# jmschrei/PyPore

Measured on NVIDIA B200. Metric: Msamples/s segmented (threshold+SpeedyStatSplit), higher is better.
Workload: dtype f64

## Files before the change

### include/pypore_b200.h

```cpp
#ifndef PYPORE_B200_H
#define PYPORE_B200_H

#include <stdint.h>

#ifdef __cplusplus
extern "C" {
#endif

typedef struct pp_ctx pp_ctx;

enum pp_status {
    PP_OK = 0,
    PP_ERR_CUDA = -1,
    PP_ERR_ARG = -2,
    PP_ERR_CAPACITY = -3,
    PP_ERR_STATE = -4,
    PP_ERR_FILTER_LEN = -5
};

enum pp_rule {
    PP_RULE_DURATION_GT = 1,
    PP_RULE_MIN_GT = 2,
    PP_RULE_MAX_LT = 4,
    PP_RULE_DURATION_LT = 8
};

enum pp_prefix_mode {
    PP_PREFIX_AUTO = 0,
    PP_PREFIX_SEQUENTIAL = 1,
    PP_PREFIX_PARALLEL = 2
};

int pp_version(void);
int pp_device_count(void);
int pp_create(int device, void *cuda_stream, pp_ctx **out);
void pp_destroy(pp_ctx *ctx);
const char *pp_last_error(pp_ctx *ctx);
int pp_sync(pp_ctx *ctx);
void *pp_stream(pp_ctx *ctx);
int pp_host_alloc(pp_ctx *ctx, int64_t bytes, void **out);
void pp_host_free(pp_ctx *ctx, void *p);
enum pp_option {
    PP_OPT_SCREEN = 0,
    PP_OPT_SPINE = 1,
    PP_OPT_SPLIT_CTAS = 2,
    PP_OPT_SPLIT_KERNEL = 3
};
int pp_set_option(pp_ctx *ctx, int option, int64_t value);
int pp_get_option(pp_ctx *ctx, int option, int64_t *value);
int64_t pp_launch_count(pp_ctx *ctx);
int pp_stage_ms(pp_ctx *ctx, int stage, float *ms);

int pp_trace_upload(pp_ctx *ctx, const float *host, int64_t n, int64_t extra_capacity);
int pp_trace_upload_f64(pp_ctx *ctx, const double *host, int64_t n);
int pp_trace_upload_adc16(pp_ctx *ctx, const int16_t *host, int64_t n, double scale, double offset);
int pp_adc16_check(double scale, double offset);
int pp_adc16_key_threshold(double scale, double offset, double threshold, int32_t *key, int32_t *kxor);
int pp_trace_prefetch(pp_ctx *ctx, const float *host, int64_t n, int64_t extra_capacity);
int pp_trace_swap(pp_ctx *ctx);
int pp_trace_prefetch_ms(pp_ctx *ctx, float *ms);
int pp_trace_adopt(pp_ctx *ctx, const float *dev, int64_t n, int64_t capacity);
int pp_trace_append(pp_ctx *ctx, const float *src, int64_t n, int src_is_device);
int pp_trace_truncate(pp_ctx *ctx, int64_t n);
int pp_trace_extend(pp_ctx *ctx, int64_t n);
int64_t pp_trace_len(pp_ctx *ctx);
const float *pp_trace_device_ptr(pp_ctx *ctx);

int pp_threshold_scan(pp_ctx *ctx, double threshold, int64_t scan_len, int64_t *n_runs);
int pp_runs_download(pp_ctx *ctx, int64_t cap, int64_t *start, int64_t *length, double *mn,
                     double *mx, uint8_t *below);
int pp_runs_download_range(pp_ctx *ctx, int64_t first, int64_t count, int64_t *start, int64_t *length,
                           double *mn, double *mx, uint8_t *below);
int pp_select_events(pp_ctx *ctx, int rule_mask, int64_t duration_gt, int64_t duration_lt,
                     double min_gt, double max_lt, int skip_first, int skip_last,
                     int64_t *n_events, int64_t *n_event_samples);
int pp_set_events(pp_ctx *ctx, const int64_t *start, const int64_t *length, int64_t n_events);
int pp_append_event(pp_ctx *ctx, int64_t start, int64_t length);
int pp_events_download(pp_ctx *ctx, int64_t cap, int64_t *start, int64_t *length);

int pp_events_upload_f64(pp_ctx *ctx, const double *host, const int64_t *length, int64_t n_events);

int pp_filter_events(pp_ctx *ctx, const double *b, const double *a, const double *zi, int ncoef);
int pp_event_samples_download(pp_ctx *ctx, int64_t cap, double *out);

int pp_statsplit(pp_ctx *ctx, int min_width, int max_width, int window_width, double min_gain,
                 int prefix_mode, int64_t *n_segments);
int pp_prefix(pp_ctx *ctx, int prefix_mode);
int pp_window_gains(pp_ctx *ctx, int64_t ev, int n_windows, const int32_t *ps, const int32_t *pe, int min_width,
                    double *out, int64_t cap);

int pp_segment_stats(pp_ctx *ctx);
int pp_segments_download(pp_ctx *ctx, int64_t cap, int32_t *event, int64_t *start, int64_t *end,
                         double *mean, double *std, double *mn, double *mx);
int pp_event_stats_download(pp_ctx *ctx, int64_t cap, double *mean, double *std, double *mn, double *mx);
const void *pp_table_device_ptr(pp_ctx *ctx, int which);
int pp_split_counters(pp_ctx *ctx, int64_t out[8]);

int pp_debug_screen(pp_ctx *ctx, int64_t ev, int ps, int pe, int min_width, double *h_screen,
                    double *h_exact, uint8_t *ok, double *eps);
int pp_debug_prefix(pp_ctx *ctx, int64_t cap, double *c, double *c2, uint8_t *redone);

int pp_debug_lg2_error(pp_ctx *ctx, double *max_err);

typedef struct pp_pipeline_params {
    double threshold;
    int rule_mask;
    int64_t duration_gt, duration_lt;
    double min_gt, max_lt;
    int filter_ncoef;
    const double *filter_b, *filter_a, *filter_zi;
    int min_width, max_width, window_width;
    double min_gain;
    int prefix_mode;
    int with_stats;
} pp_pipeline_params;
int pp_pipeline(pp_ctx *ctx, const pp_pipeline_params *p, int64_t out[4]);
int pp_pipeline_host(pp_ctx *ctx, const float *host, int64_t n, int64_t chunk_samples,
                     const pp_pipeline_params *p, int64_t out[4]);
typedef struct pp_host_tables {
    int64_t cap_events;
    int64_t *ev_start, *ev_len;
    int64_t cap_segments;
    int32_t *seg_event;
    int64_t *seg_start, *seg_end;
    double *mean, *std, *min, *max;
} pp_host_tables;
int pp_pipeline_host_tables(pp_ctx *ctx, const float *host, int64_t n, int64_t chunk_samples,
                            const pp_pipeline_params *p, const pp_host_tables *tables, int64_t out[4]);
int pp_pipeline_host_adc16(pp_ctx *ctx, const int16_t *host, int64_t n, double scale, double offset,
                           int64_t chunk_samples, const pp_pipeline_params *p,
                           const pp_host_tables *tables , int64_t out[4]);

typedef struct pp_hmm {
    int n_states;
    const double *mean, *inv_std, *log_norm, *log_start, *log_trans , *log_end ;
} pp_hmm;
int pp_hmm_decode(pp_ctx *ctx, const pp_hmm *model, int algorithm, int merge, int64_t *n_segments);
int pp_hmm_decode_sequences(pp_ctx *ctx, const pp_hmm *model, int algorithm, const double *x, const int64_t *len,
                            int64_t n);
int pp_hmm_download(pp_ctx *ctx, int64_t cap_seq, double *log_prob, int64_t cap_states, int32_t *state);

int pp_shard_scan(pp_ctx *ctx, double threshold, int64_t scan_len, double *dev_record);
int pp_shard_finish(pp_ctx *ctx, const pp_pipeline_params *p, int skip_first, int skip_last, int has_event,
                    int64_t ev_start, int64_t ev_len, int64_t *dev_record);
int pp_shard_plan(pp_ctx *ctx, const double *dev_infos, int rank, int world, const pp_pipeline_params *p,
                  int64_t halo_avail, int64_t *dev_plan);
int pp_shard_finish_planned(pp_ctx *ctx, const pp_pipeline_params *p, const int64_t *dev_plan, int64_t *dev_record);
int pp_shard_commit(pp_ctx *ctx, const int64_t rec[8]);
int pp_ctl_create(pp_ctx *ctx, int rank, int world, void *ipc_handle_out, void **local_ptr_out);
int pp_ctl_open(pp_ctx *ctx, const void *ipc_handles, void *const *local_ptrs);
int pp_ctl_exchange(pp_ctx *ctx, const void *dev_src, int n_words, void *dev_dst);
typedef struct pp_unpacked_tables {
    int64_t cap_events, cap_segments;
    int64_t *ev_start, *ev_len;
    int64_t *seg_event, *seg_start, *seg_end;
    double *mean, *std, *min, *max;
} pp_unpacked_tables;
int pp_unpack_tables(pp_ctx *ctx, const int64_t *dev_gathered, int world, int64_t words_per_rank,
                     const int64_t *dev_records, const pp_unpacked_tables *out, int out_is_host, void *cuda_stream);
int pp_unpack_tables_range(pp_ctx *ctx, const int64_t *dev_gathered, int world, int64_t words_per_rank,
                           const int64_t *dev_records, int rank_lo, int rank_hi, const pp_unpacked_tables *out,
                           int out_is_host, void *cuda_stream);
int pp_pack_tables(pp_ctx *ctx, const int64_t *dev_records, int rank, int64_t sample_offset, int64_t *dev_out,
                   int64_t cap_words);

#ifdef __cplusplus
}
#endif
#endif
```

### pypore_b200/csrc/api.cu

```cuda
#include "common.cuh"
#include "threshold.cuh"
#include "prefix.cuh"
#include "split.cuh"
#include "split_flow.cuh"
#include "stats.cuh"
#include "filter.cuh"
#include "hmm.cuh"

#include <new>
#include <stdarg.h>
#include <stdlib.h>

#include <nvtx3/nvToolsExt.h>

namespace {

struct DevBuf {
    void *p = nullptr;
    size_t cap = 0;
};

enum { ST_THRESHOLD = 0, ST_SELECT, ST_FILTER, ST_PREFIX, ST_SPLIT, ST_COMPACT, ST_STATS, ST_COUNT };

struct StageRange {
    explicit StageRange(const char *name) { nvtxRangePushA(name); }
    ~StageRange() { nvtxRangePop(); }
};

}

struct pp_ctx {
    int device = 0;
    int sm_count = 148;
    cudaStream_t stream = nullptr;
    bool own_stream = false;
    char err[512] = {0};
    int64_t launches = 0;

    DevBuf trace_buf;
    struct Pending {
        DevBuf buf;
        int64_t n = -1;
        cudaEvent_t done = nullptr, t0 = nullptr, t1 = nullptr;
    } pend[2];
    int n_pend = 0;
    DevBuf trace_spare;
    const float *trace = nullptr;
    const double *trace64 = nullptr;
    const int16_t *trace16 = nullptr;
    PPAdc adc = {1.0, 0.0};
    int64_t n = 0, trace_cap = 0;
    bool adopted = false;

    PPCounters *ctr = nullptr;
    PPCounters *h_ctr = nullptr;

    DevBuf k1_rec, k1_staged, k1_blk, run_start, run_minkey, run_maxkey, run_len, run_min, run_max, run_below;
    int64_t cap_runs = 0;
    int64_t n_runs = -1;
    int64_t scan_len = 0;
    int64_t k1_tiles_done = 0;
    int k1_flip = 0;

    DevBuf ev_start, ev_len, ev_off;
    int64_t cap_events = 0;
    int64_t n_events = -1, n_event_samples = -1;
    int src_kind = 0;
    DevBuf flat64;
    int64_t flat_cap = 0;

    DevBuf cc, bits, tasks, ready, block_count, block_off, inexact, Ttab, ev_tile_off, k2_bits, k2_tiles;
    DevBuf hk;
    DevBuf unpack_flag;
    DevBuf ctl_buf, ctl_peers_dev;
    void *ctl_peers[64] = {nullptr};
    bool ctl_ipc[64] = {false};
    int ctl_rank = -1, ctl_world = 0;
    unsigned long long ctl_seq = 0;
    int opt_spine = 1;
    int T_len = 0;
    int opt_screen = 1;
    int opt_split_ctas = 0;
    int opt_split_kernel = PP_SPLIT_KERNEL_DEFAULT;
    int64_t q_cap = 0;
    DevBuf seg_flat, seg_event, seg_start, seg_end, seg_mean, seg_std, seg_min, seg_max;
    int64_t cap_segs = 0;
    int64_t n_segments = -1;
    bool stats_valid = false;
    int64_t split_counters[8] = {0, 0, 0, 0, 0, 0, 0, 0};
    bool prefix_valid = false;
    int prefix_mode = PP_PREFIX_AUTO;

    DevBuf evs_mean, evs_std, evs_min, evs_max;

    DevBuf filt_tmp, filt_carry, filt_coef;

    DevBuf hmm_model, hmm_x, hmm_off, hmm_logp, hmm_state, hmm_bp, hmm_next, hmm_old_flat, hmm_old_state;
    int64_t hmm_n_seq = -1, hmm_n_rows = -1;
    bool hmm_states = false;

    cudaStream_t copy_stream = nullptr;
    cudaEvent_t copy_ev = nullptr, compute_ev = nullptr;
    cudaEvent_t pf_t0 = nullptr, pf_t1 = nullptr;
    int64_t n_words = 0, n_blocks = 0;

    cudaEvent_t ev[ST_COUNT + 1] = {0};
    bool stage_ran[ST_COUNT] = {false};
    bool rec[ST_COUNT + 1] = {false};
};

namespace {

int fail(pp_ctx *c, int code, const char *fmt, ...)
{
    if (c) {
        va_list ap;
        va_start(ap, fmt);
        vsnprintf(c->err, sizeof c->err, fmt, ap);
        va_end(ap);
    }
    return code;
}

#define CK(call)                                                                          \
    do {                                                                                  \
        cudaError_t e_ = (call);                                                          \
        if (e_ != cudaSuccess)                                                            \
            return fail(ctx, PP_ERR_CUDA, "%s failed: %s (%s:%d)", #call,                 \
                        cudaGetErrorString(e_), __FILE__, __LINE__);                      \
    } while (0)

#define CKR(call)                              \
    do {                                       \
        int r_ = (call);                       \
        if (r_ != PP_OK) return r_;            \
    } while (0)

#define LAUNCHED(ctx)                                                                     \
    do {                                                                                  \
        (ctx)->launches++;                                                                \
        cudaError_t e_ = cudaGetLastError();                                              \
        if (e_ != cudaSuccess)                                                            \
            return fail(ctx, PP_ERR_CUDA, "kernel launch failed: %s (%s:%d)",             \
                        cudaGetErrorString(e_), __FILE__, __LINE__);                      \
    } while (0)

int ensure(pp_ctx *ctx, DevBuf &b, size_t bytes)
{
    if (bytes <= b.cap && b.p) return PP_OK;
    bytes = (bytes + 255) & ~(size_t)255;
    CK(cudaStreamSynchronize(ctx->stream));
    if (b.p) CK(cudaFree(b.p));
    b.p = nullptr;
    b.cap = 0;
    CK(cudaMalloc(&b.p, bytes));
    b.cap = bytes;
    return PP_OK;
}

void release(DevBuf &b)
{
    if (b.p) cudaFree(b.p);
    b.p = nullptr;
    b.cap = 0;
}

int set_device(pp_ctx *ctx)
{
    CK(cudaSetDevice(ctx->device));
    return PP_OK;
}

int record_boundary(pp_ctx *ctx, int i)
{
    CK(cudaEventRecord(ctx->ev[i], ctx->stream));
    ctx->rec[i] = true;
    return PP_OK;
}

void reset_stages(pp_ctx *ctx)
{
    for (int i = 0; i < ST_COUNT; ++i) ctx->stage_ran[i] = false;
    for (int i = 0; i <= ST_COUNT; ++i) ctx->rec[i] = false;
}

PPSource make_source(pp_ctx *ctx)
{
    PPSource s;
    s.trace = ctx->trace;
    s.trace64 = ctx->trace64;
    s.trace16 = ctx->trace16;
    s.adc = ctx->adc;
    s.flat = (const double *)ctx->flat64.p;
    s.ev_start = (const int64_t *)ctx->ev_start.p;
    s.ev_off = (const int64_t *)ctx->ev_off.p;
    s.kind = ctx->src_kind;
    return s;
}

bool has_trace(const pp_ctx *ctx) { return ctx->trace || ctx->trace64 || ctx->trace16; }

int trace_kind(const pp_ctx *ctx)
{
    return ctx->trace64 ? PP_SRC_TRACE64 : ctx->trace16 ? PP_SRC_ADC16 : PP_SRC_TRACE32;
}

void point_trace(pp_ctx *ctx, void *p, size_t elem)
{
    ctx->trace = elem == sizeof(float) ? (const float *)p : nullptr;
    ctx->trace64 = elem == sizeof(double) ? (const double *)p : nullptr;
    ctx->trace16 = elem == sizeof(int16_t) ? (const int16_t *)p : nullptr;
}

const double *f64_samples(pp_ctx *ctx)
{
    return ctx->src_kind == PP_SRC_TRACE64 ? ctx->trace64 : (const double *)ctx->flat64.p;
}
const int64_t *f64_bases(pp_ctx *ctx)
{
    return (const int64_t *)(ctx->src_kind == PP_SRC_TRACE64 ? ctx->ev_start.p : ctx->ev_off.p);
}

int fetch_counters(pp_ctx *ctx)
{
    CK(cudaMemcpyAsync(ctx->h_ctr, ctx->ctr, sizeof(PPCounters), cudaMemcpyDeviceToHost, ctx->stream));
    CK(cudaStreamSynchronize(ctx->stream));
    return PP_OK;
}

int ensure_run_buffers(pp_ctx *ctx, int64_t cap_runs)
{
    if (cap_runs <= ctx->cap_runs) return PP_OK;
    CKR(ensure(ctx, ctx->run_start, sizeof(int64_t) * cap_runs));
    CKR(ensure(ctx, ctx->run_minkey, sizeof(unsigned long long) * cap_runs));
    CKR(ensure(ctx, ctx->run_maxkey, sizeof(unsigned long long) * cap_runs));
    CKR(ensure(ctx, ctx->run_len, sizeof(int64_t) * cap_runs));
    CKR(ensure(ctx, ctx->run_min, sizeof(double) * cap_runs));
// ... 42 lines not shown
int launch_threshold_tiles(pp_ctx *ctx, const T *x, typename K1Key<T>::V thr, int kxor, int64_t upto,
                           int64_t tile_begin, int64_t ntiles)
{
    const size_t smem = sizeof(K1Smem<T>);
    static int per_sm = 0;
    if (per_sm == 0) {
        CK(cudaFuncSetAttribute(k1_scan_tiles<T>, cudaFuncAttributeMaxDynamicSharedMemorySize, (int)smem));
        int nb = 0;
        CK(cudaOccupancyMaxActiveBlocksPerMultiprocessor(&nb, k1_scan_tiles<T>, K1_CTA_THREADS, smem));
        per_sm = nb > 0 ? nb : 1;
    }
    int64_t grid = (int64_t)ctx->sm_count * per_sm;
    if (grid > ntiles) grid = ntiles;
    k1_scan_tiles<T><<<(unsigned)grid, K1_CTA_THREADS, smem, ctx->stream>>>(
        x, upto, thr, kxor, tile_begin, ntiles, (K1Record *)ctx->k1_rec.p, (K1Staged *)ctx->k1_staged.p);
    LAUNCHED(ctx);
    const int64_t rec_begin = tile_begin * K1_WARPS, rec_end = (tile_begin + ntiles) * K1_WARPS;
    const int64_t nblk = (rec_end - rec_begin + K1B_THREADS - 1) / K1B_THREADS;
    CK(cudaMemsetAsync(ctx->k1_blk.p, 0, sizeof(unsigned long long) * nblk, ctx->stream));
    k1_stitch<T><<<(unsigned)nblk, K1B_THREADS, 0, ctx->stream>>>(
        x, upto, thr, kxor, rec_begin, rec_end, (const K1Record *)ctx->k1_rec.p, (const K1Staged *)ctx->k1_staged.p,
        (unsigned long long *)ctx->k1_blk.p, ctx->ctr, ctx->k1_flip, (int64_t *)ctx->run_start.p,
        (unsigned long long *)ctx->run_minkey.p, (unsigned long long *)ctx->run_maxkey.p, ctx->cap_runs);
    LAUNCHED(ctx);
    ctx->k1_flip ^= 1;
    return PP_OK;
}

int enqueue_threshold_tiles(pp_ctx *ctx, double threshold, int64_t upto, int64_t ntiles)
{
    StageRange nvtx_range("pypore:threshold");
    if (ntiles > 0) {
        if (ctx->trace64) {
            CKR(launch_threshold_tiles<double>(ctx, ctx->trace64, threshold, 0, upto, ctx->k1_tiles_done, ntiles));
        } else if (ctx->trace16) {
            int32_t key = 0, kxor = 0;
            pp_adc16_key_threshold(ctx->adc.scale, ctx->adc.offset, threshold, &key, &kxor);
            CKR(launch_threshold_tiles<int16_t>(ctx, ctx->trace16, key, kxor, upto, ctx->k1_tiles_done, ntiles));
        } else {
            float thr_f = (float)threshold;
            if ((double)thr_f < threshold) thr_f = nextafterf(thr_f, INFINITY);
            CKR(launch_threshold_tiles<float>(ctx, ctx->trace, thr_f, 0, upto, ctx->k1_tiles_done, ntiles));
        }
        ctx->k1_tiles_done += ntiles;
    }
    k1_finalize_runs<<<ctx->sm_count, 256, 0, ctx->stream>>>(
        upto, ctx->ctr, (const int64_t *)ctx->run_start.p, (const unsigned long long *)ctx->run_minkey.p,
        (const unsigned long long *)ctx->run_maxkey.p, ctx->cap_runs, (int64_t *)ctx->run_len.p,
        (double *)ctx->run_min.p, (double *)ctx->run_max.p, (unsigned char *)ctx->run_below.p,
        ctx->trace16 != nullptr, ctx->adc);
    LAUNCHED(ctx);
    return PP_OK;
}

int enqueue_threshold(pp_ctx *ctx, double threshold, int64_t scan_len)
{
    if (!has_trace(ctx) || ctx->n <= 0) return fail(ctx, PP_ERR_STATE, "no trace resident");
    if (scan_len < 0 || scan_len > ctx->n) scan_len = ctx->n;
    CKR(begin_threshold(ctx, scan_len));
    return enqueue_threshold_tiles(ctx, threshold, scan_len, (scan_len + K1_TILE - 1) / K1_TILE);
}

int enqueue_select(pp_ctx *ctx, int rule_mask, int64_t duration_gt, int64_t duration_lt,
                   double min_gt, double max_lt, int skip_first, int skip_last, int incremental = 0,
                   const long long *dev_plan = nullptr)
{
    StageRange nvtx_range("pypore:select");
    ctx->src_kind = trace_kind(ctx);
    ctx->flat_cap = ctx->n;
    k1_select_events<<<1, SEL_THREADS, 0, ctx->stream>>>(
        ctx->ctr, (const int64_t *)ctx->run_start.p, (const int64_t *)ctx->run_len.p,
        (const double *)ctx->run_min.p, (const double *)ctx->run_max.p, ctx->cap_runs, rule_mask,
        duration_gt, duration_lt, min_gt, max_lt, skip_first, skip_last, (int64_t *)ctx->ev_start.p,
        (int64_t *)ctx->ev_len.p, (int64_t *)ctx->ev_off.p, ctx->cap_events, incremental, dev_plan);
    LAUNCHED(ctx);
    ctx->n_events = ctx->n_event_samples = ctx->n_segments = -1;
    ctx->stats_valid = false;
    ctx->prefix_valid = false;
    return PP_OK;
}

template <int NZ>
void launch_filter_sequential(pp_ctx *ctx, const PPSource &src, int backward)
{
    k5_filter_sequential<NZ><<<ctx->sm_count * 8, 64, 0, ctx->stream>>>(
        src, (const int64_t *)ctx->ev_len.p, ctx->ctr, (const K5Coef *)ctx->filt_coef.p,
        (double *)ctx->filt_tmp.p, (double *)ctx->flat64.p, backward);
}

template <int NZ>
void launch_filter_pass(pp_ctx *ctx, const PPSource &src, int backward)
{
    cudaFuncSetAttribute(k5_filter_pass<NZ>, cudaFuncAttributeMaxDynamicSharedMemorySize,
                         (int)k5_smem_bytes<NZ>());
    k5_filter_pass<NZ><<<ctx->sm_count * 4, K5_THREADS, k5_smem_bytes<NZ>(), ctx->stream>>>(
        src, (const int64_t *)ctx->ev_len.p, ctx->ctr, (const K5Coef *)ctx->filt_coef.p,
        (double *)ctx->filt_tmp.p, (double *)ctx->flat64.p, backward);
}

int enqueue_filter(pp_ctx *ctx, const double *b, const double *a, const double *zi, int nc)
{
    StageRange nvtx_range("pypore:filter");
    if (nc < 2 || nc > FILT_MAX_COEF) return fail(ctx, PP_ERR_ARG, "filter order must be 1..%d", FILT_NZ);
    if (a[0] != 1.0) return fail(ctx, PP_ERR_ARG, "filter coefficients must be normalised (a[0] == 1)");
    const int64_t ncap = ctx->flat_cap;
    if (ncap <= 0) return fail(ctx, PP_ERR_STATE, "no events selected");
    const int P = 3 * nc;
    int64_t max_events = ncap / (P + 1) + 1;
    if (ctx->n_events >= 0 && ctx->n_events < max_events) max_events = ctx->n_events;
    if (ctx->cap_events < max_events) max_events = ctx->cap_events;
    CKR(ensure(ctx, ctx->filt_tmp, sizeof(double) * (size_t)(ncap + 2 * P * max_events + 64)));
    CKR(ensure(ctx, ctx->flat64, sizeof(double) * (size_t)ncap));
    CKR(ensure(ctx, ctx->filt_coef, sizeof(K5Coef)));
    K5Coef C;
    k5_prepare(b, a, zi, nc, &C);
    CK(cudaMemcpyAsync(ctx->filt_coef.p, &C, sizeof C, cudaMemcpyHostToDevice, ctx->stream));
    for (int backward = 0; backward < 2; ++backward) {
        PPSource src = make_source(ctx);
        switch (nc - 1) {
        case 1: launch_filter_pass<1>(ctx, src, backward); break;
        case 2: launch_filter_pass<2>(ctx, src, backward); break;
        case 3: launch_filter_sequential<3>(ctx, src, backward); break;
        case 4: launch_filter_sequential<4>(ctx, src, backward); break;
        case 5: launch_filter_sequential<5>(ctx, src, backward); break;
        case 6: launch_filter_sequential<6>(ctx, src, backward); break;
        case 7: launch_filter_sequential<7>(ctx, src, backward); break;
        default: launch_filter_sequential<8>(ctx, src, backward); break;
        }
        LAUNCHED(ctx);
    }
    ctx->src_kind = PP_SRC_FLAT64;
    CKR(record_boundary(ctx, ST_FILTER + 1));
    ctx->stage_ran[ST_FILTER] = true;
    ctx->n_segments = -1;
    ctx->stats_valid = false;
    ctx->prefix_valid = false;
    return PP_OK;
}

int prepare_split(pp_ctx *ctx, int mw, int MW, int W)
{
    if (mw < 0 || MW < mw || W < 2 * mw || W / 2 < 1)
        return fail(ctx, PP_ERR_ARG, "invalid split parameters (min_width=%d max_width=%d window_width=%d)",
                    mw, MW, W);
    const int64_t ncap = ctx->flat_cap;
    if (ncap <= 0) return fail(ctx, PP_ERR_STATE, "no events selected");
    const int64_t div = mw > 0 ? mw : 1;
    const int64_t cap_segs = 2 * (ncap / div) + ctx->cap_events + 16;
    const int64_t q_cap = ctx->cap_events + 2 * (ncap / div) + 1024;
    const int64_t n_words = (ncap + 31) / 32 + 1;
    const int64_t n_blocks = (n_words + CP_BLOCK_WORDS - 1) / CP_BLOCK_WORDS;
    CKR(ensure(ctx, ctx->cc, sizeof(double2) * ncap));
    CKR(ensure(ctx, ctx->bits, sizeof(unsigned) * n_words));
    CKR(ensure(ctx, ctx->tasks, sizeof(PPTask) * q_cap));
    CKR(ensure(ctx, ctx->ready, sizeof(int) * q_cap));
    CKR(ensure(ctx, ctx->block_count, sizeof(unsigned) * n_blocks));
    CKR(ensure(ctx, ctx->block_off, sizeof(unsigned long long) * n_blocks));
    if (cap_segs > ctx->cap_segs) {
        CKR(ensure(ctx, ctx->seg_flat, sizeof(int64_t) * cap_segs));
        CKR(ensure(ctx, ctx->seg_event, sizeof(int) * cap_segs));
        CKR(ensure(ctx, ctx->seg_start, sizeof(int64_t) * cap_segs));
        CKR(ensure(ctx, ctx->seg_end, sizeof(int64_t) * cap_segs));
        CKR(ensure(ctx, ctx->seg_mean, sizeof(double) * cap_segs));
        CKR(ensure(ctx, ctx->seg_std, sizeof(double) * cap_segs));
        CKR(ensure(ctx, ctx->seg_min, sizeof(double) * cap_segs));
        CKR(ensure(ctx, ctx->seg_max, sizeof(double) * cap_segs));
        ctx->cap_segs = cap_segs;
    }
    ctx->q_cap = q_cap;
    ctx->n_words = n_words;
    ctx->n_blocks = n_blocks;
    if (W + 1 > ctx->T_len) {
        CKR(ensure(ctx, ctx->Ttab, sizeof(double) * (size_t)(W + 1)));
        k3_fill_RN<<<ctx->sm_count, 256, 0, ctx->stream>>>((double *)ctx->Ttab.p, W + 1);
        LAUNCHED(ctx);
        ctx->T_len = W + 1;
    }
    CK(cudaMemsetAsync(ctx->bits.p, 0, sizeof(unsigned) * n_words, ctx->stream));
    CK(cudaMemsetAsync(&ctx->ctr->seg_done, 0, 3 * sizeof(unsigned long long), ctx->stream));
    return PP_OK;
}

template <typename T>
int enqueue_prefix_tiled(pp_ctx *ctx, const PPSource &src, const T *samples, int prefix_mode)
{
    k2_event_scan<T><<<ctx->sm_count * K2F_CFG_CTAS * 2, K2F_WARPS * 32, 0, ctx->stream>>>(
        src, samples, (const int64_t *)ctx->ev_len.p, ctx->ctr, (unsigned *)ctx->inexact.p, (double2 *)ctx->cc.p,
        prefix_mode != PP_PREFIX_PARALLEL);
    LAUNCHED(ctx);
    const int grid = ctx->sm_count * 8;
    k2_tile_reduce<T><<<grid, K2_THREADS, 0, ctx->stream>>>(
        src, samples, (const int64_t *)ctx->ev_len.p, (const int64_t *)ctx->ev_tile_off.p, ctx->ctr,
        (K2TileState *)ctx->k2_tiles.p, (K2EventBits *)ctx->k2_bits.p);
    LAUNCHED(ctx);
    k2_event_carries<<<ctx->sm_count * 2, 256, 0, ctx->stream>>>(
        ctx->ctr, (const int64_t *)ctx->ev_len.p, (const int64_t *)ctx->ev_tile_off.p,
        (K2TileState *)ctx->k2_tiles.p, (const K2EventBits *)ctx->k2_bits.p, (unsigned *)ctx->inexact.p,
        prefix_mode != PP_PREFIX_PARALLEL);
    LAUNCHED(ctx);
    k2_tile_scan<T><<<grid, K2_THREADS, 0, ctx->stream>>>(
        src, samples, (const int64_t *)ctx->ev_len.p, (const int64_t *)ctx->ev_tile_off.p, ctx->ctr,
        (const K2TileState *)ctx->k2_tiles.p, (double2 *)ctx->cc.p);
    LAUNCHED(ctx);
    return PP_OK;
}

int enqueue_prefix(pp_ctx *ctx, int prefix_mode)
{
    StageRange nvtx_range("pypore:prefix");
    const int64_t ncap = ctx->flat_cap;
    PPSource src = make_source(ctx);
    ctx->prefix_mode = prefix_mode;
    if (prefix_mode == PP_PREFIX_SEQUENTIAL) {
        k2_prefix_sequential<<<ctx->sm_count * 3, K2S_WARPS * 32, 0, ctx->stream>>>(
            src, (const int64_t *)ctx->ev_len.p, ctx->ctr, nullptr, (double2 *)ctx->cc.p);
        LAUNCHED(ctx);
    } else {
        const int64_t max_tiles = ncap / K2_TILE + ctx->cap_events + 2;
        CKR(ensure(ctx, ctx->ev_tile_off, sizeof(int64_t) * (ctx->cap_events + 2)));
        CKR(ensure(ctx, ctx->k2_bits, sizeof(K2EventBits) * (ctx->cap_events + 1)));
        CKR(ensure(ctx, ctx->inexact, sizeof(unsigned) * (ctx->cap_events + 1)));
        CKR(ensure(ctx, ctx->k2_tiles, sizeof(K2TileState) * (size_t)max_tiles));
        k2_tile_offsets<<<1, 1024, 0, ctx->stream>>>(ctx->ctr, (const int64_t *)ctx->ev_len.p,
                                                     (int64_t *)ctx->ev_tile_off.p, (K2EventBits *)ctx->k2_bits.p,
                                                     (unsigned *)ctx->inexact.p);
        LAUNCHED(ctx);
        if (ctx->src_kind == PP_SRC_TRACE32) CKR(enqueue_prefix_tiled<float>(ctx, src, ctx->trace, prefix_mode));
        else if (ctx->src_kind == PP_SRC_ADC16) CKR(enqueue_prefix_tiled<int16_t>(ctx, src, ctx->trace16, prefix_mode));
        else CKR(enqueue_prefix_tiled<double>(ctx, src, f64_samples(ctx), prefix_mode));
        if (prefix_mode != PP_PREFIX_PARALLEL) {
            k2_prefix_sequential<<<ctx->sm_count * 3, K2S_WARPS * 32, 0, ctx->stream>>>(
                src, (const int64_t *)ctx->ev_len.p, ctx->ctr, (const unsigned *)ctx->inexact.p,
                (double2 *)ctx->cc.p);
            LAUNCHED(ctx);
        }
    }
    return PP_OK;
}

int enqueue_search(pp_ctx *ctx, int mw, int MW, int W, double min_gain)
{
    StageRange nvtx_range("pypore:split");
    const int64_t q_cap = ctx->q_cap;
    CK(cudaMemsetAsync(ctx->ready.p, 0, sizeof(int) * q_cap, ctx->stream));
    K3Global G;
    G.cc = (const double2 *)ctx->cc.p;
    G.ev_off = (const int64_t *)ctx->ev_off.p;
    G.ev_len = (const int64_t *)ctx->ev_len.p;
    G.bits = (unsigned *)ctx->bits.p;
    G.tasks = (PPTask *)ctx->tasks.p;
    G.ready = (int *)ctx->ready.p;
    G.q_cap = q_cap;
    G.ctr = ctx->ctr;
    if (W + 1 > ctx->T_len) {
        CKR(ensure(ctx, ctx->Ttab, sizeof(double) * (size_t)(W + 1)));
        k3_fill_RN<<<ctx->sm_count, 256, 0, ctx->stream>>>((double *)ctx->Ttab.p, W + 1);
        LAUNCHED(ctx);
        ctx->T_len = W + 1;
    }
    G.RN = (const double *)ctx->Ttab.p;
    G.screen = ctx->opt_screen;
#if K3_CFG_HALFKEY
    CKR(ensure(ctx, ctx->hk, 2 * sizeof(unsigned long long) * (size_t)ctx->flat_cap));
    G.hkL = (unsigned long long *)ctx->hk.p;
    G.hkR = G.hkL + ctx->flat_cap;
#endif
    K3Params P;
    P.mw = mw; P.MW = MW; P.W = W; P.min_gain = min_gain;
    k3_init_queue<<<ctx->sm_count, 256, 0, ctx->stream>>>(G, ctx->opt_spine);
    LAUNCHED(ctx);
    if (ctx->opt_spine) {
        k3_spine<<<(ctx->sm_count / K3S_CLUSTER) * K3S_CLUSTER, K3S_THREADS, 0, ctx->stream>>>(G, P);
        LAUNCHED(ctx);
    }
    const int wave = ctx->sm_count * (ctx->opt_split_kernel ? K3F_CTAS_PER_SM : K3_CTAS_PER_SM);
    const int k3_grid = ctx->opt_split_ctas > 0 && ctx->opt_split_ctas < wave ? ctx->opt_split_ctas : wave;
    if (ctx->opt_split_kernel)
        k3_flow<<<k3_grid, K3F_THREADS, K3F_SMEM_BYTES, ctx->stream>>>(G, P);
    else
        k3_split<<<k3_grid, K3_THREADS, K3_SMEM_BYTES, ctx->stream>>>(G, P);
    LAUNCHED(ctx);
    return PP_OK;
}

int enqueue_compact(pp_ctx *ctx)
{
    StageRange nvtx_range("pypore:compact");
    const int64_t n_blocks = ctx->n_blocks;
    k3c_count<<<(unsigned)n_blocks, CP_THREADS, 0, ctx->stream>>>((const unsigned *)ctx->bits.p, ctx->ctr,
                                                                 (unsigned *)ctx->block_count.p);
    LAUNCHED(ctx);
    k3c_scan<<<1, 1024, 0, ctx->stream>>>((const unsigned *)ctx->block_count.p,
                                          (unsigned long long *)ctx->block_off.p, ctx->ctr, ctx->cap_segs);
    LAUNCHED(ctx);
    k3c_write<<<(unsigned)n_blocks, CP_THREADS, 0, ctx->stream>>>(
        (const unsigned *)ctx->bits.p, (const unsigned long long *)ctx->block_off.p,
        (const int64_t *)ctx->ev_off.p, ctx->ctr, (int64_t *)ctx->seg_flat.p, (int *)ctx->seg_event.p,
        (int64_t *)ctx->seg_start.p, ctx->cap_segs);
    LAUNCHED(ctx);
    k3c_ends<<<ctx->sm_count, 256, 0, ctx->stream>>>(ctx->ctr, (const int64_t *)ctx->seg_flat.p,
                                                     (const int *)ctx->seg_event.p,
                                                     (const int64_t *)ctx->ev_off.p,
                                                     (int64_t *)ctx->seg_end.p, ctx->cap_segs);
    LAUNCHED(ctx);
    return PP_OK;
}

int enqueue_export(pp_ctx *ctx, const PPHostTables &H, int with_stats)
{
    StageRange nvtx_range("pypore:export");
    k_export_tables<<<ctx->sm_count * 2, 256, 0, ctx->stream>>>(
        ctx->ctr, H, (const int64_t *)ctx->ev_start.p, (const int64_t *)ctx->ev_len.p, (const int *)ctx->seg_event.p,
        (const int64_t *)ctx->seg_start.p, (const int64_t *)ctx->seg_end.p, (const double *)ctx->seg_mean.p,
        (const double *)ctx->seg_std.p, (const double *)ctx->seg_min.p, (const double *)ctx->seg_max.p, with_stats);
    LAUNCHED(ctx);
    k_tables_advance<<<1, 32, 0, ctx->stream>>>(ctx->ctr);
    LAUNCHED(ctx);
    return PP_OK;
}

int enqueue_split(pp_ctx *ctx, int mw, int MW, int W, double min_gain, int prefix_mode)
{
    CKR(prepare_split(ctx, mw, MW, W));
    CKR(enqueue_prefix(ctx, prefix_mode));
    ctx->prefix_valid = true;
    CKR(record_boundary(ctx, ST_PREFIX + 1));
    ctx->stage_ran[ST_PREFIX] = true;
    CKR(enqueue_search(ctx, mw, MW, W, min_gain));
    CKR(record_boundary(ctx, ST_SPLIT + 1));
    ctx->stage_ran[ST_SPLIT] = true;
    CKR(enqueue_compact(ctx));
    CKR(record_boundary(ctx, ST_COMPACT + 1));
    ctx->stage_ran[ST_COMPACT] = true;
    ctx->n_segments = -1;
    ctx->stats_valid = false;
    return PP_OK;
}

int launch_stats(pp_ctx *ctx, int rows_are_events, const int64_t *flat_start, const int *row_event, int64_t cap_rows,
                 double *mean, double *sd, double *mn, double *mx)
{
    const unsigned grid = ctx->sm_count * 8;
    const int64_t *ev_off = (const int64_t *)ctx->ev_off.p;
    if (ctx->src_kind == PP_SRC_TRACE32)
        k4_segment_stats<float><<<grid, 256, 0, ctx->stream>>>(
            ctx->trace, (const int64_t *)ctx->ev_start.p, ev_off, ctx->ctr, rows_are_events, flat_start, row_event,
            cap_rows, mean, sd, mn, mx, ctx->adc);
    else if (ctx->src_kind == PP_SRC_ADC16)
        k4_segment_stats<int16_t><<<grid, 256, 0, ctx->stream>>>(
            ctx->trace16, (const int64_t *)ctx->ev_start.p, ev_off, ctx->ctr, rows_are_events, flat_start, row_event,
            cap_rows, mean, sd, mn, mx, ctx->adc);
    else
        k4_segment_stats<double><<<grid, 256, 0, ctx->stream>>>(
            f64_samples(ctx), f64_bases(ctx), ev_off, ctx->ctr, rows_are_events, flat_start, row_event, cap_rows,
            mean, sd, mn, mx, ctx->adc);
    LAUNCHED(ctx);
    return PP_OK;
}

int enqueue_stats(pp_ctx *ctx)
{
    StageRange nvtx_range("pypore:stats");
    CKR(launch_stats(ctx, 0, (const int64_t *)ctx->seg_flat.p, (const int *)ctx->seg_event.p, ctx->cap_segs,
                     (double *)ctx->seg_mean.p, (double *)ctx->seg_std.p, (double *)ctx->seg_min.p,
                     (double *)ctx->seg_max.p));
    CKR(record_boundary(ctx, ST_STATS + 1));
    ctx->stage_ran[ST_STATS] = true;
    ctx->stats_valid = true;
    return PP_OK;
}

int check_overflow(pp_ctx *ctx)
{
    const unsigned o = ctx->h_ctr->overflow;
    if (o & PP_OVF_QUEUE) return fail(ctx, PP_ERR_CAPACITY, "split work queue overflow");
    if (o & PP_OVF_SEGS) return fail(ctx, PP_ERR_CAPACITY, "segment table overflow");
    if (o & PP_OVF_FILTER_SHORT)
        return fail(ctx, PP_ERR_FILTER_LEN,
                    "The length of the input vector x must be greater than padlen");
    return PP_OK;
}

void absorb_counters(pp_ctx *ctx)
{
    const PPCounters *h = ctx->h_ctr;
    ctx->n_events = (int64_t)h->n_events;
    ctx->n_event_samples = (int64_t)h->n_event_samples;
    ctx->split_counters[0] = (int64_t)h->n_cand;
    ctx->split_counters[1] = (int64_t)h->n_scan;
    ctx->split_counters[2] = (int64_t)h->n_seq_redo;
    ctx->split_counters[3] = (int64_t)h->n_tasks;
    ctx->split_counters[4] = (int64_t)h->n_exact;
    ctx->split_counters[5] = (int64_t)h->n_sure;
    ctx->split_counters[6] = (int64_t)h->n_multi;
    ctx->split_counters[7] = (int64_t)h->n_full;
}

}

extern "C" {

int pp_version(void) { return 100; }

int pp_device_count(void)
{
    int n = 0;
    if (cudaGetDeviceCount(&n) != cudaSuccess) return 0;
    return n;
}

int pp_create(int device, void *cuda_stream, pp_ctx **out)
{
    if (!out) return PP_ERR_ARG;
    *out = nullptr;
    pp_ctx *ctx = new (std::nothrow) pp_ctx();
    if (!ctx) return PP_ERR_ARG;
    ctx->device = device;
    cudaError_t e = cudaSetDevice(device);
    if (e != cudaSuccess) { delete ctx; return PP_ERR_CUDA; }
    cudaDeviceProp prop;
    if (cudaGetDeviceProperties(&prop, device) != cudaSuccess) { delete ctx; return PP_ERR_CUDA; }
    ctx->sm_count = prop.multiProcessorCount;
    if (prop.major < 10) {
        delete ctx;
        return PP_ERR_CUDA;
    }
    if (cuda_stream) {
        ctx->stream = (cudaStream_t)cuda_stream;
    } else {
        if (cudaStreamCreateWithFlags(&ctx->stream, cudaStreamNonBlocking) != cudaSuccess) {
            delete ctx;
            return PP_ERR_CUDA;
        }
        ctx->own_stream = true;
    }
    bool ok = cudaMalloc((void **)&ctx->ctr, sizeof(PPCounters)) == cudaSuccess &&
              cudaMallocHost((void **)&ctx->h_ctr, sizeof(PPCounters)) == cudaSuccess &&
              cudaMemset(ctx->ctr, 0, sizeof(PPCounters)) == cudaSuccess;
    for (int i = 0; ok && i <= ST_COUNT; ++i) ok = cudaEventCreate(&ctx->ev[i]) == cudaSuccess;
    ok = ok && cudaFuncSetAttribute(k3_split, cudaFuncAttributeMaxDynamicSharedMemorySize,
                                    (int)K3_SMEM_BYTES) == cudaSuccess;
    ok = ok && cudaFuncSetAttribute(k3_flow, cudaFuncAttributeMaxDynamicSharedMemorySize,
                                    (int)K3F_SMEM_BYTES) == cudaSuccess;
    if (!ok) { pp_destroy(ctx); return PP_ERR_CUDA; }
    memset(ctx->h_ctr, 0, sizeof(PPCounters));
    *out = ctx;
    return PP_OK;
}

void pp_destroy(pp_ctx *ctx)
{
    if (!ctx) return;
    cudaSetDevice(ctx->device);
    if (ctx->stream) cudaStreamSynchronize(ctx->stream);
    for (int q = 0; q < 64; ++q)
        if (ctx->ctl_ipc[q] && ctx->ctl_peers[q]) cudaIpcCloseMemHandle(ctx->ctl_peers[q]);
    DevBuf *bufs[] = {&ctx->trace_buf, &ctx->pend[0].buf, &ctx->pend[1].buf, &ctx->trace_spare, &ctx->k1_rec, &ctx->k1_staged, &ctx->k1_blk, &ctx->run_start, &ctx->run_minkey,
                      &ctx->run_maxkey, &ctx->run_len, &ctx->run_min, &ctx->run_max, &ctx->run_below,
                      &ctx->ev_start, &ctx->ev_len, &ctx->ev_off, &ctx->flat64, &ctx->cc, &ctx->bits,
                      &ctx->tasks, &ctx->ready, &ctx->block_count, &ctx->block_off, &ctx->inexact, &ctx->Ttab, &ctx->ev_tile_off, &ctx->k2_bits, &ctx->k2_tiles,
                      &ctx->seg_flat, &ctx->seg_event, &ctx->seg_start, &ctx->seg_end, &ctx->seg_mean,
                      &ctx->seg_std, &ctx->seg_min, &ctx->seg_max, &ctx->evs_mean, &ctx->evs_std,
                      &ctx->evs_min, &ctx->evs_max, &ctx->filt_tmp, &ctx->filt_carry, &ctx->filt_coef, &ctx->hk, &ctx->unpack_flag, &ctx->ctl_buf, &ctx->ctl_peers_dev,
                      &ctx->hmm_model, &ctx->hmm_x, &ctx->hmm_off, &ctx->hmm_logp, &ctx->hmm_state, &ctx->hmm_bp,
                      &ctx->hmm_next, &ctx->hmm_old_flat, &ctx->hmm_old_state};
    for (DevBuf *b : bufs) release(*b);
    if (ctx->ctr) cudaFree(ctx->ctr);
    if (ctx->h_ctr) cudaFreeHost(ctx->h_ctr);
    for (int i = 0; i <= ST_COUNT; ++i)
        if (ctx->ev[i]) cudaEventDestroy(ctx->ev[i]);
    if (ctx->copy_ev) cudaEventDestroy(ctx->copy_ev);
    if (ctx->compute_ev) cudaEventDestroy(ctx->compute_ev);
    if (ctx->pf_t0) cudaEventDestroy(ctx->pf_t0);
    if (ctx->pf_t1) cudaEventDestroy(ctx->pf_t1);
    for (auto &q : ctx->pend) {
        if (q.done) cudaEventDestroy(q.done);
        if (q.t0) cudaEventDestroy(q.t0);
        if (q.t1) cudaEventDestroy(q.t1);
    }
    if (ctx->copy_stream) cudaStreamDestroy(ctx->copy_stream);
    if (ctx->own_stream && ctx->stream) cudaStreamDestroy(ctx->stream);
    delete ctx;
}

const char *pp_last_error(pp_ctx *ctx) { return ctx ? ctx->err : "null context"; }

void *pp_stream(pp_ctx *ctx) { return ctx ? (void *)ctx->stream : nullptr; }

int pp_host_alloc(pp_ctx *ctx, int64_t bytes, void **out)
{
    if (!ctx || !out || bytes <= 0) return fail(ctx, PP_ERR_ARG, "bad host allocation");
    CKR(set_device(ctx));
    CK(cudaMallocHost(out, (size_t)bytes));
    return PP_OK;
}

void pp_host_free(pp_ctx *ctx, void *p)
{
    if (ctx) cudaSetDevice(ctx->device);
    if (p) cudaFreeHost(p);
}

int pp_sync(pp_ctx *ctx)
{
    if (!ctx) return PP_ERR_ARG;
    CKR(set_device(ctx));
    CK(cudaStreamSynchronize(ctx->stream));
    return PP_OK;
}

int pp_set_option(pp_ctx *ctx, int option, int64_t value)
{
    if (!ctx) return PP_ERR_ARG;
    switch (option) {
    case PP_OPT_SCREEN: ctx->opt_screen = value ? 1 : 0; return PP_OK;
    case PP_OPT_SPINE: ctx->opt_spine = value ? 1 : 0; return PP_OK;
    case PP_OPT_SPLIT_KERNEL: ctx->opt_split_kernel = value ? 1 : 0; return PP_OK;
    case PP_OPT_SPLIT_CTAS:
        if (value < 0 || value > (1 << 20)) return fail(ctx, PP_ERR_ARG, "bad CTA count %lld", (long long)value);
        ctx->opt_split_ctas = (int)value;
        return PP_OK;
    default: return fail(ctx, PP_ERR_ARG, "unknown option %d", option);
    }
}

int pp_get_option(pp_ctx *ctx, int option, int64_t *value)
{
    if (!ctx || !value) return PP_ERR_ARG;
    switch (option) {
    case PP_OPT_SCREEN: *value = ctx->opt_screen; return PP_OK;
    case PP_OPT_SPINE: *value = ctx->opt_spine; return PP_OK;
    case PP_OPT_SPLIT_KERNEL: *value = ctx->opt_split_kernel; return PP_OK;
    case PP_OPT_SPLIT_CTAS: *value = ctx->opt_split_ctas; return PP_OK;
    default: return fail(ctx, PP_ERR_ARG, "unknown option %d", option);
    }
}

int64_t pp_launch_count(pp_ctx *ctx) { return ctx ? ctx->launches : 0; }

int pp_stage_ms(pp_ctx *ctx, int stage, float *ms)
{
    if (!ctx || !ms || stage < 0 || stage >= ST_COUNT) return PP_ERR_ARG;
    *ms = 0.f;
    if (!ctx->stage_ran[stage] || !ctx->rec[stage + 1]) return PP_OK;
    int prev = stage;
    while (prev > 0 && !ctx->rec[prev]) --prev;
    if (!ctx->rec[prev]) return PP_OK;
    CK(cudaEventElapsedTime(ms, ctx->ev[prev], ctx->ev[stage + 1]));
    return PP_OK;
}

static int trace_upload_impl(pp_ctx *ctx, const void *host, int64_t n, int64_t extra_capacity, size_t elem)
{
    if (!ctx || !host || n <= 0 || extra_capacity < 0) return fail(ctx, PP_ERR_ARG, "bad trace");
    CKR(set_device(ctx));
    CKR(ensure(ctx, ctx->trace_buf, elem * (size_t)(n + extra_capacity)));
    CK(cudaMemcpyAsync(ctx->trace_buf.p, host, elem * (size_t)n, cudaMemcpyHostToDevice, ctx->stream));
    point_trace(ctx, ctx->trace_buf.p, elem);
    ctx->n = n;
    ctx->trace_cap = (int64_t)(ctx->trace_buf.cap / elem);
    ctx->adopted = false;
    ctx->n_runs = ctx->n_events = ctx->n_event_samples = ctx->n_segments = -1;
    ctx->prefix_valid = false;
    return PP_OK;
}

int pp_trace_upload(pp_ctx *ctx, const float *host, int64_t n, int64_t extra_capacity)
{
    return trace_upload_impl(ctx, host, n, extra_capacity, sizeof(float));
}

int pp_trace_upload_f64(pp_ctx *ctx, const double *host, int64_t n)
{
    return trace_upload_impl(ctx, host, n, 0, sizeof(double));
}

static double adc_decode_host(int c, double scale, double offset)
{
    volatile double prod = (double)c * scale;
    return prod + offset;
}

int pp_adc16_check(double scale, double offset)
{
    if (!isfinite(scale) || scale == 0.0 || !isfinite(offset)) return PP_ERR_ARG;
    if (!isfinite(adc_decode_host(-32768, scale, offset)) || !isfinite(adc_decode_host(32767, scale, offset)))
        return PP_ERR_ARG;
    return PP_OK;
}

int pp_adc16_key_threshold(double scale, double offset, double threshold, int32_t *key, int32_t *kxor)
{
    if (!key || !kxor || pp_adc16_check(scale, offset) != PP_OK) return PP_ERR_ARG;
    const int kx = scale < 0.0 ? -1 : 0;
    int lo = -32768, hi = 32768;
    while (lo < hi) {
        const int mid = lo + ((hi - lo) >> 1);
        if (!(adc_decode_host(mid ^ kx, scale, offset) < threshold)) hi = mid;
        else lo = mid + 1;
    }
    *key = lo;
    *kxor = kx;
    return PP_OK;
}

int pp_trace_upload_adc16(pp_ctx *ctx, const int16_t *host, int64_t n, double scale, double offset)
{
    if (pp_adc16_check(scale, offset) != PP_OK)
        return fail(ctx, PP_ERR_ARG, "ADC scale must be finite and non-zero, offset finite, every count decoding finite");
    CKR(trace_upload_impl(ctx, host, n, 0, sizeof(int16_t)));
    ctx->adc = PPAdc{scale, offset};
    return PP_OK;
}

static int ensure_copy_stream(pp_ctx *ctx)
{
    if (!ctx->copy_stream) {
        CK(cudaStreamCreateWithFlags(&ctx->copy_stream, cudaStreamNonBlocking));
        CK(cudaEventCreateWithFlags(&ctx->copy_ev, cudaEventDisableTiming));
        CK(cudaEventCreateWithFlags(&ctx->compute_ev, cudaEventDisableTiming));
    }
    return PP_OK;
}

int pp_trace_prefetch(pp_ctx *ctx, const float *host, int64_t n, int64_t extra_capacity)
{
    if (!ctx || !host || n <= 0 || extra_capacity < 0) return fail(ctx, PP_ERR_ARG, "bad trace");
    if (ctx->trace16) return fail(ctx, PP_ERR_STATE, "prefetch takes float32 traces; an ADC trace is resident");
    if (ctx->n_pend >= 2) return fail(ctx, PP_ERR_STATE, "two prefetched traces are already waiting for pp_trace_swap");
    CKR(set_device(ctx));
    CKR(ensure_copy_stream(ctx));
    pp_ctx::Pending &q = ctx->pend[ctx->n_pend];
    if (!q.done) {
        CK(cudaEventCreateWithFlags(&q.done, cudaEventDisableTiming));
        CK(cudaEventCreate(&q.t0));
        CK(cudaEventCreate(&q.t1));
    }
    if (!q.buf.p && ctx->trace_spare.p) {
        q.buf = ctx->trace_spare;
        ctx->trace_spare = DevBuf();
    }
    CKR(ensure(ctx, q.buf, sizeof(float) * (size_t)(n + extra_capacity)));
    CK(cudaEventRecord(ctx->compute_ev, ctx->stream));
    CK(cudaStreamWaitEvent(ctx->copy_stream, ctx->compute_ev, 0));
    CK(cudaEventRecord(q.t0, ctx->copy_stream));
    CK(cudaMemcpyAsync(q.buf.p, host, sizeof(float) * (size_t)n, cudaMemcpyHostToDevice, ctx->copy_stream));
    CK(cudaEventRecord(q.t1, ctx->copy_stream));
    CK(cudaEventRecord(q.done, ctx->copy_stream));
    q.n = n;
    ++ctx->n_pend;
    return PP_OK;
}

int pp_trace_prefetch_ms(pp_ctx *ctx, float *ms)
{
    if (!ctx || !ms) return PP_ERR_ARG;
    if (!ctx->pf_t1) return fail(ctx, PP_ERR_STATE, "no prefetched trace has been swapped in so far");
    CKR(set_device(ctx));
    CK(cudaEventSynchronize(ctx->pf_t1));
    CK(cudaEventElapsedTime(ms, ctx->pf_t0, ctx->pf_t1));
    return PP_OK;
}

int pp_trace_swap(pp_ctx *ctx)
{
    if (!ctx) return PP_ERR_ARG;
    if (ctx->n_pend <= 0) return fail(ctx, PP_ERR_STATE, "no prefetched trace");
    CKR(set_device(ctx));
    pp_ctx::Pending &q = ctx->pend[0];
    CK(cudaStreamWaitEvent(ctx->stream, q.done, 0));
    if (ctx->trace_spare.p) release(ctx->trace_spare);
    ctx->trace_spare = ctx->trace_buf;
    ctx->trace_buf = q.buf;
    q.buf = DevBuf();
    cudaEvent_t a = ctx->pf_t0, b = ctx->pf_t1;
    ctx->pf_t0 = q.t0; ctx->pf_t1 = q.t1;
    q.t0 = a; q.t1 = b;
    if (!q.t0) { CK(cudaEventCreate(&q.t0)); CK(cudaEventCreate(&q.t1)); }
    point_trace(ctx, ctx->trace_buf.p, sizeof(float));
    ctx->n = q.n;
    q.n = -1;
    if (ctx->n_pend == 2) {
        pp_ctx::Pending t = ctx->pend[0];
        ctx->pend[0] = ctx->pend[1];
        ctx->pend[1] = t;
    }
// ... 331 lines not shown
}

int pp_segment_stats(pp_ctx *ctx)
{
    if (!ctx) return PP_ERR_ARG;
    if (ctx->n_segments < 0) return fail(ctx, PP_ERR_STATE, "pp_statsplit has not run");
    CKR(set_device(ctx));
    reset_stages(ctx);
    CKR(record_boundary(ctx, ST_STATS));
    CKR(enqueue_stats(ctx));
    return PP_OK;
}

int pp_segments_download(pp_ctx *ctx, int64_t cap, int32_t *event, int64_t *start, int64_t *end,
                         double *mean, double *std, double *mn, double *mx)
{
    if (!ctx) return PP_ERR_ARG;
    if (ctx->n_segments < 0) return fail(ctx, PP_ERR_STATE, "pp_statsplit has not run");
    if (cap < ctx->n_segments) return fail(ctx, PP_ERR_CAPACITY, "segment buffers too small");
    if ((mean || std || mn || mx) && !ctx->stats_valid)
        return fail(ctx, PP_ERR_STATE, "pp_segment_stats has not run");
    CKR(set_device(ctx));
    const size_t s = (size_t)ctx->n_segments;
    if (s) {
        if (event) CK(cudaMemcpyAsync(event, ctx->seg_event.p, 4 * s, cudaMemcpyDeviceToHost, ctx->stream));
        if (start) CK(cudaMemcpyAsync(start, ctx->seg_start.p, 8 * s, cudaMemcpyDeviceToHost, ctx->stream));
        if (end) CK(cudaMemcpyAsync(end, ctx->seg_end.p, 8 * s, cudaMemcpyDeviceToHost, ctx->stream));
        if (mean) CK(cudaMemcpyAsync(mean, ctx->seg_mean.p, 8 * s, cudaMemcpyDeviceToHost, ctx->stream));
        if (std) CK(cudaMemcpyAsync(std, ctx->seg_std.p, 8 * s, cudaMemcpyDeviceToHost, ctx->stream));
        if (mn) CK(cudaMemcpyAsync(mn, ctx->seg_min.p, 8 * s, cudaMemcpyDeviceToHost, ctx->stream));
        if (mx) CK(cudaMemcpyAsync(mx, ctx->seg_max.p, 8 * s, cudaMemcpyDeviceToHost, ctx->stream));
    }
    CK(cudaStreamSynchronize(ctx->stream));
    return PP_OK;
}

int pp_event_stats_download(pp_ctx *ctx, int64_t cap, double *mean, double *std, double *mn, double *mx)
{
    if (!ctx) return PP_ERR_ARG;
    if (ctx->n_events < 0) return fail(ctx, PP_ERR_STATE, "no event table");
    if (cap < ctx->n_events) return fail(ctx, PP_ERR_CAPACITY, "event buffers too small");
    CKR(set_device(ctx));
    const size_t e = (size_t)ctx->n_events;
    if (!e) return PP_OK;
    CKR(ensure(ctx, ctx->evs_mean, 8 * e));
    CKR(ensure(ctx, ctx->evs_std, 8 * e));
    CKR(ensure(ctx, ctx->evs_min, 8 * e));
    CKR(ensure(ctx, ctx->evs_max, 8 * e));
    CKR(launch_stats(ctx, 1, (const int64_t *)ctx->ev_off.p, nullptr, (int64_t)e, (double *)ctx->evs_mean.p,
                     (double *)ctx->evs_std.p, (double *)ctx->evs_min.p, (double *)ctx->evs_max.p));
    if (mean) CK(cudaMemcpyAsync(mean, ctx->evs_mean.p, 8 * e, cudaMemcpyDeviceToHost, ctx->stream));
    if (std) CK(cudaMemcpyAsync(std, ctx->evs_std.p, 8 * e, cudaMemcpyDeviceToHost, ctx->stream));
    if (mn) CK(cudaMemcpyAsync(mn, ctx->evs_min.p, 8 * e, cudaMemcpyDeviceToHost, ctx->stream));
    if (mx) CK(cudaMemcpyAsync(mx, ctx->evs_max.p, 8 * e, cudaMemcpyDeviceToHost, ctx->stream));
    CK(cudaStreamSynchronize(ctx->stream));
    return PP_OK;
}

const void *pp_table_device_ptr(pp_ctx *ctx, int which)
{
    if (!ctx) return nullptr;
    switch (which) {
    case 0: return ctx->seg_event.p;
    case 1: return ctx->seg_start.p;
    case 2: return ctx->seg_end.p;
    case 3: return ctx->seg_mean.p;
    case 4: return ctx->seg_std.p;
    case 5: return ctx->seg_min.p;
    case 6: return ctx->seg_max.p;
    case 7: return ctx->ev_start.p;
    case 8: return ctx->ev_len.p;
    default: return nullptr;
    }
}

int pp_split_counters(pp_ctx *ctx, int64_t out[8])
{
    if (!ctx || !out) return PP_ERR_ARG;
    for (int i = 0; i < 8; ++i) out[i] = ctx->split_counters[i];
    return PP_OK;
}

int pp_debug_screen(pp_ctx *ctx, int64_t ev, int ps, int pe, int min_width, double *h_screen,
                    double *h_exact, uint8_t *ok, double *eps)
{
    if (!ctx || !h_screen || !h_exact || !ok) return PP_ERR_ARG;
    if (ctx->n_segments < 0) return fail(ctx, PP_ERR_STATE, "pp_statsplit has not run");
    const int n = pe - ps - 2 * min_width + 1;
    if (ev < 0 || ev >= ctx->n_events || ps < 0 || n <= 0 || pe - ps + 1 > ctx->T_len)
        return fail(ctx, PP_ERR_ARG, "bad debug window");
    CKR(set_device(ctx));
    DevBuf a, b, c;
    CKR(ensure(ctx, a, 8 * (size_t)n));
    CKR(ensure(ctx, b, 8 * (size_t)n));
    CKR(ensure(ctx, c, (size_t)n));
    K3Global G;
    memset(&G, 0, sizeof G);
    G.cc = (const double2 *)ctx->cc.p;
    G.ev_off = (const int64_t *)ctx->ev_off.p;
    G.RN = (const double *)ctx->Ttab.p;
    k3_debug_screen<<<64, 256, 0, ctx->stream>>>(G, (int)ev, ps, pe, min_width, (double *)a.p, (double *)b.p,
                                                 (unsigned char *)c.p);
    LAUNCHED(ctx);
    CK(cudaMemcpyAsync(h_screen, a.p, 8 * (size_t)n, cudaMemcpyDeviceToHost, ctx->stream));
    CK(cudaMemcpyAsync(h_exact, b.p, 8 * (size_t)n, cudaMemcpyDeviceToHost, ctx->stream));
    CK(cudaMemcpyAsync(ok, c.p, (size_t)n, cudaMemcpyDeviceToHost, ctx->stream));
    CK(cudaStreamSynchronize(ctx->stream));
    release(a); release(b); release(c);
    if (eps) *eps = (double)(pe - ps) * K3_EPS_PER_SAMPLE + K3_EPS_CONST;
    return PP_OK;
}

int pp_debug_prefix(pp_ctx *ctx, int64_t cap, double *c, double *c2, uint8_t *redone)
{
    if (!ctx || !c || !c2 || !redone) return PP_ERR_ARG;
    if (!ctx->prefix_valid) return fail(ctx, PP_ERR_STATE, "prefix sums are not resident (pp_prefix / pp_statsplit)");
    if (cap < ctx->n_event_samples || cap < ctx->n_events) return fail(ctx, PP_ERR_CAPACITY, "buffers too small");
    CKR(set_device(ctx));
    const size_t n = (size_t)ctx->n_event_samples, e = (size_t)ctx->n_events;
    double2 *cc = (double2 *)malloc(sizeof(double2) * (n ? n : 1));
    unsigned *fl = (unsigned *)malloc(sizeof(unsigned) * (e ? e : 1));
    if (!cc || !fl) { free(cc); free(fl); return fail(ctx, PP_ERR_ARG, "out of host memory"); }
    auto run = [&]() -> int {
        if (n) CK(cudaMemcpyAsync(cc, ctx->cc.p, sizeof(double2) * n, cudaMemcpyDeviceToHost, ctx->stream));
        if (e && ctx->prefix_mode == PP_PREFIX_AUTO)
            CK(cudaMemcpyAsync(fl, ctx->inexact.p, sizeof(unsigned) * e, cudaMemcpyDeviceToHost, ctx->stream));
        CK(cudaStreamSynchronize(ctx->stream));
        return PP_OK;
    };
    const int rc = run();
    if (rc == PP_OK) {
        for (size_t i = 0; i < n; ++i) { c[i] = cc[i].x; c2[i] = cc[i].y; }
        for (size_t i = 0; i < e; ++i)
            redone[i] = ctx->prefix_mode == PP_PREFIX_AUTO ? (fl[i] != 0u) : ctx->prefix_mode == PP_PREFIX_SEQUENTIAL;
    }
    free(cc); free(fl);
    return rc;
}

int pp_debug_lg2_error(pp_ctx *ctx, double *max_err)
{
    if (!ctx || !max_err) return PP_ERR_ARG;
    CKR(set_device(ctx));
    DevBuf a;
    CKR(ensure(ctx, a, 256));
    CK(cudaMemsetAsync(a.p, 0, 8, ctx->stream));
    k3_debug_lg2_error<<<ctx->sm_count * 4, 256, 0, ctx->stream>>>((unsigned long long *)a.p);
    LAUNCHED(ctx);
    CK(cudaMemcpyAsync(max_err, a.p, 8, cudaMemcpyDeviceToHost, ctx->stream));
    CK(cudaStreamSynchronize(ctx->stream));
    release(a);
    return PP_OK;
}

int pp_pipeline(pp_ctx *ctx, const pp_pipeline_params *p, int64_t out[4])
{
    if (!ctx || !p) return PP_ERR_ARG;
    CKR(set_device(ctx));
    for (int attempt = 0; attempt < 2; ++attempt) {
        reset_stages(ctx);
        CKR(record_boundary(ctx, 0));
        CKR(enqueue_threshold(ctx, p->threshold, -1));
        CKR(record_boundary(ctx, ST_THRESHOLD + 1));
        ctx->stage_ran[ST_THRESHOLD] = true;
        CKR(enqueue_select(ctx, p->rule_mask, p->duration_gt, p->duration_lt, p->min_gt, p->max_lt, 0, 0));
        CKR(record_boundary(ctx, ST_SELECT + 1));
        ctx->stage_ran[ST_SELECT] = true;
        if (p->filter_ncoef > 0)
            CKR(enqueue_filter(ctx, p->filter_b, p->filter_a, p->filter_zi, p->filter_ncoef));
        CKR(enqueue_split(ctx, p->min_width, p->max_width, p->window_width, p->min_gain, p->prefix_mode));
        if (p->with_stats) CKR(enqueue_stats(ctx));
        CKR(fetch_counters(ctx));
        const int64_t runs = (int64_t)ctx->h_ctr->n_runs;
        if (runs > ctx->cap_runs) {
            CKR(ensure_run_buffers(ctx, runs + 16));
            continue;
        }
        absorb_counters(ctx);
        ctx->n_runs = runs;
        CKR(check_overflow(ctx));
        ctx->n_segments = (int64_t)ctx->h_ctr->n_segments;
        if (out) {
            out[0] = runs;
            out[1] = ctx->n_events;
            out[2] = ctx->n_event_samples;
            out[3] = ctx->n_segments;
        }
        return PP_OK;
    }
    return fail(ctx, PP_ERR_CAPACITY, "run table overflow");
}

int pp_shard_scan(pp_ctx *ctx, double threshold, int64_t scan_len, double *dev_record)
{
    if (!ctx || !dev_record) return PP_ERR_ARG;
    if (ctx->trace16) return fail(ctx, PP_ERR_STATE, "the sharded path takes float32 traces");
    CKR(set_device(ctx));
    reset_stages(ctx);
    CKR(record_boundary(ctx, 0));
    CKR(enqueue_threshold(ctx, threshold, scan_len));
    CKR(record_boundary(ctx, ST_THRESHOLD + 1));
    ctx->stage_ran[ST_THRESHOLD] = true;
    k1_boundary_record<<<1, 32, 0, ctx->stream>>>(
        ctx->scan_len, ctx->ctr, (const int64_t *)ctx->run_start.p, (const int64_t *)ctx->run_len.p,
        (const double *)ctx->run_min.p, (const double *)ctx->run_max.p, (const unsigned char *)ctx->run_below.p,
        ctx->cap_runs, dev_record);
    LAUNCHED(ctx);
    return PP_OK;
}

int pp_shard_finish(pp_ctx *ctx, const pp_pipeline_params *p, int skip_first, int skip_last, int has_event,
                    int64_t ev_start, int64_t ev_len, int64_t *dev_record)
{
    if (!ctx || !p || !dev_record) return PP_ERR_ARG;
    if (ctx->trace16) return fail(ctx, PP_ERR_STATE, "the sharded path takes float32 traces");
    if (p->filter_ncoef > 0) return fail(ctx, PP_ERR_ARG, "the sharded path does not filter");
    CKR(set_device(ctx));
    CKR(enqueue_select(ctx, p->rule_mask, p->duration_gt, p->duration_lt, p->min_gt, p->max_lt, skip_first,
                       skip_last));
    if (has_event) {
        if (ev_start < 0 || ev_len <= 0 || ev_start + ev_len > ctx->n)
            return fail(ctx, PP_ERR_ARG, "bad appended event");
        k_append_event<<<1, 1, 0, ctx->stream>>>(ctx->ctr, (int64_t *)ctx->ev_start.p, (int64_t *)ctx->ev_len.p,
                                                 (int64_t *)ctx->ev_off.p, ev_start, ev_len);
        LAUNCHED(ctx);
    }
    CKR(record_boundary(ctx, ST_SELECT + 1));
    ctx->stage_ran[ST_SELECT] = true;
    CKR(enqueue_split(ctx, p->min_width, p->max_width, p->window_width, p->min_gain, p->prefix_mode));
    if (p->with_stats) CKR(enqueue_stats(ctx));
    k_result_record<<<1, 32, 0, ctx->stream>>>(ctx->ctr, (long long *)dev_record);
    LAUNCHED(ctx);
    return PP_OK;
}

int pp_shard_plan(pp_ctx *ctx, const double *dev_infos, int rank, int world, const pp_pipeline_params *p,
                  int64_t halo_avail, int64_t *dev_plan)
{
    if (!ctx || !p || !dev_infos || !dev_plan || world < 1 || rank < 0 || rank >= world || halo_avail < 0)
        return fail(ctx, PP_ERR_ARG, "bad shard plan arguments");
    if (ctx->trace16) return fail(ctx, PP_ERR_STATE, "the sharded path takes float32 traces");
    CKR(set_device(ctx));
    k_shard_plan<<<1, 32, 0, ctx->stream>>>(dev_infos, rank, world, p->rule_mask, p->duration_gt, p->duration_lt,
                                            p->min_gt, p->max_lt, halo_avail, (long long *)dev_plan);
    LAUNCHED(ctx);
    return PP_OK;
}

int pp_shard_finish_planned(pp_ctx *ctx, const pp_pipeline_params *p, const int64_t *dev_plan, int64_t *dev_record)
{
    if (!ctx || !p || !dev_plan || !dev_record) return PP_ERR_ARG;
    if (ctx->trace16) return fail(ctx, PP_ERR_STATE, "the sharded path takes float32 traces");
    if (p->filter_ncoef > 0) return fail(ctx, PP_ERR_ARG, "the sharded path does not filter");
    CKR(set_device(ctx));
    CKR(enqueue_select(ctx, p->rule_mask, p->duration_gt, p->duration_lt, p->min_gt, p->max_lt, 0, 0, 0,
                       (const long long *)dev_plan));
    k_append_planned_event<<<1, 32, 0, ctx->stream>>>(ctx->ctr, (int64_t *)ctx->ev_start.p, (int64_t *)ctx->ev_len.p,
                                                      (int64_t *)ctx->ev_off.p, ctx->cap_events,
                                                      (const long long *)dev_plan);
    LAUNCHED(ctx);
    CKR(record_boundary(ctx, ST_SELECT + 1));
    ctx->stage_ran[ST_SELECT] = true;
    CKR(enqueue_split(ctx, p->min_width, p->max_width, p->window_width, p->min_gain, p->prefix_mode));
    if (p->with_stats) CKR(enqueue_stats(ctx));
    k_result_record<<<1, 32, 0, ctx->stream>>>(ctx->ctr, (long long *)dev_record, (const long long *)dev_plan);
    LAUNCHED(ctx);
    return PP_OK;
}

int pp_shard_commit(pp_ctx *ctx, const int64_t rec[8])
{
    if (!ctx || !rec) return PP_ERR_ARG;
    if (ctx->trace16) return fail(ctx, PP_ERR_STATE, "the sharded path takes float32 traces");
    ctx->n_runs = rec[0];
    ctx->n_events = rec[1];
    ctx->n_event_samples = rec[2];
    ctx->n_segments = rec[3];
    ctx->split_counters[0] = rec[5];
    ctx->split_counters[1] = rec[6];
    ctx->split_counters[4] = rec[7];
    const unsigned o = (unsigned)rec[4];
    if (o & PP_OVF_CTL) return fail(ctx, PP_ERR_STATE, "a peer's control record did not arrive (pp_ctl_exchange timed out)");
    if (rec[0] > ctx->cap_runs) return fail(ctx, PP_ERR_CAPACITY, "run table overflow");
    if (o & PP_OVF_QUEUE) return fail(ctx, PP_ERR_CAPACITY, "split work queue overflow");
    if (o & PP_OVF_SEGS) return fail(ctx, PP_ERR_CAPACITY, "segment table overflow");
    return PP_OK;
}

int pp_pack_tables(pp_ctx *ctx, const int64_t *dev_records, int rank, int64_t sample_offset, int64_t *dev_out,
                   int64_t cap_words)
{
    if (!ctx || !dev_out || !dev_records || rank < 0) return PP_ERR_ARG;
    CKR(set_device(ctx));
    k_pack_tables<<<ctx->sm_count * 4, 256, 0, ctx->stream>>>(
        (const long long *)dev_records, rank, cap_words, sample_offset, (const int64_t *)ctx->ev_start.p,
        (const int64_t *)ctx->ev_len.p, (const int *)ctx->seg_event.p, (const int64_t *)ctx->seg_start.p,
        (const int64_t *)ctx->seg_end.p, (const double *)ctx->seg_mean.p, (const double *)ctx->seg_std.p,
        (const double *)ctx->seg_min.p, (const double *)ctx->seg_max.p, (long long *)dev_out);
    LAUNCHED(ctx);
    return PP_OK;
}

int pp_ctl_create(pp_ctx *ctx, int rank, int world, void *ipc_handle_out, void **local_ptr_out)
{
    if (!ctx || rank < 0 || world < 1 || world > PP_MAX_WORLD || rank >= world)
        return fail(ctx, PP_ERR_ARG, "bad control-exchange arguments");
    CKR(set_device(ctx));
    const size_t bytes = sizeof(unsigned long long) * 2 * (size_t)world * PP_CTL_SLOT;
    CKR(ensure(ctx, ctx->ctl_buf, bytes));
    CK(cudaMemsetAsync(ctx->ctl_buf.p, 0, ctx->ctl_buf.cap, ctx->stream));
    CK(cudaStreamSynchronize(ctx->stream));
    ctx->ctl_rank = rank;
    ctx->ctl_world = world;
    ctx->ctl_seq = 0;
    if (ipc_handle_out) {
        cudaIpcMemHandle_t h;
        CK(cudaIpcGetMemHandle(&h, ctx->ctl_buf.p));
        memcpy(ipc_handle_out, &h, sizeof h);
    }
    if (local_ptr_out) *local_ptr_out = ctx->ctl_buf.p;
    return PP_OK;
}

int pp_ctl_open(pp_ctx *ctx, const void *ipc_handles, void *const *local_ptrs)
{
    if (!ctx || ctx->ctl_world < 1 || (!ipc_handles && !local_ptrs))
        return fail(ctx, PP_ERR_ARG, "pp_ctl_create first; handles or pointers of every rank");
    CKR(set_device(ctx));
    for (int q = 0; q < ctx->ctl_world; ++q) {
        if (q == ctx->ctl_rank) { ctx->ctl_peers[q] = ctx->ctl_buf.p; continue; }
        if (local_ptrs) { ctx->ctl_peers[q] = local_ptrs[q]; continue; }
        cudaIpcMemHandle_t h;
        memcpy(&h, (const char *)ipc_handles + (size_t)q * sizeof h, sizeof h);
        CK(cudaIpcOpenMemHandle(&ctx->ctl_peers[q], h, cudaIpcMemLazyEnablePeerAccess));
        ctx->ctl_ipc[q] = true;
    }
    CKR(ensure(ctx, ctx->ctl_peers_dev, sizeof(void *) * PP_MAX_WORLD));
    CK(cudaMemcpyAsync(ctx->ctl_peers_dev.p, ctx->ctl_peers, sizeof(void *) * (size_t)ctx->ctl_world,
                       cudaMemcpyHostToDevice, ctx->stream));
    CK(cudaStreamSynchronize(ctx->stream));
    return PP_OK;
}

int pp_ctl_exchange(pp_ctx *ctx, const void *dev_src, int n_words, void *dev_dst)
{
    if (!ctx || !dev_src || !dev_dst || n_words < 1 || n_words > PP_CTL_PAYLOAD)
        return fail(ctx, PP_ERR_ARG, "bad control record");
    if (!ctx->ctl_peers_dev.p) return fail(ctx, PP_ERR_STATE, "pp_ctl_open has not run");
    CKR(set_device(ctx));
    const unsigned long long seq = ++ctx->ctl_seq;
    k_ctl_exchange<<<1, 64, 0, ctx->stream>>>((unsigned long long *const *)ctx->ctl_peers_dev.p, ctx->ctl_rank,
                                              ctx->ctl_world, seq, (const unsigned long long *)dev_src, n_words,
                                              (unsigned long long *)dev_dst, ctx->ctr);
    LAUNCHED(ctx);
    return PP_OK;
}

int pp_unpack_tables(pp_ctx *ctx, const int64_t *dev_gathered, int world, int64_t words_per_rank,
                     const int64_t *dev_records, const pp_unpacked_tables *out, int out_is_host, void *cuda_stream)
{
    return pp_unpack_tables_range(ctx, dev_gathered, world, words_per_rank, dev_records, 0, world, out, out_is_host,
                                  cuda_stream);
}

int pp_unpack_tables_range(pp_ctx *ctx, const int64_t *dev_gathered, int world, int64_t words_per_rank,
                           const int64_t *dev_records, int rank_lo, int rank_hi, const pp_unpacked_tables *out,
                           int out_is_host, void *cuda_stream)
{
    if (!ctx || !dev_gathered || !dev_records || !out || world < 1 || world > PP_MAX_WORLD || words_per_rank < 0 ||
        rank_lo < 0 || rank_hi > world || rank_lo >= rank_hi ||
        (words_per_rank & 1) || !out->ev_start || !out->ev_len || !out->seg_event || !out->seg_start ||
        !out->seg_end || !out->mean || !out->std || !out->min || !out->max)
        return fail(ctx, PP_ERR_ARG, "bad unpack arguments");
    CKR(set_device(ctx));
    PPUnpacked O;
    O.cap_events = out->cap_events;
    O.cap_segments = out->cap_segments;
    void *src[9] = {out->ev_start, out->ev_len, out->seg_event, out->seg_start, out->seg_end,
                    out->mean, out->std, out->min, out->max};
    void *dst[9];
    for (int i = 0; i < 9; ++i) {
        dst[i] = src[i];
        if (out_is_host) CK(cudaHostGetDevicePointer(&dst[i], src[i], 0));
    }
    O.ev_start = (long long *)dst[0]; O.ev_len = (long long *)dst[1];
    O.seg_event = (long long *)dst[2]; O.seg_start = (long long *)dst[3]; O.seg_end = (long long *)dst[4];
    O.mean = (double *)dst[5]; O.sd = (double *)dst[6]; O.mn = (double *)dst[7]; O.mx = (double *)dst[8];
    CKR(ensure(ctx, ctx->unpack_flag, 256));
    cudaStream_t st = cuda_stream ? (cudaStream_t)cuda_stream : ctx->stream;
    CK(cudaMemsetAsync(ctx->unpack_flag.p, 0, sizeof(unsigned), st));
    k_unpack_tables<<<ctx->sm_count * 4, 256, 0, st>>>(
        (const long long *)dev_gathered, world, words_per_rank, (const long long *)dev_records, rank_lo, rank_hi, O,
        (unsigned *)ctx->unpack_flag.p);
    LAUNCHED(ctx);
    if (cuda_stream) return PP_OK;
    unsigned flag = 0;
    CK(cudaMemcpyAsync(&flag, ctx->unpack_flag.p, sizeof flag, cudaMemcpyDeviceToHost, st));
    CK(cudaStreamSynchronize(st));
    if (flag & 1u) return fail(ctx, PP_ERR_CAPACITY, "unpack tables too small");
    return PP_OK;
}

static int pipeline_host_impl(pp_ctx *ctx, const void *host, int kind, PPAdc adc, int64_t n, int64_t chunk_samples,
                              const pp_pipeline_params *p, const pp_host_tables *tables, int64_t out[4])
{
    if (!ctx || !p || !host || n <= 0) return fail(ctx, PP_ERR_ARG, "bad trace");
    const size_t elem = kind == PP_SRC_ADC16 ? sizeof(int16_t) : sizeof(float);
    CKR(set_device(ctx));
    PPHostTables H;
    memset(&H, 0, sizeof H);
    if (tables) {
        if (tables->cap_events < 0 || tables->cap_segments < 0 || !tables->ev_start || !tables->ev_len ||
            !tables->seg_event || !tables->seg_start || !tables->seg_end ||
            (p->with_stats && (!tables->mean || !tables->std || !tables->min || !tables->max)))
            return fail(ctx, PP_ERR_ARG, "incomplete host tables");
        H.cap_events = tables->cap_events;
        H.cap_segments = tables->cap_segments;
        CK(cudaHostGetDevicePointer((void **)&H.ev_start, tables->ev_start, 0));
        CK(cudaHostGetDevicePointer((void **)&H.ev_len, tables->ev_len, 0));
        CK(cudaHostGetDevicePointer((void **)&H.seg_event, tables->seg_event, 0));
        CK(cudaHostGetDevicePointer((void **)&H.seg_start, tables->seg_start, 0));
        CK(cudaHostGetDevicePointer((void **)&H.seg_end, tables->seg_end, 0));
        if (p->with_stats) {
            CK(cudaHostGetDevicePointer((void **)&H.mean, tables->mean, 0));
            CK(cudaHostGetDevicePointer((void **)&H.sd, tables->std, 0));
            CK(cudaHostGetDevicePointer((void **)&H.mn, tables->min, 0));
            CK(cudaHostGetDevicePointer((void **)&H.mx, tables->max, 0));
        }
    }
    if (chunk_samples <= 0) chunk_samples = (int64_t)16 << 20;
    chunk_samples = (chunk_samples + K1_TILE - 1) / K1_TILE * K1_TILE;
    if (p->filter_ncoef > 0 || n <= chunk_samples) {
        if (kind == PP_SRC_ADC16) CKR(pp_trace_upload_adc16(ctx, (const int16_t *)host, n, adc.scale, adc.offset));
        else CKR(pp_trace_upload(ctx, (const float *)host, n, 0));
        CKR(pp_pipeline(ctx, p, out));
        if (tables) {
// ... 290 lines not shown
```

### pypore_b200/csrc/split.cuh

```cuda
#pragma once
#include "common.cuh"
#include <cooperative_groups.h>

#ifndef K3_CFG_THREADS
#define K3_CFG_THREADS 128
#endif
#ifndef K3_CFG_CTAS
#define K3_CFG_CTAS 7
#endif
constexpr int K3_THREADS = K3_CFG_THREADS;
constexpr int K3_CTAS_PER_SM = K3_CFG_CTAS;
constexpr int K3_WARPS = K3_THREADS / 32;
constexpr int K3_CAP = 10240;
#ifndef K3_CFG_LIST
#define K3_CFG_LIST 128
#endif
#ifndef K3_CFG_SURE
#define K3_CFG_SURE 1
#endif
#ifndef K3_CFG_SHARE
#define K3_CFG_SHARE 0
#endif
constexpr int K3_LIST = K3_CFG_LIST;
constexpr int K3_REQ = K3_CFG_LIST;
constexpr int K3_SHARE = K3_CFG_SHARE;
#ifndef K3_CFG_IDLE_SHARE
#define K3_CFG_IDLE_SHARE 512
#endif
constexpr int K3_IDLE_SHARE = K3_CFG_IDLE_SHARE;
constexpr int K3_PIECES = K3_LIST + K3_WARPS;
#ifndef K3_CFG_LDCS
#define K3_CFG_LDCS 0
#endif
#ifndef K3_CFG_PREFETCH
#define K3_CFG_PREFETCH 1
#endif
#ifndef K3_CFG_HALFKEY
#define K3_CFG_HALFKEY 0
#endif
constexpr int K3_NO_EBASE = 0x7fffffff;
constexpr unsigned long long K3_NO_TICKET = ~0ull;
constexpr int K3_FULL_FLAG = 0x40000000;
constexpr int K3_MULTI_FLAG = 0x20000000;
constexpr unsigned K3_ALLOC_SLOT = 1u << 20;
constexpr int K3_BAD_FLAG = 0x40000000;
constexpr int K3_RESCAN_FLAG = (int)0x80000000;
constexpr int K3_MAX_SCREEN_W = 1 << 24;

constexpr int K3_RATIO_BITS = 24;
constexpr double K3_EPS_PER_SAMPLE = 3.6e-7;
constexpr double K3_EPS_CONST = 1e-6;
constexpr double K3_KEY_PER_NAT = 12102203.161561485;
constexpr double K3_HUGE = 1e280;
constexpr unsigned long long K3_NOKEY = ~0ull;

struct PPTask { int ev, s, e, flags; };
struct K3Item { int s, e, ps, pad; };
struct K3Params { int mw, MW, W; double min_gain; };
struct K3Best { double g; int x; };
struct K3Scr { unsigned long long k1, k2; int i1, bad; };
struct K3Branches { unsigned sure, multi, full; };

struct K3Global {
    const double2 *cc;
    const int64_t *ev_off;
    const int64_t *ev_len;
    unsigned *bits;
    PPTask *tasks;
    int *ready;
    int64_t q_cap;
    PPCounters *ctr;
    const double *RN;
    int screen;
#if K3_CFG_HALFKEY
    unsigned long long *hkL, *hkR;
#endif
};

struct K3Level {
    K3Item item[K3_LIST];
    int c0[K3_LIST];
    int cn[K3_LIST];
    int flag[K3_LIST];
};

struct K3Count {
    unsigned alloc;
    int nfull;
    int nreq, nrescan, nmulti;
};

struct K3Shared {
    K3Level lv[2];
    K3Count cnt[3];
    unsigned long long win_thr[K3_LIST];
    unsigned long long best_key[K3_LIST];
    int best_idx[K3_LIST];
    unsigned long long pc_k1[K3_PIECES];
    unsigned long long pc_k2[K3_PIECES];
    int pc_i1[K3_PIECES];
    unsigned long long pc_kt[K3_PIECES];
    int req_k[K3_REQ];
    int req_i[K3_REQ];
    double req_g[K3_REQ];
    double red_g[K3_WARPS];
    unsigned long long red_k[K3_WARPS];
    int red_x[K3_WARPS];
    int share;
    int few;
    int have;
    int ev;
    long long off;
    int ebase;
    PPTask task;
    unsigned long long cand, scans, exact;
    unsigned n_sure, n_multi, n_full;
    unsigned n_cont;
    K3Global G;
    K3Params P;
};

constexpr size_t K3_SMEM_BYTES = sizeof(K3Shared);

struct K3GlobalCC {
    const double2 *g;
    __device__ __forceinline__ double2 at(int p) const
    {
        if (p < 0) return make_double2(0.0, 0.0);
        return __ldg(g + p);
    }
};

__device__ __forceinline__ double k3_var(const double2 hi, const double2 lo, int cnt)
{
    if (cnt == 0) return 0.0;
    const double n = (double)cnt;
    const double m = __ddiv_rn(__dsub_rn(hi.x, lo.x), n);
    return __dsub_rn(__ddiv_rn(__dsub_rn(hi.y, lo.y), n), __dmul_rn(m, m));
}

__device__ __forceinline__ K3Best k3_better(const K3Best a, const K3Best b)
{
    if (b.x >= 0 && (a.x < 0 || b.g > a.g || (b.g == a.g && b.x < a.x))) return b;
    return a;
}

__device__ __forceinline__ double k3_exact_gain(const double2 lo, const double2 mid, const double2 hi,
                                                int ps, int pe, int i, double tot)
{
    const double low = __dmul_rn((double)(i - ps), log(k3_var(mid, lo, i - ps)));
    const double high = __dmul_rn((double)(pe - i), log(k3_var(hi, mid, pe - i)));
    return __dsub_rn(tot, __dadd_rn(low, high));
}

__device__ __forceinline__ double k3_exact_tot(const double2 lo, const double2 hi, int ps, int pe)
{
    return __dmul_rn((double)(pe - ps), log(k3_var(hi, lo, pe - ps)));
}

template <class CC>
__device__ __forceinline__ K3Best k3_scan_range(const CC &cc, int ps, int pe, int mw,
                                                double min_gain, int first, int stride)
{
    const double2 lo = cc.at(ps - 1), hi = cc.at(pe - 1);
    const double tot = k3_exact_tot(lo, hi, ps, pe);
    K3Best b;
    b.g = min_gain;
    b.x = -1;
    const int last = pe - mw;
    for (int i = ps + mw + first; i <= last; i += stride) {
        const double g = k3_exact_gain(lo, cc.at(i - 1), hi, ps, pe, i, tot);
        if (g > b.g) { b.g = g; b.x = i; }
    }
    return b;
}

__device__ __forceinline__ K3Best k3_warp_reduce(K3Best b)
{
#pragma unroll
    for (int d = 16; d > 0; d >>= 1) {
        K3Best o;
        o.g = __shfl_xor_sync(PP_FULL, b.g, d);
        o.x = __shfl_xor_sync(PP_FULL, b.x, d);
        b = k3_better(b, o);
    }
    return b;
}

__device__ __forceinline__ K3Best k3_cta_reduce(K3Best b, K3Shared &S)
{
    const int tid = threadIdx.x;
    b = k3_warp_reduce(b);
    __syncthreads();
    if ((tid & 31) == 0) { S.red_g[tid >> 5] = b.g; S.red_x[tid >> 5] = b.x; }
    __syncthreads();
    K3Best r;
    r.g = S.red_g[0];
    r.x = S.red_x[0];
#pragma unroll
    for (int w = 1; w < K3_WARPS; ++w) {
        K3Best o;
        o.g = S.red_g[w];
        o.x = S.red_x[w];
        r = k3_better(r, o);
    }
    return r;
}

__device__ __forceinline__ bool k3_window_ebase(double vtot, int &ebase)
{
    const int e = __double2hiint(vtot) >> 20;
    ebase = e - 127;
    return e >= 128 && e <= 1919;
}

__device__ __forceinline__ bool k3_side(double S, double Q, double r, unsigned n, int ebase,
                                        unsigned long long &key)
{
    const double m = __dmul_rn(S, r);
    const double m2 = __dmul_rn(m, m);
    const double V = fma(Q, r, -m2);
    const int vh = __double2hiint(V);
    const unsigned mant = (__funnelshift_l((unsigned)__double2loint(V), (unsigned)vh, 3) & 0x007fffffu) | 0x3f800000u;
    float lg;
    asm("lg2.approx.ftz.f32 %0, %1;" : "=f"(lg) : "f"(__uint_as_float(mant)));
    const unsigned tb = __float_as_uint(__fadd_rn(lg, 1.0f));
    const unsigned x = (unsigned)((vh >> 20) - ebase);
    const unsigned LV = x * 0x00800000u + tb;
    key += (unsigned long long)n * LV;
    return (x <= 254u) & ((__double2hiint(m2) - vh) < (K3_RATIO_BITS << 20));
}

__device__ __forceinline__ bool k3_screen_key(const double2 mid, const double r1, const double r2, const double2 lo,
                                              const double2 hi, unsigned n1, unsigned n2, int ebase,
                                              unsigned long long &key)
{
    key = 0ull;
    const bool ok1 = k3_side(__dsub_rn(mid.x, lo.x), __dsub_rn(mid.y, lo.y), r1, n1, ebase, key);
    const bool ok2 = k3_side(__dsub_rn(hi.x, mid.x), __dsub_rn(hi.y, mid.y), r2, n2, ebase, key);
    return ok1 & ok2;
}

__device__ __forceinline__ bool k3_screen_key_at(const double2 *__restrict__ ccg, const double2 lo, const double2 hi,
                                                 int ps, int pe, int i, const double *__restrict__ RN, int ebase,
                                                 unsigned long long &key)
{
    return k3_screen_key(__ldg(ccg + (i - 1)), __ldg(RN + (i - ps)), __ldg(RN + (pe - i)), lo, hi,
                         (unsigned)(i - ps), (unsigned)(pe - i), ebase, key);
}

__device__ __forceinline__ void k3_scr_init(K3Scr &a)
{
    a.k1 = a.k2 = K3_NOKEY;
    a.i1 = -1;
    a.bad = 0;
}

__device__ __forceinline__ void k3_scr_update(K3Scr &a, bool ok, unsigned long long key, int i)
{
    if (!ok) a.bad = 1;
    else if (key < a.k2) {
        if (key < a.k1) { a.k2 = a.k1; a.k1 = key; a.i1 = i; }
        else a.k2 = key;
    }
}

#ifndef K3_CFG_UNROLL
#define K3_CFG_UNROLL 2
#endif
#ifndef K3_CFG_L1PF
#define K3_CFG_L1PF 1
#endif
__device__ __forceinline__ void k3_prefetch_l1(const void *p) { asm volatile("prefetch.global.L1 [%0];" ::"l"(p)); }
#if K3_CFG_LDCS
#define K3_LD_MID(p) __ldcs(p)
// ... 130 lines not shown

template <int MODE>
__device__ __forceinline__ void k3_hk_eval(unsigned long long *hkL, unsigned long long *hkR, const double2 lo,
                                           const double2 hi, int ps, int pe, int ebase, int j, const double2 m,
                                           double r1, double r2, unsigned long long h, bool store, K3Scr &a)
{
    unsigned long long kl = 0ull, kr = 0ull;
    bool ok = true;
    if (MODE != 1) {
        ok = k3_side(__dsub_rn(m.x, lo.x), __dsub_rn(m.y, lo.y), r1, (unsigned)(j - ps), ebase, kl);
        if (store) __stcg(hkL + j, kl);
    } else {
        kl = h;
    }
    if (MODE != 2) {
        ok = ok & k3_side(__dsub_rn(hi.x, m.x), __dsub_rn(hi.y, m.y), r2, (unsigned)(pe - j), ebase, kr);
        if (store) __stcg(hkR + j, kr);
    } else {
        kr = h;
    }
    k3_scr_update(a, ok, kl + kr, j);
}

template <int MODE>
__device__ __forceinline__ void k3_screen_lane_hk(const double2 *__restrict__ ccg, unsigned long long *hkL,
                                                  unsigned long long *hkR, const double2 lo, const double2 hi, int ps,
                                                  int pe, int ebase, const double *__restrict__ RN, int i, int i_last,
                                                  int stride, bool store, K3Scr &a)
{
    if (i > i_last) return;
    double2 mA = make_double2(0.0, 0.0), mB = mA, mA_n = mA, mB_n = mA;
    double a1 = 0.0, a2 = 0.0, b1 = 0.0, b2 = 0.0, a1_n = 0.0, a2_n = 0.0, b1_n = 0.0, b2_n = 0.0;
    unsigned long long hA = 0ull, hB = 0ull, hA_n = 0ull, hB_n = 0ull;
    k3_hk_load<MODE>(ccg, hkL, hkR, RN, ps, pe, i, mA, a1, a2, hA);
    bool haveB = i + stride <= i_last;
    if (haveB) k3_hk_load<MODE>(ccg, hkL, hkR, RN, ps, pe, i + stride, mB, b1, b2, hB);
    for (;;) {
        const int in = i + 2 * stride;
        const bool nextA = haveB && in <= i_last, nextB = nextA && in + stride <= i_last;
        if (nextA) k3_hk_load<MODE>(ccg, hkL, hkR, RN, ps, pe, in, mA_n, a1_n, a2_n, hA_n);
        if (nextB) k3_hk_load<MODE>(ccg, hkL, hkR, RN, ps, pe, in + stride, mB_n, b1_n, b2_n, hB_n);
        k3_hk_eval<MODE>(hkL, hkR, lo, hi, ps, pe, ebase, i, mA, a1, a2, hA, store, a);
        if (haveB) k3_hk_eval<MODE>(hkL, hkR, lo, hi, ps, pe, ebase, i + stride, mB, b1, b2, hB, store, a);
        if (!nextA) break;
        i = in;
        mA = mA_n; a1 = a1_n; a2 = a2_n; hA = hA_n;
        mB = mB_n; b1 = b1_n; b2 = b2_n; hB = hB_n;
        haveB = nextB;
    }
}
#endif

__device__ __forceinline__ unsigned long long k3_eps2_key(int n)
{
    return (unsigned long long)(2.0 * ((double)n * K3_EPS_PER_SAMPLE + K3_EPS_CONST) * K3_KEY_PER_NAT) + 2ull;
}

__device__ __forceinline__ unsigned long long k3_okey(double g)
{
    const long long b = __double_as_longlong(__dadd_rn(g, 0.0));
    return (unsigned long long)(b ^ ((b >> 63) | (long long)0x8000000000000000LL));
}

__device__ __forceinline__ unsigned long long k3_warp_min_u64(unsigned long long k)
{
    const unsigned hi = (unsigned)(k >> 32);
    const unsigned mh = __reduce_min_sync(PP_FULL, hi);
    const unsigned lo = hi == mh ? (unsigned)k : 0xffffffffu;
    const unsigned ml = __reduce_min_sync(PP_FULL, lo);
    return ((unsigned long long)mh << 32) | ml;
}

__device__ __forceinline__ void k3_warp_summary(const K3Scr &a, unsigned long long &K1, unsigned long long &K2,
                                                int &I1, bool &bad)
{
    const int lane = threadIdx.x & 31;
    K1 = k3_warp_min_u64(a.k1);
    const int winner = __ffs(__ballot_sync(PP_FULL, a.k1 == K1)) - 1;
    K2 = k3_warp_min_u64(lane == winner ? a.k2 : a.k1);
    I1 = __shfl_sync(PP_FULL, a.i1, winner);
    bad = __any_sync(PP_FULL, a.bad != 0);
}

template <class CC>
__device__ __forceinline__ K3Best k3_cta_scan(const CC &cc, int ps, int pe, const K3Params &P,
                                              const K3Global &G, K3Shared &S)
{
    const int tid = threadIdx.x;
    K3Best b;
    b.g = P.min_gain;
    b.x = -1;
    const double2 lo = cc.at(ps - 1), hi = cc.at(pe - 1);
    const double tot = k3_exact_tot(lo, hi, ps, pe);
    int ebase = 0;
    bool screen = G.screen && P.mw >= 1 && pe - ps <= K3_MAX_SCREEN_W && fabs(tot) <= K3_HUGE;
    screen = screen && k3_window_ebase(k3_var(hi, lo, pe - ps), ebase);
    K3Scr a;
    k3_scr_init(a);
    if (screen) {
        k3_screen_lane(cc.g, lo, hi, ps, pe, ebase, G.RN, ps + P.mw + tid, pe - P.mw, K3_THREADS, a);
        if (__syncthreads_or(a.bad)) screen = false;
    }
    if (!screen) {
        if (tid == 0 && G.screen && P.mw >= 1 && P.W <= K3_MAX_SCREEN_W) S.n_full += 1;
        b = k3_scan_range(cc, ps, pe, P.mw, P.min_gain, tid, K3_THREADS);
        return k3_cta_reduce(b, S);
    }
    unsigned long long m = k3_warp_min_u64(a.k1);
    if ((tid & 31) == 0) S.red_k[tid >> 5] = m;
    __syncthreads();
    m = S.red_k[0];
#pragma unroll
    for (int w = 1; w < K3_WARPS; ++w) m = S.red_k[w] < m ? S.red_k[w] : m;
    const unsigned long long thr = m + k3_eps2_key(pe - ps);
    const unsigned ncont = (a.k1 <= thr ? 1u : 0u) + (a.k2 <= thr ? 1u : 0u);
    if (ncont) atomicAdd(&S.n_cont, ncont);
    unsigned nexact = 0;
    if (a.k2 <= thr) {
        const int last = pe - P.mw;
        for (int i = ps + P.mw + tid; i <= last; i += K3_THREADS) {
            unsigned long long key;
            k3_screen_key_at(cc.g, lo, hi, ps, pe, i, G.RN, ebase, key);
            if (key <= thr) {
                const double g = k3_exact_gain(lo, cc.at(i - 1), hi, ps, pe, i, tot);
                ++nexact;
                if (g > b.g) { b.g = g; b.x = i; }
            }
        }
    } else if (a.k1 <= thr) {
        const double g = k3_exact_gain(lo, cc.at(a.i1 - 1), hi, ps, pe, a.i1, tot);
        ++nexact;
        if (g > b.g) { b.g = g; b.x = a.i1; }
    }
    if (nexact) atomicAdd(&S.exact, (unsigned long long)nexact);
    b = k3_cta_reduce(b, S);
    if (tid == 0) {
        if (S.n_cont > 1) S.n_multi += 1;
        S.n_cont = 0;
    }
    return b;
}

__device__ __forceinline__ void k3_emit(const K3Global &G, int64_t off, int x)
{
    const int64_t f = off + x;
    atomicOr(&G.bits[f >> 5], 1u << (unsigned)(f & 31));
}

__device__ __forceinline__ bool k3_worth(const K3Params &P, int s, int e)
{
    return ((long long)e - s > 2LL * P.mw) || (e - s > P.MW);
}

__device__ void k3_push_global(const K3Global &G, int ev, int s, int e, int ps)
{
    atomicAdd((unsigned long long *)&G.ctr->q_pending, 1ull);
    const unsigned long long slot = atomicAdd(&G.ctr->q_tail, 1ull);
    if ((int64_t)slot >= G.q_cap) {
        atomicOr(&G.ctr->overflow, (unsigned)PP_OVF_QUEUE);
        atomicAdd((unsigned long long *)&G.ctr->q_pending, (unsigned long long)(-1LL));
        return;
    }
    PPTask t;
    t.ev = ev; t.s = s; t.e = e; t.flags = ps - s;
    *reinterpret_cast<int4 *>(&G.tasks[slot]) = *reinterpret_cast<int4 *>(&t);
    __threadfence();
    atomicExch(&G.ready[slot], 1);
}

__device__ __forceinline__ int k3_forced(const K3Params &P, int s, int e)
{
    const long long a = (long long)s + P.MW, b = (long long)e - P.mw;
    return (int)(a < b ? a : b);
}

__device__ __forceinline__ int k3_next_ps(const K3Params &P, int ps, int e)
{
    const long long n = (long long)ps + P.W / 2;
    return (int)(n < e ? n : e);
}

__device__ __forceinline__ int k3_window_end(const K3Params &P, const K3Item &it)
{
    const long long pe_l = (long long)it.ps + P.W;
    return (int)(pe_l < it.e ? pe_l : it.e);
}

__device__ __forceinline__ void k3_mark_full(K3Level &L, K3Count &C, int k)
{
    if (!(atomicOr(&L.flag[k], K3_FULL_FLAG) & K3_FULL_FLAG)) atomicAdd(&C.nfull, 1);
}

__device__ __noinline__ void k3_place(K3Shared *Sp, K3Level *nxp, K3Count *ncp, int screen, K3Item it)
{
    K3Shared &S = *Sp;
    const K3Global &G = S.G;
    const K3Params &P = S.P;
    K3Level &nx = *nxp;
    K3Count &nc = *ncp;
    const int mw = P.mw, MW = P.MW;
    const int64_t off = (int64_t)S.off;
    K3Item st[4];
    int sp = 0;
    for (;;) {
        for (;;) {
            const long long lim = (long long)it.e - 2LL * mw;
            if (it.ps >= lim) {
                if (it.e - it.s > MW) {
                    const int x = k3_forced(P, it.s, it.e);
                    k3_emit(G, off, x);
                    K3Item l, r;
                    l.s = it.s; l.e = x; l.ps = it.s; l.pad = 0;
                    r.s = x; r.e = it.e; r.ps = x; r.pad = 0;
                    const bool wl = k3_worth(P, l.s, l.e), wr = k3_worth(P, r.s, r.e);
                    if (wl && wr) {
                        if (sp < 4) st[sp++] = r; else k3_push_global(G, S.ev, r.s, r.e, r.ps);
                        it = l;
                        continue;
                    }
                    if (wl) { it = l; continue; }
                    if (wr) { it = r; continue; }
                }
                break;
            }
            if (it.ps > (long long)it.s + MW) {
                const int x = k3_forced(P, it.s, it.e);
                k3_emit(G, off, x);
                if (!k3_worth(P, x, it.e)) break;
                it.s = x; it.ps = x;
#if K3_CFG_HALFKEY
                it.pad = 0;
#endif
                continue;
            }
            const int pe = k3_window_end(P, it);
            if (pe - it.ps <= 2 * mw) { it.ps = k3_next_ps(P, it.ps, it.e); continue; }
            const bool ok = screen && S.ebase != K3_NO_EBASE;
            const unsigned nch = ok ? (unsigned)((pe - it.ps - 2 * mw + 1 + 31) >> 5) : 0u;
            const unsigned old = atomicAdd(&nc.alloc, K3_ALLOC_SLOT | nch);
            const unsigned slot = old >> 20;
            if (slot >= (unsigned)K3_LIST) {
                k3_push_global(G, S.ev, it.s, it.e, it.ps);
                break;
            }
            nx.item[slot] = it;
            nx.c0[slot] = (int)(old & (K3_ALLOC_SLOT - 1u));
            nx.cn[slot] = (int)nch;
            nx.flag[slot] = ok ? 0 : K3_FULL_FLAG;
            if (!ok) atomicAdd(&nc.nfull, 1);
            break;
        }
        if (sp == 0) break;
        it = st[--sp];
    }
}

#ifndef K3_CFG_NOINLINE_RESOLVE
#define K3_CFG_NOINLINE_RESOLVE 0
#endif
#if K3_CFG_NOINLINE_RESOLVE
__device__ __noinline__
#else
__device__ __forceinline__
#endif
void k3_resolve(const K3Global &G, K3Shared &S, K3Level &nx, K3Count &nc,
                                           const K3Params &P, int screen, const K3Item it, int x, int reuse = 0)
{
    const int pe = k3_window_end(P, it);
    atomicAdd(&S.cand, (unsigned long long)(pe - it.ps - 2 * P.mw + 1));
    atomicAdd(&S.scans, 1ull);
    K3Item c;
    c.pad = 0;
    if (x >= 0) {
        k3_emit(G, (int64_t)S.off, x);
#if K3_CFG_HALFKEY
        c.pad = (reuse && it.ps == it.s) ? 1 : 0;
#endif
        if (k3_worth(P, it.s, x)) { c.s = it.s; c.e = x; c.ps = it.s; k3_place(&S, &nx, &nc, screen, c); }
#if K3_CFG_HALFKEY
        c.pad = (reuse && pe == it.e) ? 2 : 0;
#endif
        if (k3_worth(P, x, it.e)) {
            bool away = K3_SHARE > 0 && x - it.s >= K3_SHARE && it.e - x >= K3_SHARE;
            if (!away && K3_IDLE_SHARE > 0 && S.share > 0 && x - it.s >= K3_IDLE_SHARE && it.e - x >= K3_IDLE_SHARE)
                away = atomicSub(&S.share, 1) > 0;
            if (away) k3_push_global(G, S.ev, x, it.e, x);
            else { c.s = x; c.e = it.e; c.ps = x; k3_place(&S, &nx, &nc, screen, c); }
        }
    } else {
#if K3_CFG_HALFKEY
        c.pad = 0;
#endif
        c.s = it.s; c.e = it.e; c.ps = k3_next_ps(P, it.ps, it.e);
        k3_place(&S, &nx, &nc, screen, c);
    }
}

__device__ __forceinline__ void k3_request(K3Shared &S, K3Level &L, K3Count &C, int k, int i)
{
    const int r = atomicAdd(&C.nreq, 1);
    if (r < K3_REQ) { S.req_k[r] = k; S.req_i[r] = i; }
    else k3_mark_full(L, C, k);
}

template <class F>
__device__ __forceinline__ void k3_for_pieces(const K3Level &L, int warp, int nwin, int nchunk, F f)
{
    const int per = (nchunk + K3_WARPS - 1) / K3_WARPS;
    const int c_lo = warp * per;
    const int c_hi = c_lo + per < nchunk ? c_lo + per : nchunk;
    if (c_lo >= c_hi) return;
    int lo_s = 0, hi_s = nwin;
    while (hi_s - lo_s > 1) {
        const int mid = (lo_s + hi_s) >> 1;
        if (L.c0[mid] <= c_lo) lo_s = mid; else hi_s = mid;
    }
    int slot = lo_s;
    int c = c_lo;
    while (c < c_hi) {
        while (L.c0[slot] + L.cn[slot] <= c) ++slot;
        const int w_c0 = L.c0[slot], w_c1 = w_c0 + L.cn[slot];
        const int cb = w_c1 < c_hi ? w_c1 : c_hi;
        f(slot, c - w_c0, cb - w_c0);
        c = cb;
    }
}

#ifndef K3_CFG_NOINLINE_SCREEN
#define K3_CFG_NOINLINE_SCREEN 0
#endif
#if K3_CFG_NOINLINE_SCREEN
__device__ __noinline__
#else
__device__ __forceinline__
#endif
void k3_screen_level(const K3Global &G, const K3Params &P, K3Shared &S, int cur, int nwin, int nchunk)
{
    const K3Level &L = S.lv[cur];
    const int lane = threadIdx.x & 31, warp = threadIdx.x >> 5;
    const int mw = P.mw;
    const double2 *ccg = G.cc + S.off;
    K3GlobalCC acc;
    acc.g = ccg;
    const int ebase = S.ebase;
    k3_for_pieces(L, warp, nwin, nchunk, [&](int slot, int ca, int cb) {
        const K3Item it = L.item[slot];
        const int w_pe = k3_window_end(P, it);
        const int w_last = w_pe - mw;
        const int i_end = it.ps + mw + cb * 32 - 1;
        const double2 w_lo = acc.at(it.ps - 1), w_hi = acc.at(w_pe - 1);
        K3Scr a;
        k3_scr_init(a);
#if K3_CFG_HALFKEY
        {
            unsigned long long *hl = G.hkL + S.off, *hr = G.hkR + S.off;
            const int hmode = (it.ps == it.s && w_pe == it.e) ? (it.pad & 3) : 0;
            const int i0 = it.ps + mw + ca * 32 + lane, i1 = i_end < w_last ? i_end : w_last;
            const bool st = (long long)w_pe - it.ps > 3LL * mw;
            if (hmode == 1) k3_screen_lane_hk<1>(ccg, hl, hr, w_lo, w_hi, it.ps, w_pe, ebase, G.RN, i0, i1, 32, st, a);
            else if (hmode == 2) k3_screen_lane_hk<2>(ccg, hl, hr, w_lo, w_hi, it.ps, w_pe, ebase, G.RN, i0, i1, 32, st, a);
            else k3_screen_lane_hk<0>(ccg, hl, hr, w_lo, w_hi, it.ps, w_pe, ebase, G.RN, i0, i1, 32, st, a);
        }
#else
        k3_screen_lane(ccg, w_lo, w_hi, it.ps, w_pe, ebase, G.RN, it.ps + mw + ca * 32 + lane,
                       i_end < w_last ? i_end : w_last, 32, a);
#endif
        unsigned long long K1, K2;
        int I1;
        bool bad;
        k3_warp_summary(a, K1, K2, I1, bad);
        unsigned long long kt = 0ull;
        const unsigned nw = (unsigned)(w_pe - it.ps);
        const bool tok = k3_side(__dsub_rn(w_hi.x, w_lo.x), __dsub_rn(w_hi.y, w_lo.y), __ldg(G.RN + nw), nw, ebase, kt);
        if (lane == 0) {
            S.pc_k1[slot + warp] = K1;
            S.pc_k2[slot + warp] = K2;
            S.pc_i1[slot + warp] = ((I1 - it.ps) & 0x1fffffff) | (bad ? K3_BAD_FLAG : 0);
            S.pc_kt[slot + warp] = tok ? kt : K3_NOKEY;
        }
    });
}

__global__ void __launch_bounds__(K3_THREADS, K3_CTAS_PER_SM) k3_split(K3Global G, K3Params P)
{
    extern __shared__ __align__(16) unsigned char k3_smem[];
    K3Shared &S = *reinterpret_cast<K3Shared *>(k3_smem);
    const int tid = threadIdx.x, lane = tid & 31, warp = tid >> 5;
    const int mw = P.mw, MW = P.MW, W = P.W;
    const int screen = (G.screen && mw >= 1 && W <= K3_MAX_SCREEN_W) ? 1 : 0;

    if (tid == 0) {
        S.G = G;
        S.P = P;
        S.few = ((long long)G.ctr->n_events - (long long)G.ctr->ev_begin) < 2LL * gridDim.x ? 1 : 0;
        S.n_sure = 0; S.n_multi = 0; S.n_full = 0; S.n_cont = 0;
    }
    if (tid == 0 && blockIdx.x == 0) G.ctr->n_long = 0ull;
    for (;;) {
        __syncthreads();
        if (tid == 0) {
            const unsigned long long h = atomicAdd(&G.ctr->q_head, 1ull);
            bool ok = false;
            for (;;) {
                if ((int64_t)h < G.q_cap && *((volatile int *)&G.ready[h]) != 0) { ok = true; break; }
                if (*((volatile long long *)&G.ctr->q_pending) <= 0) break;
                __nanosleep(256);
            }
            S.have = ok ? 1 : 0;
            if (ok) {
                __threadfence();
                const int4 t = __ldcg(reinterpret_cast<const int4 *>(&G.tasks[h]));
                PPTask tk;
                tk.ev = t.x; tk.s = t.y; tk.e = t.z; tk.flags = t.w;
                S.task = tk;
                S.ev = t.x;
                S.off = (long long)G.ev_off[t.x];
                K3GlobalCC a;
                a.g = G.cc + S.off;
                int ebase = 0;
                const bool eok = screen && k3_window_ebase(k3_var(a.at(tk.e - 1), a.at(tk.s - 1), tk.e - tk.s), ebase);
                S.ebase = eok ? ebase : K3_NO_EBASE;
            }
            S.share = 0;
            S.cand = 0;
            S.scans = 0;
            S.exact = 0;
            for (int q = 0; q < 3; ++q) {
                S.cnt[q].alloc = 0; S.cnt[q].nfull = 0; S.cnt[q].nreq = 0; S.cnt[q].nrescan = 0; S.cnt[q].nmulti = 0;
            }
        }
        __syncthreads();
        if (!S.have) break;

        {
            const int ev = S.ev;
            const int64_t off = (int64_t)S.off;
            int s = S.task.s;
            const int e = S.task.e;
            K3GlobalCC acc;
            acc.g = G.cc + off;
            int ps = s + S.task.flags;
            bool done = false;
            while ((long long)e - s > K3_CAP) {
                const long long lim = (long long)e - 2LL * mw;
                if (ps >= lim) {
                    if (e - s <= MW) { done = true; break; }
                    const int x = k3_forced(P, s, e);
                    if (tid == 0) {
                        k3_emit(G, off, x);
                        if (k3_worth(P, s, x)) k3_push_global(G, ev, s, x, s);
                    }
                    s = x; ps = s;
                    continue;
                }
                if (ps > (long long)s + MW) {
                    const int x = k3_forced(P, s, e);
                    if (tid == 0) k3_emit(G, off, x);
                    s = x; ps = s;
                    continue;
                }
                const long long pe_l = (long long)ps + W;
                const int pe = (int)(pe_l < e ? pe_l : e);
                if (pe - ps <= 2 * mw) { ps = k3_next_ps(P, ps, e); continue; }
                const K3Best b = k3_cta_scan(acc, ps, pe, P, G, S);
                if (tid == 0) {
                    atomicAdd(&S.cand, (unsigned long long)(pe - ps - 2 * mw + 1));
                    atomicAdd(&S.scans, 1ull);
                }
                if (b.x >= 0) {
                    if (tid == 0) {
                        k3_emit(G, off, b.x);
                        if (k3_worth(P, s, b.x)) k3_push_global(G, ev, s, b.x, s);
                    }
                    s = b.x; ps = s;
                } else {
                    ps = k3_next_ps(P, ps, e);
                }
            }
            if (!done && tid == 0) {
                K3Item it;
                it.s = s; it.e = e; it.ps = ps; it.pad = 0;
                k3_place(&S, &S.lv[0], &S.cnt[0], screen, it);
            }
        }

        int cur = 0, ci = 0;
        __syncthreads();
        for (;;) {
            K3Level &L = S.lv[cur], &NX = S.lv[cur ^ 1];
            K3Count &C = S.cnt[ci], &NC = S.cnt[ci == 2 ? 0 : ci + 1];
            const unsigned al = C.alloc;
            int nwin = (int)(al >> 20);
            int nchunk = (int)(al & (K3_ALLOC_SLOT - 1u));
            if (nwin == 0) break;
            if (nwin > K3_LIST) {
                nwin = K3_LIST;
                nchunk = L.c0[K3_LIST - 1] + L.cn[K3_LIST - 1];
            }
            const int per = (nchunk + K3_WARPS - 1) / K3_WARPS;
            const double2 *ccg = G.cc + S.off;
            K3GlobalCC acc;
            acc.g = ccg;
            const int ebase = S.ebase;
            unsigned long long qh = 0ull, qt = 0ull;
            if (K3_IDLE_SHARE > 0 && tid == 0 && S.few) {
                qh = *((volatile unsigned long long *)&G.ctr->q_head);
                qt = *((volatile unsigned long long *)&G.ctr->q_tail);
            }
            k3_screen_level(G, P, S, cur, nwin, nchunk);
            if (K3_IDLE_SHARE > 0 && tid == 0 && S.few) {
                const long long waiting = (long long)(qh - qt);
                S.share = waiting > 0 ? (int)(waiting > 64 ? 64 : waiting) : 0;
            }
            __syncthreads();
            if (tid == 0) {
                K3Count &Z = S.cnt[ci == 0 ? 2 : ci - 1];
                Z.alloc = 0; Z.nfull = 0; Z.nreq = 0; Z.nrescan = 0; Z.nmulti = 0;
            }
            for (int k = tid; k < nwin; k += K3_THREADS) {
                const int c0 = L.c0[k], cn = L.cn[k];
                if (cn == 0) continue;
                const int w_first = c0 / per, w_last = (c0 + cn - 1) / per;
                unsigned long long gmin = K3_NOKEY;
                bool bad = false;
                for (int w = w_first; w <= w_last; ++w) {
                    const unsigned long long k1 = S.pc_k1[k + w];
                    gmin = k1 < gmin ? k1 : gmin;
                    bad = bad || (S.pc_i1[k + w] & K3_BAD_FLAG);
                }
                if (bad || gmin == K3_NOKEY) { k3_mark_full(L, C, k); continue; }
                const K3Item it = L.item[k];
                const int nw = k3_window_end(P, it) - it.ps;
                const unsigned long long eps2 = k3_eps2_key(nw);
                const unsigned long long thr = gmin + eps2;
                S.win_thr[k] = thr;
                int nr = 0, i_one = 0;
                bool rescan = false;
                for (int w = w_first; w <= w_last; ++w) {
                    if (S.pc_k2[k + w] <= thr) rescan = true;
                    else if (S.pc_k1[k + w] <= thr) { ++nr; i_one = it.ps + (S.pc_i1[k + w] & 0x1fffffff); }
                }
#if K3_CFG_SURE
                if (!rescan && nr == 1) {
                    const unsigned long long kt = S.pc_kt[k + w_first];
                    if (kt != K3_NOKEY) {
                        const double d = (double)(long long)(kt - gmin);
                        const double want = P.min_gain * K3_KEY_PER_NAT;
                        const double margin = (double)eps2 + 64.0;
                        if (d > want + margin || d < want - margin) {
                            atomicAdd(&S.n_sure, 1u);
                            k3_resolve(G, S, NX, NC, P, screen, it, d > want ? i_one : -1, 1);
                            continue;
                        }
                    }
                }
#endif
                if (rescan || nr > 1) {
                    atomicOr(&L.flag[k], K3_MULTI_FLAG);
                    atomicAdd(&C.nmulti, 1);
                    S.best_key[k] = 0ull;
                    S.best_idx[k] = 0x7fffffff;
                }
                if (rescan) atomicAdd(&C.nrescan, 1);
                for (int w = w_first; w <= w_last; ++w) {
                    if (S.pc_k2[k + w] <= thr) S.pc_i1[k + w] |= K3_RESCAN_FLAG;
                    else if (S.pc_k1[k + w] <= thr) k3_request(S, L, C, k, it.ps + (S.pc_i1[k + w] & 0x1fffffff));
                }
            }
            __syncthreads();
            bool more_work = false;
            if (C.nrescan) {
                more_work = true;
                k3_for_pieces(L, warp, nwin, nchunk, [&](int slot, int ca, int cb) {
                    if (!(S.pc_i1[slot + warp] & K3_RESCAN_FLAG)) return;
                    if (L.flag[slot] & K3_FULL_FLAG) return;
                    const K3Item it = L.item[slot];
                    const int w_pe = k3_window_end(P, it);
                    const int w_last = w_pe - mw;
                    int i_end = it.ps + mw + cb * 32 - 1;
                    i_end = i_end < w_last ? i_end : w_last;
                    const double2 w_lo = acc.at(it.ps - 1), w_hi = acc.at(w_pe - 1);
                    const unsigned long long thr = S.win_thr[slot];
                    for (int i = it.ps + mw + ca * 32 + lane; i <= i_end; i += 32) {
                        unsigned long long key;
                        k3_screen_key_at(ccg, w_lo, w_hi, it.ps, w_pe, i, G.RN, ebase, key);
                        if (key <= thr) k3_request(S, L, C, slot, i);
                    }
                });
                __syncthreads();
            }
            const int nreq = C.nreq < K3_REQ ? C.nreq : K3_REQ;
            if (nreq) {
                more_work = true;
                for (int r0 = 0; r0 < nreq; r0 += 10 * K3_WARPS) {
                    const int part = lane % 3;
                    const int r = r0 + warp * 10 + lane / 3;
                    const bool act = lane < 30 && r < nreq;
                    double v = 0.0;
                    int k = 0, i = 0, fl = 0;
                    K3Item it;
                    it.s = it.e = it.ps = it.pad = 0;
                    if (act) {
                        k = S.req_k[r];
                        i = S.req_i[r];
                        it = L.item[k];
                        fl = L.flag[k];
                        const int w_ps = it.ps, w_pe = k3_window_end(P, it);
                        const double2 lo = acc.at(w_ps - 1), hi = acc.at(w_pe - 1), mid = acc.at(i - 1);
                        if (part == 0) v = k3_exact_tot(lo, hi, w_ps, w_pe);
                        else if (part == 1) v = __dmul_rn((double)(i - w_ps), log(k3_var(mid, lo, i - w_ps)));
                        else v = __dmul_rn((double)(w_pe - i), log(k3_var(hi, mid, w_pe - i)));
                    }
                    const double low = __shfl_down_sync(PP_FULL, v, 1), high = __shfl_down_sync(PP_FULL, v, 2);
                    if (act && part == 0) {
                        const double g = __dsub_rn(v, __dadd_rn(low, high));
                        if (fl & K3_MULTI_FLAG) {
                            S.req_g[r] = g;
                            if (g > P.min_gain) atomicMax(&S.best_key[k], k3_okey(g));
                        } else if (!(fl & K3_FULL_FLAG)) {
                            k3_resolve(G, S, NX, NC, P, screen, it, g > P.min_gain ? i : -1, 1);
                        }
                    }
                }
                if (tid == 0) atomicAdd(&S.exact, (unsigned long long)nreq);
                if (C.nmulti) {
                    __syncthreads();
                    for (int r = tid; r < nreq; r += K3_THREADS) {
                        const int k = S.req_k[r];
                        if (!(L.flag[k] & K3_MULTI_FLAG)) continue;
                        const double g = S.req_g[r];
                        if (g > P.min_gain && k3_okey(g) == S.best_key[k]) atomicMin(&S.best_idx[k], S.req_i[r]);
                    }
                    __syncthreads();
                    for (int k = tid; k < nwin; k += K3_THREADS) {
                        const int fl = L.flag[k];
                        if ((fl & K3_MULTI_FLAG) && !(fl & K3_FULL_FLAG)) {
                            atomicAdd(&S.n_multi, 1u);
                            k3_resolve(G, S, NX, NC, P, screen, L.item[k], S.best_key[k] ? S.best_idx[k] : -1, 1);
                        }
                    }
                }
            }
            if (C.nfull) {
                more_work = true;
                __syncthreads();
                for (int k = 0; k < nwin; ++k) {
                    if (!(L.flag[k] & K3_FULL_FLAG)) continue;
                    const K3Item it = L.item[k];
                    const int pe = k3_window_end(P, it);
                    K3Best b = k3_scan_range(acc, it.ps, pe, mw, P.min_gain, tid, K3_THREADS);
                    b = k3_cta_reduce(b, S);
                    if (tid == 0) {
                        if (screen) {
                            atomicAdd(&S.exact, (unsigned long long)(pe - it.ps - 2 * mw + 1));
                            S.n_full += 1;
                        }
                        k3_resolve(G, S, NX, NC, P, screen, it, b.x);
                    }
                }
            }
            if (more_work) __syncthreads();
            cur ^= 1;
            ci = ci == 2 ? 0 : ci + 1;
        }
        __syncthreads();
        if (tid == 0) {
            atomicAdd(&G.ctr->n_cand, S.cand);
            atomicAdd(&G.ctr->n_scan, S.scans);
            atomicAdd(&G.ctr->n_exact, S.exact);
            atomicAdd(&G.ctr->n_tasks, 1ull);
            __threadfence();
            atomicAdd((unsigned long long *)&G.ctr->q_pending, (unsigned long long)(-1LL));
        }
    }
    if (tid == 0) {
        if (S.n_sure) atomicAdd(&G.ctr->n_sure, (unsigned long long)S.n_sure);
        if (S.n_multi) atomicAdd(&G.ctr->n_multi, (unsigned long long)S.n_multi);
        if (S.n_full) atomicAdd(&G.ctr->n_full, (unsigned long long)S.n_full);
    }
}

#ifndef K3S_CFG_CLUSTER
#define K3S_CFG_CLUSTER 4
#endif
#ifndef K3S_CFG_THREADS
#define K3S_CFG_THREADS 512
#endif
constexpr int K3S_CLUSTER = K3S_CFG_CLUSTER;
constexpr int K3S_THREADS = K3S_CFG_THREADS;
constexpr int K3S_WARPS = K3S_THREADS / 32;
constexpr int K3S_TOTAL = K3S_CLUSTER * K3S_THREADS;

struct K3SpineShared {
    unsigned long long wk1[K3S_WARPS], wk2[K3S_WARPS];
    int wi1[K3S_WARPS];
    int wbad[K3S_WARPS];
    unsigned long long ck1[2][K3S_CLUSTER], ck2[2][K3S_CLUSTER];
    int ci1[2][K3S_CLUSTER];
    int cbad[2][K3S_CLUSTER];
    double wred_g[K3S_WARPS];
    int wred_x[K3S_WARPS];
    double cred_g[2][K3S_CLUSTER];
    int cred_x[2][K3S_CLUSTER];
    int list[K3S_THREADS];
    unsigned char flag[K3S_THREADS];
    int n_list;
};

__device__ __forceinline__ K3Best k3_spine_reduce(K3Best b, K3SpineShared &S, int par)
{
    namespace cg = cooperative_groups;
    cg::cluster_group cluster = cg::this_cluster();
    const int tid = threadIdx.x, lane = tid & 31, warp = tid >> 5;
    b = k3_warp_reduce(b);
    if (lane == 0) { S.wred_g[warp] = b.g; S.wred_x[warp] = b.x; }
    __syncthreads();
    if (warp == 0) {
        K3Best c;
        c.g = lane < K3S_WARPS ? S.wred_g[lane] : 0.0;
        c.x = lane < K3S_WARPS ? S.wred_x[lane] : -1;
        c = k3_warp_reduce(c);
        if (lane == 0) {
            const int rank = (int)cluster.block_rank();
            for (int r = 0; r < K3S_CLUSTER; ++r) {
                K3SpineShared *R = cluster.map_shared_rank(&S, r);
                R->cred_g[par][rank] = c.g;
                R->cred_x[par][rank] = c.x;
            }
        }
    }
    cluster.sync();
    K3Best r;
    r.g = S.cred_g[par][0];
    r.x = S.cred_x[par][0];
#pragma unroll
    for (int w = 1; w < K3S_CLUSTER; ++w) {
        K3Best o;
        o.g = S.cred_g[par][w];
        o.x = S.cred_x[par][w];
        r = k3_better(r, o);
    }
    return r;
}

__device__ __forceinline__ int k3_spine_scan(const K3GlobalCC &acc, int ps, int pe, const K3Params &P, const K3Global &G,
                                             K3SpineShared &S, int ebase, bool screen, int par, unsigned &nexact,
                                             K3Branches &br)
{
    namespace cg = cooperative_groups;
    cg::cluster_group cluster = cg::this_cluster();
    const int tid = threadIdx.x, lane = tid & 31, warp = tid >> 5;
    const int rank = (int)cluster.block_rank();
    const int gtid = rank * K3S_THREADS + tid;
    const double2 lo = acc.at(ps - 1), hi = acc.at(pe - 1);
    asm volatile("prefetch.global.L2 [%0];" ::"l"(acc.g + pe + (long long)gtid * 8));
    if (screen) {
        K3Scr a;
        k3_scr_init(a);
        k3_screen_lane(acc.g, lo, hi, ps, pe, ebase, G.RN, ps + P.mw + gtid, pe - P.mw, K3S_TOTAL, a);
        unsigned long long K1, K2;
        int I1;
        bool bad;
        k3_warp_summary(a, K1, K2, I1, bad);
        unsigned long long kt = 0ull;
        const unsigned nw = (unsigned)(pe - ps);
        const bool tok = k3_side(__dsub_rn(hi.x, lo.x), __dsub_rn(hi.y, lo.y), __ldg(G.RN + nw), nw, ebase, kt);
        if (lane == 0) { S.wk1[warp] = K1; S.wk2[warp] = K2; S.wi1[warp] = I1; S.wbad[warp] = bad ? 1 : 0; }
        __syncthreads();
        if (warp == 0) {
            K3Scr c;
            k3_scr_init(c);
            if (lane < K3S_WARPS) { c.k1 = S.wk1[lane]; c.k2 = S.wk2[lane]; c.i1 = S.wi1[lane]; c.bad = S.wbad[lane]; }
            unsigned long long C1, C2;
            int CI;
            bool cbad;
            k3_warp_summary(c, C1, C2, CI, cbad);
            if (lane == 0) {
                for (int r = 0; r < K3S_CLUSTER; ++r) {
                    K3SpineShared *R = cluster.map_shared_rank(&S, r);
                    R->ck1[par][rank] = C1;
                    R->ck2[par][rank] = C2;
                    R->ci1[par][rank] = CI;
                    R->cbad[par][rank] = cbad ? 1 : 0;
                }
            }
        }
        cluster.sync();
        unsigned long long gmin = K3_NOKEY;
        bool anybad = false;
#pragma unroll
        for (int w = 0; w < K3S_CLUSTER; ++w) {
            const unsigned long long k1 = S.ck1[par][w];
            gmin = k1 < gmin ? k1 : gmin;
            anybad = anybad || S.cbad[par][w];
        }
        if (!anybad && gmin != K3_NOKEY) {
            const unsigned long long eps2 = k3_eps2_key(pe - ps);
            const unsigned long long thr = gmin + eps2;
            int nr = 0, i_one = -1;
            bool rescan = false;
#pragma unroll
            for (int w = 0; w < K3S_CLUSTER; ++w) {
                if (S.ck2[par][w] <= thr) rescan = true;
                else if (S.ck1[par][w] <= thr) { ++nr; i_one = S.ci1[par][w]; }
            }
            if (!rescan && nr == 1 && tok) {
                const double d = (double)(long long)(kt - gmin);
                const double want = P.min_gain * K3_KEY_PER_NAT;
                const double margin = (double)eps2 + 64.0;
                if (d > want + margin) { ++br.sure; return i_one; }
                if (d < want - margin) { ++br.sure; return -1; }
            }
            if (rescan || nr > 1) ++br.multi;
            K3Best b;
            b.g = P.min_gain;
            b.x = -1;
            const double tot = k3_exact_tot(lo, hi, ps, pe);
            if (a.k2 <= thr) {
                const int last = pe - P.mw;
                for (int i = ps + P.mw + gtid; i <= last; i += K3S_TOTAL) {
                    unsigned long long key;
                    k3_screen_key_at(acc.g, lo, hi, ps, pe, i, G.RN, ebase, key);
                    if (key <= thr) {
                        const double g = k3_exact_gain(lo, acc.at(i - 1), hi, ps, pe, i, tot);
                        ++nexact;
                        if (g > b.g) { b.g = g; b.x = i; }
                    }
                }
            } else if (a.k1 <= thr) {
                const double g = k3_exact_gain(lo, acc.at(a.i1 - 1), hi, ps, pe, a.i1, tot);
                ++nexact;
                if (g > b.g) { b.g = g; b.x = a.i1; }
            }
            return k3_spine_reduce(b, S, par).x;
        }
    }
    if (screen) ++br.full;
    K3Best b = k3_scan_range(acc, ps, pe, P.mw, P.min_gain, gtid, K3S_TOTAL);
    if (ps + P.mw + gtid <= pe - P.mw) nexact += (unsigned)((pe - P.mw - (ps + P.mw + gtid)) / K3S_TOTAL + 1);
    return k3_spine_reduce(b, S, par).x;
}

struct K3SpineQueue {
    long long next, end;
    __device__ __forceinline__ void push(const K3Global &G, int ev, int s, int e, int ps)
    {
        if (next == end) {
            next = (long long)atomicAdd(&G.ctr->q_tail, 32ull);
            atomicAdd((unsigned long long *)&G.ctr->q_pending, 32ull);
            end = next + 32;
        }
        if (next < G.q_cap) {
            PPTask t;
            t.ev = ev; t.s = s; t.e = e; t.flags = ps - s;
            *reinterpret_cast<int4 *>(&G.tasks[next]) = *reinterpret_cast<int4 *>(&t);
            G.ready[next] = 1;
        } else {
            atomicOr(&G.ctr->overflow, (unsigned)PP_OVF_QUEUE);
            atomicAdd((unsigned long long *)&G.ctr->q_pending, (unsigned long long)(-1LL));
        }
        ++next;
    }
    __device__ __forceinline__ void flush(const K3Global &G, int ev)
    {
        while (next < end) push(G, ev, 0, 0, 0);
    }
};

__global__ void __cluster_dims__(K3S_CLUSTER, 1, 1) __launch_bounds__(K3S_THREADS, 1) k3_spine(K3Global G, K3Params P)
{
    namespace cg = cooperative_groups;
    cg::cluster_group cluster = cg::this_cluster();
    __shared__ K3SpineShared S;
    const int tid = threadIdx.x;
    const int rank = (int)cluster.block_rank();
    const int cid = blockIdx.x / K3S_CLUSTER, ncl = gridDim.x / K3S_CLUSTER;
    const bool leader = rank == 0 && tid == 0;
    const int mw = P.mw, MW = P.MW, W = P.W;
    const bool screen_ok = G.screen && mw >= 1 && W <= K3_MAX_SCREEN_W;
    if (G.ctr->n_long == 0ull) return;
    const int64_t n_events = (int64_t)G.ctr->n_events, ev_begin = (int64_t)G.ctr->ev_begin;
    int par = 0;
    K3SpineQueue Q;
    Q.next = Q.end = 0;
    for (int64_t base = ev_begin + cid; base < n_events; base += (int64_t)K3S_THREADS * ncl) {
        __syncthreads();
        {
            const int64_t cand_ev = base + (int64_t)tid * ncl;
            bool is_long = false;
            if (cand_ev < n_events) {
                const int64_t l = G.ev_len[cand_ev];
                is_long = l > K3_CAP && l < 0x7fffffffLL;
            }
            S.flag[tid] = is_long ? 1 : 0;
        }
        __syncthreads();
        if (tid == 0) {
            int n = 0;
            for (int t = 0; t < K3S_THREADS; ++t)
                if (S.flag[t]) S.list[n++] = (int)(base + (int64_t)t * ncl);
            S.n_list = n;
        }
        __syncthreads();
        const int n_mine = S.n_list;
        for (int q = 0; q < n_mine; ++q) {
            const int ev = S.list[q];
            const int64_t off = G.ev_off[ev];
            const int e = (int)G.ev_len[ev];
            K3GlobalCC acc;
            acc.g = G.cc + off;
            int ebase = 0;
            const bool screen = screen_ok && k3_window_ebase(k3_var(acc.at(e - 1), acc.at(-1), e), ebase);
            int s = 0, ps = 0;
            unsigned long long cand = 0, scans = 0;
            unsigned nexact = 0;
            K3Branches br;
            br.sure = br.multi = br.full = 0u;
            while ((long long)e - s > K3_CAP) {
                const long long lim = (long long)e - 2LL * mw;
                if (ps >= lim) {
                    if (e - s <= MW) { s = e; break; }
                    const int x = k3_forced(P, s, e);
                    if (leader) {
                        k3_emit(G, off, x);
                        if (k3_worth(P, s, x)) Q.push(G, ev, s, x, s);
                    }
                    s = x; ps = s;
                    continue;
                }
                if (ps > (long long)s + MW) {
                    const int x = k3_forced(P, s, e);
                    if (leader) k3_emit(G, off, x);
                    s = x; ps = s;
                    continue;
                }
                const long long pe_l = (long long)ps + W;
                const int pe = (int)(pe_l < e ? pe_l : e);
                if (pe - ps <= 2 * mw) { ps = k3_next_ps(P, ps, e); continue; }
                const int x = k3_spine_scan(acc, ps, pe, P, G, S, ebase, screen, par, nexact, br);
                if (screen_ok && !screen) ++br.full;
                par ^= 1;
                cand += (unsigned long long)(pe - ps - 2 * mw + 1);
                scans += 1;
                if (x >= 0) {
                    if (leader) {
                        k3_emit(G, off, x);
                        if (k3_worth(P, s, x)) Q.push(G, ev, s, x, s);
                    }
                    s = x; ps = s;
                } else {
                    ps = k3_next_ps(P, ps, e);
                }
            }
            if (leader && s < e && k3_worth(P, s, e)) Q.push(G, ev, s, e, ps);
            if (leader) Q.flush(G, ev);
#pragma unroll
            for (int d = 16; d > 0; d >>= 1) nexact += __shfl_xor_sync(PP_FULL, nexact, d);
            if ((tid & 31) == 0 && nexact) atomicAdd(&G.ctr->n_exact, (unsigned long long)nexact);
            if (leader) {
                atomicAdd(&G.ctr->n_cand, cand);
                atomicAdd(&G.ctr->n_scan, scans);
                if (br.sure) atomicAdd(&G.ctr->n_sure, (unsigned long long)br.sure);
                if (br.multi) atomicAdd(&G.ctr->n_multi, (unsigned long long)br.multi);
                if (br.full) atomicAdd(&G.ctr->n_full, (unsigned long long)br.full);
            }
        }
    }
    cluster.sync();
}

__global__ void __launch_bounds__(256)
k3_debug_screen(K3Global G, int ev, int ps, int pe, int mw, double *h_screen, double *h_exact,
                unsigned char *ok_out)
{
    K3GlobalCC cc;
    cc.g = G.cc + G.ev_off[ev];
    const double2 lo = cc.at(ps - 1), hi = cc.at(pe - 1);
    int ebase = 0;
    const bool wok = k3_window_ebase(k3_var(hi, lo, pe - ps), ebase);
    const int n = pe - mw - (ps + mw) + 1;
    for (int j = blockIdx.x * blockDim.x + threadIdx.x; j < n; j += gridDim.x * blockDim.x) {
        const int i = ps + mw + j;
        unsigned long long key = 0;
        const bool ok = wok && k3_screen_key_at(cc.g, lo, hi, ps, pe, i, G.RN, ebase, key);
        const double2 mid = cc.at(i - 1);
        const double low = __dmul_rn((double)(i - ps), log(k3_var(mid, lo, i - ps)));
        const double high = __dmul_rn((double)(pe - i), log(k3_var(hi, mid, pe - i)));
        h_screen[j] = 0.6931471805599453094 * ((double)key / 8388608.0 + (double)(pe - ps) * (double)(ebase - 1150));
        h_exact[j] = __dadd_rn(low, high);
        ok_out[j] = ok ? 1 : 0;
    }
}

__global__ void __launch_bounds__(256)
k3_window_gains(K3Global G, int ev, int n_windows, const int *__restrict__ ps_a, const int *__restrict__ pe_a, int mw,
                const int64_t *__restrict__ out_off, double *__restrict__ out)
{
    K3GlobalCC cc;
    cc.g = G.cc + G.ev_off[ev];
    for (int w = blockIdx.y; w < n_windows; w += gridDim.y) {
        const int ps = ps_a[w], pe = pe_a[w];
        const int n = pe - ps - 2 * mw + 1;
        if (n <= 0) continue;
        const double2 lo = cc.at(ps - 1), hi = cc.at(pe - 1);
        const double tot = k3_exact_tot(lo, hi, ps, pe);
        double *o = out + out_off[w];
        for (int j = blockIdx.x * blockDim.x + threadIdx.x; j < n; j += gridDim.x * blockDim.x) {
            const int i = ps + mw + j;
            o[j] = k3_exact_gain(lo, cc.at(i - 1), hi, ps, pe, i, tot);
        }
    }
}

__global__ void __launch_bounds__(256) k3_debug_lg2_error(unsigned long long *max_bits)
{
    double worst = 0.0;
    for (unsigned k = blockIdx.x * blockDim.x + threadIdx.x; k < (1u << 23); k += gridDim.x * blockDim.x) {
        const float m = __uint_as_float(0x3f800000u | k);
        float lg;
        asm("lg2.approx.ftz.f32 %0, %1;" : "=f"(lg) : "f"(m));
        const unsigned tb = __float_as_uint(__fadd_rn(lg, 1.0f));
        const double fixed = (double)(tb - 0x3f800000u) / 8388608.0;
        const double err = fabs(fixed - log2((double)m));
        worst = err > worst ? err : worst;
    }
    atomicMax(max_bits, (unsigned long long)__double_as_longlong(worst));
}

__global__ void __launch_bounds__(256) k3_fill_RN(double *RN, int len)
{
    for (int n = blockIdx.x * blockDim.x + threadIdx.x; n < len; n += gridDim.x * blockDim.x)
        RN[n] = n > 0 ? __ddiv_rn(1.0, (double)n) : 0.0;
}

__global__ void __launch_bounds__(256)
k3_init_queue(K3Global G, int use_spine)
{
    const int64_t n_events = (int64_t)G.ctr->n_events;
    const int64_t ev_begin = (int64_t)G.ctr->ev_begin;
    for (int64_t e = ev_begin + blockIdx.x * (int64_t)blockDim.x + threadIdx.x; e < n_events;
         e += (int64_t)gridDim.x * blockDim.x) {
        const int64_t off = G.ev_off[e];
        const int64_t len = G.ev_len[e];
        const int64_t slot = e - ev_begin;
        atomicOr(&G.bits[off >> 5], 1u << (unsigned)(off & 31));
        if (slot < G.q_cap && len < 0x7fffffffLL) {
            PPTask t;
            t.ev = (int)e; t.s = 0; t.e = (int)len; t.flags = 0;
            if (use_spine && len > K3_CAP) {
                t.e = 0;
                atomicAdd(&G.ctr->n_long, 1ull);
            }
            G.tasks[slot] = t;
            G.ready[slot] = 1;
        } else {
            atomicOr(&G.ctr->overflow, (unsigned)PP_OVF_QUEUE);
        }
    }
    if (blockIdx.x == 0 && threadIdx.x == 0) {
        const int64_t cnt = n_events - ev_begin;
        const int64_t q = cnt < G.q_cap ? cnt : G.q_cap;
        G.ctr->q_head = 0;
        G.ctr->q_tail = (unsigned long long)q;
        G.ctr->q_pending = (long long)q;
        if (ev_begin == 0) {
            G.ctr->n_cand = 0;
            G.ctr->n_scan = 0;
            G.ctr->n_tasks = 0;
            G.ctr->n_exact = 0;
            G.ctr->n_sure = 0;
            G.ctr->n_multi = 0;
            G.ctr->n_full = 0;
        }
    }
}

constexpr int CP_THREADS = 256;
constexpr int CP_WPT = 4;
constexpr int CP_BLOCK_WORDS = CP_THREADS * CP_WPT;

__device__ __forceinline__ unsigned k3c_word(const unsigned *__restrict__ bits, int64_t w, int64_t lo, int64_t hi)
{
    const int64_t b0 = w << 5;
    if (b0 + 32 <= lo || b0 >= hi) return 0u;
    unsigned v = bits[w];
    if (b0 < lo) v &= ~0u << (unsigned)(lo - b0);
    if (b0 + 32 > hi) v &= ~0u >> (unsigned)(b0 + 32 - hi);
    return v;
}

__global__ void __launch_bounds__(CP_THREADS)
k3c_count(const unsigned *__restrict__ bits, const PPCounters *ctr, unsigned *__restrict__ block_count)
{
    __shared__ unsigned wsum[CP_THREADS / 32];
    const int tid = threadIdx.x;
    const int64_t lo = (int64_t)ctr->flat_done, hi = (int64_t)ctr->n_event_samples;
    const int64_t blk0 = (int64_t)blockIdx.x * CP_BLOCK_WORDS;
    if ((blk0 + CP_BLOCK_WORDS) * 32 <= lo || blk0 * 32 >= hi) return;
    const int64_t w0 = blk0 + tid * CP_WPT;
    unsigned c = 0;
#pragma unroll
    for (int k = 0; k < CP_WPT; ++k) c += __popc(k3c_word(bits, w0 + k, lo, hi));
#pragma unroll
    for (int d = 16; d > 0; d >>= 1) c += __shfl_xor_sync(PP_FULL, c, d);
    if ((tid & 31) == 0) wsum[tid >> 5] = c;
    __syncthreads();
    if (tid == 0) {
        unsigned t = 0;
        for (int w = 0; w < CP_THREADS / 32; ++w) t += wsum[w];
        block_count[blockIdx.x] = t;
    }
}

__global__ void __launch_bounds__(1024)
k3c_scan(const unsigned *__restrict__ block_count, unsigned long long *__restrict__ block_off, PPCounters *ctr,
         int64_t cap_segs)
{
    __shared__ unsigned long long wtot[32];
    __shared__ unsigned long long s_carry;
    const int tid = threadIdx.x, lane = tid & 31, warp = tid >> 5;
    const int64_t lo = (int64_t)ctr->flat_done, hi = (int64_t)ctr->n_event_samples;
    const int64_t b_lo = lo / (CP_BLOCK_WORDS * 32);
    const int64_t b_hi = hi > lo ? (hi - 1) / (CP_BLOCK_WORDS * 32) + 1 : b_lo;
    if (tid == 0) s_carry = ctr->seg_done;
    __syncthreads();
    for (int64_t c0 = b_lo; c0 < b_hi; c0 += 1024) {
        const int64_t b = c0 + tid;
        const unsigned long long v = b < b_hi ? block_count[b] : 0ull;
        unsigned long long inc = v;
#pragma unroll
        for (int d = 1; d < 32; d <<= 1) {
            unsigned long long t = __shfl_up_sync(PP_FULL, inc, d);
            if (lane >= d) inc += t;
        }
        if (lane == 31) wtot[warp] = inc;
        __syncthreads();
        unsigned long long add = 0;
        for (int w = 0; w < warp; ++w) add += wtot[w];
        const unsigned long long excl = s_carry + add + inc - v;
        if (b < b_hi) block_off[b] = excl;
        __syncthreads();
        if (tid == 1023) s_carry = excl + v;
        __syncthreads();
    }
    if (tid == 0) {
        ctr->n_segments = s_carry;
        if ((int64_t)s_carry > cap_segs) atomicOr(&ctr->overflow, (unsigned)PP_OVF_SEGS);
    }
}

__global__ void __launch_bounds__(CP_THREADS)
k3c_write(const unsigned *__restrict__ bits, const unsigned long long *__restrict__ block_off,
          const int64_t *__restrict__ ev_off, const PPCounters *ctr, int64_t *__restrict__ seg_flat,
          int *__restrict__ seg_event, int64_t *__restrict__ seg_start, int64_t cap_segs)
{
    __shared__ unsigned wsum[CP_THREADS / 32];
    const int tid = threadIdx.x, lane = tid & 31, warp = tid >> 5;
    const int64_t lo = (int64_t)ctr->flat_done, hi = (int64_t)ctr->n_event_samples;
    const int64_t blk0 = (int64_t)blockIdx.x * CP_BLOCK_WORDS;
    if ((blk0 + CP_BLOCK_WORDS) * 32 <= lo || blk0 * 32 >= hi) return;
    const int64_t w0 = blk0 + tid * CP_WPT;
    unsigned wv[CP_WPT];
    unsigned c = 0;
#pragma unroll
    for (int k = 0; k < CP_WPT; ++k) {
        wv[k] = k3c_word(bits, w0 + k, lo, hi);
        c += __popc(wv[k]);
    }
    unsigned inc = c;
#pragma unroll
    for (int d = 1; d < 32; d <<= 1) {
        unsigned t = __shfl_up_sync(PP_FULL, inc, d);
        if (lane >= d) inc += t;
    }
    if (lane == 31) wsum[warp] = inc;
    __syncthreads();
    unsigned add = 0;
    for (int w = 0; w < warp; ++w) add += wsum[w];
    if (c == 0) return;
    unsigned long long k = block_off[blockIdx.x] + add + inc - c;
    const int64_t n_events = (int64_t)ctr->n_events;
    int64_t ev = -1, ev_end = 0, ev_begin = 0;
#pragma unroll
    for (int q = 0; q < CP_WPT; ++q) {
        unsigned w = wv[q];
        while (w) {
            const int bit = __ffs(w) - 1;
            w &= w - 1;
            const int64_t f = (w0 + q) * 32 + bit;
            if (ev < 0) {
                ev = pp_upper_index(ev_off, n_events, f);
                ev_begin = ev_off[ev];
                ev_end = ev_off[ev + 1];
            }
            while (f >= ev_end) { ++ev; ev_begin = ev_end; ev_end = ev_off[ev + 1]; }
            if ((int64_t)k < cap_segs) {
                seg_flat[k] = f;
                seg_event[k] = (int)ev;
                seg_start[k] = f - ev_begin;
            }
            ++k;
        }
    }
}

__global__ void __launch_bounds__(256)
k3c_ends(const PPCounters *ctr, const int64_t *__restrict__ seg_flat,
         const int *__restrict__ seg_event, const int64_t *__restrict__ ev_off,
         int64_t *__restrict__ seg_end, int64_t cap_segs)
{
    int64_t S = (int64_t)ctr->n_segments;
    if (S > cap_segs) S = cap_segs;
    const int64_t total = (int64_t)ctr->n_event_samples;
    for (int64_t k = (int64_t)ctr->seg_done + blockIdx.x * (int64_t)blockDim.x + threadIdx.x; k < S;
         k += (int64_t)gridDim.x * blockDim.x) {
        const int64_t fe = (k + 1 < S) ? seg_flat[k + 1] : total;
        seg_end[k] = fe - ev_off[seg_event[k]];
    }
}

struct PPHostTables {
    int64_t cap_events;
    int64_t *ev_start, *ev_len;
    int64_t cap_segments;
    int *seg_event;
    int64_t *seg_start, *seg_end;
// ... 42 lines not shown
```

### pypore_b200/csrc/split_flow.cuh

```cuda
#pragma once
#include "split.cuh"

#ifndef K3F_CFG_CTAS
#define K3F_CFG_CTAS 7
#endif
#ifndef K3F_CFG_MIN_PIECE
#define K3F_CFG_MIN_PIECE 32
#endif
#ifndef K3F_CFG_MAXP
#define K3F_CFG_MAXP 8
#endif
#ifndef K3F_CFG_THREADS
#define K3F_CFG_THREADS 128
#endif
constexpr int K3F_THREADS = K3F_CFG_THREADS;
constexpr int K3F_WARPS = K3F_THREADS / 32;
constexpr int K3F_CTAS_PER_SM = K3F_CFG_CTAS;
constexpr int K3F_MAXP = K3F_CFG_MAXP;
constexpr int K3F_MIN_PIECE = K3F_CFG_MIN_PIECE;
constexpr int K3F_WINS = 48;
constexpr int K3F_STACK = K3F_WINS * K3F_MAXP;
#ifndef K3F_CFG_EVS
#define K3F_CFG_EVS 3
#endif
constexpr int K3F_EVS = K3F_CFG_EVS;
#ifndef K3F_CFG_LOCAL
#define K3F_CFG_LOCAL 2048
#endif
constexpr int K3F_LOCAL = K3F_CFG_LOCAL;
constexpr int K3F_LSTACK = 24;
#ifndef PP_SPLIT_KERNEL_DEFAULT
#define PP_SPLIT_KERNEL_DEFAULT 0
#endif
constexpr long long K3F_SPIN_LIMIT = 1LL << 26;

struct K3FWin {
    int s, e, ps;
    short evs;
    unsigned char npieces;
    unsigned char exact;
    int piece_chunks;
    int done;
    int pad;
    unsigned long long k1[K3F_MAXP];
    unsigned long long k2[K3F_MAXP];
    int i1[K3F_MAXP];
};

struct K3FEvent {
    long long off;
    int ev;
    int ebase;
    int live;
    int pad;
};

struct K3FShared {
    K3FWin win[K3F_WINS];
    int free_list[K3F_WINS];
    int stack[K3F_STACK];
    K3FEvent evs[K3F_EVS];
    K3Item lst[K3F_WARPS][K3F_LSTACK];
    int n_free, top, lock, fetching, drained, few, failed, pad;
    unsigned long long cand, scans, exact, tasks;
    unsigned long long sure, multi, full;
    K3Global G;
    K3Params P;
};

constexpr size_t K3F_SMEM_BYTES = sizeof(K3FShared);

__device__ __forceinline__ void f_lock(K3FShared &S)
{
    while (atomicCAS(&S.lock, 0, 1) != 0) { }
    __threadfence_block();
}

__device__ __forceinline__ void f_unlock(K3FShared &S)
{
    __threadfence_block();
    atomicExch(&S.lock, 0);
}

__device__ __forceinline__ void f_push_global(const K3Global &G, int ev, int s, int e, int ps)
{
    atomicAdd((unsigned long long *)&G.ctr->q_pending, 1ull);
    const unsigned long long slot = atomicAdd(&G.ctr->q_tail, 1ull);
    if ((int64_t)slot >= G.q_cap) {
        atomicOr(&G.ctr->overflow, (unsigned)PP_OVF_QUEUE);
        atomicAdd((unsigned long long *)&G.ctr->q_pending, (unsigned long long)(-1LL));
        return;
    }
    PPTask t;
    t.ev = ev; t.s = s; t.e = e; t.flags = ps - s;
    *reinterpret_cast<int4 *>(&G.tasks[slot]) = *reinterpret_cast<int4 *>(&t);
    __threadfence();
    atomicExch(&G.ready[slot], 1);
}

__device__ __forceinline__ void f_finish_event(K3FShared &S, int es)
{
    S.evs[es].ev = -1;
    S.tasks += 1;
    __threadfence();
    atomicAdd((unsigned long long *)&S.G.ctr->q_pending, (unsigned long long)(-1LL));
}

__device__ __forceinline__ void f_register(K3FShared &S, int es, const K3Item &it, int screen)
{
    const K3Params &P = S.P;
    const int pe = k3_window_end(P, it);
    const int nch = (pe - it.ps - 2 * P.mw + 1 + 31) >> 5;
    if (S.n_free == 0) {
        f_push_global(S.G, S.evs[es].ev, it.s, it.e, it.ps);
        return;
    }
    const int w = S.free_list[--S.n_free];
    K3FWin &Wn = S.win[w];
    int np = 1, pc = nch;
    if (nch > K3F_MIN_PIECE) {
        np = (nch + K3F_MIN_PIECE - 1) / K3F_MIN_PIECE;
        if (np > K3F_MAXP) np = K3F_MAXP;
        pc = (nch + np - 1) / np;
        np = (nch + pc - 1) / pc;
    }
    Wn.s = it.s; Wn.e = it.e; Wn.ps = it.ps;
    Wn.evs = (short)es;
    Wn.npieces = (unsigned char)np;
    Wn.exact = (screen && S.evs[es].ebase != K3_NO_EBASE) ? 0 : 1;
    Wn.piece_chunks = pc;
    Wn.done = 0;
    S.evs[es].live += 1;
    for (int p = np - 1; p >= 0; --p) S.stack[S.top++] = (w << 4) | p;
}

__device__ __noinline__ void f_place(K3FShared *Sp, int es, int screen, K3Item it)
{
    K3FShared &S = *Sp;
    const K3Global &G = S.G;
    const K3Params &P = S.P;
    const int mw = P.mw, MW = P.MW;
    const int64_t off = (int64_t)S.evs[es].off;
    K3Item st[4];
    int sp = 0;
    for (;;) {
        for (;;) {
            const long long lim = (long long)it.e - 2LL * mw;
            if (it.ps >= lim) {
                if (it.e - it.s > MW) {
                    const int x = k3_forced(P, it.s, it.e);
                    k3_emit(G, off, x);
                    K3Item l, r;
                    l.s = it.s; l.e = x; l.ps = it.s; l.pad = 0;
                    r.s = x; r.e = it.e; r.ps = x; r.pad = 0;
                    const bool wl = k3_worth(P, l.s, l.e), wr = k3_worth(P, r.s, r.e);
                    if (wl && wr) {
                        if (sp < 4) st[sp++] = r; else f_push_global(G, S.evs[es].ev, r.s, r.e, r.s);
                        it = l;
                        continue;
                    }
                    if (wl) { it = l; continue; }
                    if (wr) { it = r; continue; }
                }
                break;
            }
            if (it.ps > (long long)it.s + MW) {
                const int x = k3_forced(P, it.s, it.e);
                k3_emit(G, off, x);
                if (!k3_worth(P, x, it.e)) break;
                it.s = x; it.ps = x;
                continue;
            }
            const int pe = k3_window_end(P, it);
            if (pe - it.ps <= 2 * mw) { it.ps = k3_next_ps(P, it.ps, it.e); continue; }
            f_register(S, es, it, screen);
            break;
        }
        if (sp == 0) break;
        it = st[--sp];
    }
}

__device__ __noinline__ K3Best f_exact_range(const double2 *ccg, int ps, int pe, int i0, int i_end, double min_gain)
{
    K3GlobalCC acc;
    acc.g = ccg;
    const double2 lo = acc.at(ps - 1), hi = acc.at(pe - 1);
    const double tot = k3_exact_tot(lo, hi, ps, pe);
    K3Best b;
    b.g = min_gain;
    b.x = -1;
    for (int i = i0; i <= i_end; i += 32) {
        const double g = k3_exact_gain(lo, acc.at(i - 1), hi, ps, pe, i, tot);
        if (g > b.g) { b.g = g; b.x = i; }
    }
    return k3_warp_reduce(b);
}

__device__ __noinline__ bool f_exact_one(const double2 *ccg, int ps, int pe, int i, double min_gain)
{
    K3GlobalCC acc;
    acc.g = ccg;
    const double2 lo = acc.at(ps - 1), hi = acc.at(pe - 1);
    return k3_exact_gain(lo, acc.at(i - 1), hi, ps, pe, i, k3_exact_tot(lo, hi, ps, pe)) > min_gain;
}

__device__ __noinline__ int f_contend(const double *RN, const double2 *ccg, int ps, int pe, int mw, int ebase, int pc,
                                      double min_gain, unsigned long long thr, unsigned single, unsigned rescan, int I1,
                                      unsigned &nexact)
{
    const int lane = threadIdx.x & 31;
    K3GlobalCC acc;
    acc.g = ccg;
    const double2 lo = acc.at(ps - 1), hi = acc.at(pe - 1);
    const double tot = k3_exact_tot(lo, hi, ps, pe);
    K3Best b;
    b.g = min_gain;
    b.x = -1;
    unsigned cnt = 0;
    if (single & (1u << lane)) {
        const int i = ps + (I1 & 0x1fffffff);
        const double g = k3_exact_gain(lo, acc.at(i - 1), hi, ps, pe, i, tot);
        ++cnt;
        if (g > b.g) { b.g = g; b.x = i; }
    }
    const int w_last = pe - mw;
    for (unsigned m = rescan; m; m &= m - 1) {
        const int p = __ffs(m) - 1;
        int i_end = ps + mw + (p + 1) * pc * 32 - 1;
        i_end = i_end < w_last ? i_end : w_last;
        K3Best r;
        r.g = min_gain;
        r.x = -1;
        for (int i = ps + mw + p * pc * 32 + lane; i <= i_end; i += 32) {
            unsigned long long key;
            k3_screen_key_at(ccg, lo, hi, ps, pe, i, RN, ebase, key);
            if (key <= thr) {
                const double g = k3_exact_gain(lo, acc.at(i - 1), hi, ps, pe, i, tot);
                ++cnt;
                if (g > r.g) { r.g = g; r.x = i; }
            }
        }
        b = k3_better(b, r);
    }
    b = k3_warp_reduce(b);
#pragma unroll
    for (int d = 16; d > 0; d >>= 1) cnt += __shfl_xor_sync(PP_FULL, cnt, d);
    nexact += cnt;
    return b.x;
}

__device__ __forceinline__ int f_decide(const K3Global &G, const K3Params &P, const double2 *ccg, const double2 lo,
                                        const double2 hi, int ps, int pe, int ebase, int np, int pc,
                                        unsigned long long K1, unsigned long long K2, int I1, unsigned &nexact,
                                        K3Branches &br)
{
    const int lane = threadIdx.x & 31;
    const int mw = P.mw;
    const bool anybad = __any_sync(PP_FULL, lane < np && (I1 & K3_BAD_FLAG));
    const unsigned long long gmin = k3_warp_min_u64(K1);
    if (anybad || gmin == K3_NOKEY) {
        nexact += (unsigned)(pe - ps - 2 * mw + 1);
        ++br.full;
        return f_exact_range(ccg, ps, pe, ps + mw + lane, pe - mw, P.min_gain).x;
    }
    const unsigned long long eps2 = k3_eps2_key(pe - ps);
    const unsigned long long thr = gmin + eps2;
    const unsigned rescan = __ballot_sync(PP_FULL, lane < np && K2 <= thr);
    const unsigned single = __ballot_sync(PP_FULL, lane < np && K2 > thr && K1 <= thr);
    if (rescan || __popc(single) != 1) {
        ++br.multi;
        return f_contend(G.RN, ccg, ps, pe, mw, ebase, pc, P.min_gain, thr, single, rescan, I1, nexact);
    }
    const int i_one = ps + (__shfl_sync(PP_FULL, I1, __ffs(single) - 1) & 0x1fffffff);
    unsigned long long kt = 0ull;
    const unsigned nw = (unsigned)(pe - ps);
    if (k3_side(__dsub_rn(hi.x, lo.x), __dsub_rn(hi.y, lo.y), __ldg(G.RN + nw), nw, ebase, kt)) {
        const double d = (double)(long long)(kt - gmin);
        const double want = P.min_gain * K3_KEY_PER_NAT;
        const double margin = (double)eps2 + 64.0;
        if (d > want + margin) { ++br.sure; return i_one; }
        if (d < want - margin) { ++br.sure; return -1; }
    }
    nexact += 1;
    return f_exact_one(ccg, ps, pe, i_one, P.min_gain) ? i_one : -1;
}

struct K3FTally { unsigned long long cand, scans, exact; K3Branches br; };

__device__ __noinline__ int f_fetch(K3FShared *Sp, int screen)
{
    K3FShared &S = *Sp;
    const K3Global &G = S.G;
    const unsigned long long h = atomicAdd(&G.ctr->q_head, 1ull);
    bool ok = false;
    for (long long spin = 0;; ++spin) {
        if ((int64_t)h < G.q_cap && *((volatile int *)&G.ready[h]) != 0) { ok = true; break; }
        if (*((volatile long long *)&G.ctr->q_pending) <= 0) break;
        if (spin > (K3F_SPIN_LIMIT >> 4)) { atomicOr(&G.ctr->overflow, (unsigned)PP_OVF_QUEUE); S.failed = 1; break; }
        __nanosleep(1000);
    }
    if (!ok) {
        f_lock(S);
        S.drained = 1;
        S.fetching = 0;
        f_unlock(S);
        return -1;
    }
    __threadfence();
    const int4 t = __ldcg(reinterpret_cast<const int4 *>(&G.tasks[h]));
    const long long off = (long long)G.ev_off[t.x];
    int ebase = K3_NO_EBASE;
    if (t.z > t.y) {
        K3GlobalCC a;
        a.g = G.cc + off;
        int eb = 0;
        if (screen && k3_window_ebase(k3_var(a.at(t.z - 1), a.at(t.y - 1), t.z - t.y), eb)) ebase = eb;
    }
    f_lock(S);
    int es = 0;
    while (es < K3F_EVS - 1 && S.evs[es].ev >= 0) ++es;
    S.evs[es].ev = t.x;
    S.evs[es].off = off;
    S.evs[es].ebase = ebase;
    S.evs[es].live = 1;
    S.fetching = 0;
    int r = -1;
    if (k3_worth(S.P, t.y, t.z)) {
        K3Item it;
        it.s = t.y; it.e = t.z; it.ps = t.y + t.w; it.pad = 0;
        if (it.e - it.s <= K3F_LOCAL) {
            S.lst[threadIdx.x >> 5][0] = it;
            r = (es << 8) | 1;
        } else {
            f_place(&S, es, screen, it);
        }
    }
    if (r < 0 && --S.evs[es].live == 0) f_finish_event(S, es);
    f_unlock(S);
    return r;
}

__device__ __noinline__ void f_retire(K3FShared *Sp, int es, int screen, int w, const K3Item *kids, int nk, int keeps)
{
    K3FShared &S = *Sp;
    f_lock(S);
    for (int k = 0; k < nk; ++k) f_place(&S, es, screen, kids[k]);
    S.free_list[S.n_free++] = w;
    if (!keeps && --S.evs[es].live == 0) f_finish_event(S, es);
    f_unlock(S);
}

__global__ void __launch_bounds__(K3F_THREADS, K3F_CTAS_PER_SM) k3_flow(K3Global G, K3Params P)
{
    extern __shared__ __align__(16) unsigned char k3f_smem[];
    K3FShared &S = *reinterpret_cast<K3FShared *>(k3f_smem);
    const int tid = threadIdx.x, lane = tid & 31;
    const int mw = P.mw, MW = P.MW;
    const int screen = (G.screen && mw >= 1 && P.W <= K3_MAX_SCREEN_W) ? 1 : 0;
    K3Item *st = S.lst[tid >> 5];

    if (tid == 0) {
        S.G = G;
        S.P = P;
        S.few = ((long long)G.ctr->n_events - (long long)G.ctr->ev_begin) < 2LL * gridDim.x ? 1 : 0;
        S.n_free = K3F_WINS;
        S.top = 0; S.lock = 0; S.fetching = 0; S.drained = 0; S.failed = 0;
        S.cand = S.scans = S.exact = S.tasks = 0ull;
        S.sure = S.multi = S.full = 0ull;
        for (int e = 0; e < K3F_EVS; ++e) { S.evs[e].ev = -1; S.evs[e].live = 0; }
    }
    for (int k = tid; k < K3F_WINS; k += K3F_THREADS) S.free_list[k] = K3F_WINS - 1 - k;
    if (tid == 0 && blockIdx.x == 0) G.ctr->n_long = 0ull;
    __syncthreads();

    K3FTally T;
    T.cand = T.scans = T.exact = 0ull;
    T.br.sure = T.br.multi = T.br.full = 0u;
    long long idle = 0;
    int ln = 0;
    int les = -1;
    for (;;) {
        K3Item it;
        int es, w = -1, p = 0, np = 1, pc = 0;
        bool exact;
        if (ln > 0) {
            it = st[--ln];
            __syncwarp();
            es = les;
        } else {
            int action = 0, entry = 0;
            if (lane == 0 && (idle == 0 || les >= 0 || *((volatile int *)&S.top) > 0 || (idle & 7) == 0)) {
                f_lock(S);
                if (les >= 0 && --S.evs[les].live == 0) f_finish_event(S, les);
                if (S.top > 0) {
                    entry = S.stack[--S.top];
                    action = 1;
                } else if (S.failed) {
                    action = 3;
                } else {
                    int free_ev = 0;
                    for (int e = 0; e < K3F_EVS; ++e) free_ev += S.evs[e].ev < 0;
                    if (S.drained) action = (free_ev == K3F_EVS && !S.fetching) ? 3 : 0;
                    else if (!S.fetching && free_ev > 0 && S.n_free >= 4) { S.fetching = 1; action = 4; }
                }
                f_unlock(S);
                if (action == 4) {
                    entry = f_fetch(&S, screen);
                    action = entry >= 0 ? 2 : 5;
                }
            }
            les = -1;
            action = __shfl_sync(PP_FULL, action, 0);
            entry = __shfl_sync(PP_FULL, entry, 0);
            if (action == 3) break;
            if (action == 0) {
                if (++idle > (K3F_SPIN_LIMIT >> 3)) {
                    if (lane == 0) { atomicOr(&G.ctr->overflow, (unsigned)PP_OVF_QUEUE); S.failed = 1; }
                    break;
                }
                __nanosleep(500);
                continue;
            }
            idle = 0;
            if (action == 5) continue;
            if (action == 2) {
                les = entry >> 8;
                ln = 1;
                continue;
            }
            w = entry >> 4;
            p = entry & 15;
            const K3FWin &Wn = S.win[w];
            it.s = Wn.s; it.e = Wn.e; it.ps = Wn.ps; it.pad = 0;
            es = Wn.evs;
            np = Wn.npieces;
            pc = Wn.piece_chunks;
        }
        const long long off = S.evs[es].off;
        const int ebase = S.evs[es].ebase;
        auto push = [&](const K3Item &c) {
            if (ln < K3F_LSTACK) {
                if (lane == 0) st[ln] = c;
                ++ln;
            } else if (lane == 0) {
                f_lock(S);
                f_place(&S, es, screen, c);
                f_unlock(S);
            }
        };
        if (w < 0) {
            bool scan = false;
            for (;;) {
                const long long lim = (long long)it.e - 2LL * mw;
                if (it.ps >= lim) {
                    if (it.e - it.s > MW) {
                        const int x = k3_forced(P, it.s, it.e);
                        if (lane == 0) k3_emit(G, off, x);
                        K3Item l, r;
                        l.s = it.s; l.e = x; l.ps = it.s; l.pad = 0;
                        r.s = x; r.e = it.e; r.ps = x; r.pad = 0;
                        const bool wl = k3_worth(P, l.s, l.e), wr = k3_worth(P, r.s, r.e);
                        if (wl && wr) { push(r); it = l; continue; }
                        if (wl) { it = l; continue; }
                        if (wr) { it = r; continue; }
                    }
                    break;
                }
                if (it.ps > (long long)it.s + MW) {
                    const int x = k3_forced(P, it.s, it.e);
                    if (lane == 0) k3_emit(G, off, x);
                    if (!k3_worth(P, x, it.e)) break;
                    it.s = x; it.ps = x;
                    continue;
                }
                const int pe_t = k3_window_end(P, it);
                if (pe_t - it.ps <= 2 * mw) { it.ps = k3_next_ps(P, it.ps, it.e); continue; }
                scan = true;
                break;
            }
            __syncwarp();
            if (!scan) continue;
        }
        exact = !(screen && ebase != K3_NO_EBASE);

        const double2 *ccg = G.cc + off;
        K3GlobalCC acc;
        acc.g = ccg;
        const int pe = k3_window_end(P, it);
        const int ncand = pe - it.ps - 2 * mw + 1;
        const int nch = (ncand + 31) >> 5;
        if (w < 0) pc = nch;
        const double2 lo = acc.at(it.ps - 1), hi = acc.at(pe - 1);
        unsigned long long K1, K2 = K3_NOKEY;
        int I1;
        {
            const int w_last = pe - mw;
            int i_end = it.ps + mw + (p + 1) * pc * 32 - 1;
            i_end = i_end < w_last ? i_end : w_last;
            const int i0 = it.ps + mw + p * pc * 32 + lane;
            if (!exact) {
                K3Scr a;
                k3_scr_init(a);
                k3_screen_lane(ccg, lo, hi, it.ps, pe, ebase, G.RN, i0, i_end, 32, a);
                bool bad;
                k3_warp_summary(a, K1, K2, I1, bad);
                I1 = ((I1 - it.ps) & 0x1fffffff) | (bad ? K3_BAD_FLAG : 0);
            } else {
                const K3Best b = f_exact_range(ccg, it.ps, pe, i0, i_end, P.min_gain);
                K1 = (unsigned long long)__double_as_longlong(b.g);
                I1 = b.x;
            }
        }
        if (np > 1) {
            K3FWin &Wn = S.win[w];
            int old = 0;
            if (lane == 0) {
                Wn.k1[p] = K1; Wn.k2[p] = K2; Wn.i1[p] = I1;
                __threadfence_block();
                old = atomicAdd(&Wn.done, 1);
                __threadfence_block();
            }
            old = __shfl_sync(PP_FULL, old, 0);
            if (old != np - 1) continue;
            const volatile K3FWin &V = Wn;
            K1 = lane < np ? V.k1[lane] : K3_NOKEY;
            K2 = lane < np ? V.k2[lane] : K3_NOKEY;
            I1 = lane < np ? V.i1[lane] : -1;
        } else if (lane != 0 && !exact) {
            K1 = K2 = K3_NOKEY;
            I1 = -1;
        }

        int x;
        unsigned nexact = 0;
        if (!exact) {
            x = f_decide(G, P, ccg, lo, hi, it.ps, pe, ebase, np, pc, K1, K2, I1, nexact, T.br);
        } else {
            K3Best b;
            b.g = __longlong_as_double((long long)K1);
            b.x = I1;
            if (np > 1) {
                if (lane >= np) { b.g = P.min_gain; b.x = -1; }
                b = k3_warp_reduce(b);
            }
            x = __shfl_sync(PP_FULL, b.x, 0);
            if (screen) {
                nexact = (unsigned)ncand;
                ++T.br.full;
            }
        }
        T.cand += (unsigned long long)ncand;
        T.scans += 1;
        T.exact += nexact;

        K3Item big[2];
        int nbig = 0;
        const int ln_before = ln;
        auto child = [&](const K3Item &c) {
            if (w < 0 || c.e - c.s <= K3F_LOCAL) push(c);
            else big[nbig++] = c;
        };
        if (x >= 0) {
            if (lane == 0) k3_emit(G, off, x);
            K3Item c;
            c.pad = 0;
            if (k3_worth(P, x, it.e)) {
                bool away = false;
                if (K3_IDLE_SHARE > 0 && S.few && x - it.s >= K3_IDLE_SHARE && it.e - x >= K3_IDLE_SHARE) {
                    int waiting = 0;
                    if (lane == 0) {
                        const unsigned long long qh = *((volatile unsigned long long *)&G.ctr->q_head);
                        const unsigned long long qt = *((volatile unsigned long long *)&G.ctr->q_tail);
                        waiting = (long long)(qh - qt) > 0 ? 1 : 0;
                    }
                    away = __shfl_sync(PP_FULL, waiting, 0) != 0;
                }
                if (away) {
                    if (lane == 0) f_push_global(G, S.evs[es].ev, x, it.e, x);
                } else {
                    c.s = x; c.e = it.e; c.ps = x;
                    child(c);
                }
            }
            if (k3_worth(P, it.s, x)) { c.s = it.s; c.e = x; c.ps = it.s; child(c); }
        } else {
            it.ps = k3_next_ps(P, it.ps, it.e);
            child(it);
        }
        if (w >= 0) {
            const int keeps = ln > ln_before ? 1 : 0;
            if (lane == 0) f_retire(&S, es, screen, w, big, nbig, keeps);
            if (keeps) les = es;
        }
        __syncwarp();
    }
    if (lane == 0) {
        atomicAdd(&S.cand, T.cand);
        atomicAdd(&S.scans, T.scans);
        atomicAdd(&S.exact, T.exact);
        if (T.br.sure) atomicAdd(&S.sure, (unsigned long long)T.br.sure);
        if (T.br.multi) atomicAdd(&S.multi, (unsigned long long)T.br.multi);
        if (T.br.full) atomicAdd(&S.full, (unsigned long long)T.br.full);
    }
    __syncthreads();
    if (tid == 0) {
        atomicAdd(&G.ctr->n_cand, S.cand);
        atomicAdd(&G.ctr->n_scan, S.scans);
        atomicAdd(&G.ctr->n_exact, S.exact);
        atomicAdd(&G.ctr->n_tasks, S.tasks);
        if (S.sure) atomicAdd(&G.ctr->n_sure, S.sure);
        if (S.multi) atomicAdd(&G.ctr->n_multi, S.multi);
        if (S.full) atomicAdd(&G.ctr->n_full, S.full);
    }
}
```

Measured before the change: 40850.

## Replace ready-flag queue with 128-bit atomic slot exchange and optional length ordering

Work-queue slots now carry their own validity: producers publish tasks with a single 128-bit atomic exchange and consumers claim them by exchanging in zeros. This drops the separate ready array, its per-call memset and the threadfence-then-flag handshake. It also adds optional length-bucketed queue ordering through a histogram and prefix-sum kernel, plus a selectable share policy and timeline instrumentation, all off by default. Risks: relies on b128 atomics being available and correct, and empty placeholder tasks must now be encoded as nonzero, which the K3_EMPTY_FLAGS marker handles.

```diff
diff --git a/include/pypore_b200.h b/include/pypore_b200.h
--- a/include/pypore_b200.h
+++ b/include/pypore_b200.h
@@ -44,7 +44,9 @@
     PP_OPT_SCREEN = 0,
     PP_OPT_SPINE = 1,
     PP_OPT_SPLIT_CTAS = 2,
-    PP_OPT_SPLIT_KERNEL = 3
+    PP_OPT_SPLIT_KERNEL = 3,
+    PP_OPT_SPLIT_ORDER = 4,
+    PP_OPT_SPLIT_SHARE = 5
 };
 int pp_set_option(pp_ctx *ctx, int option, int64_t value);
 int pp_get_option(pp_ctx *ctx, int option, int64_t *value);
diff --git a/pypore_b200/csrc/api.cu b/pypore_b200/csrc/api.cu
--- a/pypore_b200/csrc/api.cu
+++ b/pypore_b200/csrc/api.cu
@@ -69,7 +69,7 @@
     DevBuf flat64;
     int64_t flat_cap = 0;
 
-    DevBuf cc, bits, tasks, ready, block_count, block_off, inexact, Ttab, ev_tile_off, k2_bits, k2_tiles;
+    DevBuf cc, bits, tasks, q_order, block_count, block_off, inexact, Ttab, ev_tile_off, k2_bits, k2_tiles;
     DevBuf hk;
     DevBuf unpack_flag;
     DevBuf ctl_buf, ctl_peers_dev;
@@ -82,7 +82,10 @@
     int opt_screen = 1;
     int opt_split_ctas = 0;
     int opt_split_kernel = PP_SPLIT_KERNEL_DEFAULT;
+    int opt_split_order = K3_ORDER_TRACE;
+    int opt_split_share = 0;
     int64_t q_cap = 0;
+    bool q_dirty = true;
     DevBuf seg_flat, seg_event, seg_start, seg_end, seg_mean, seg_std, seg_min, seg_max;
     int64_t cap_segs = 0;
     int64_t n_segments = -1;
@@ -431,8 +434,9 @@
     const int64_t n_blocks = (n_words + CP_BLOCK_WORDS - 1) / CP_BLOCK_WORDS;
     CKR(ensure(ctx, ctx->cc, sizeof(double2) * ncap));
     CKR(ensure(ctx, ctx->bits, sizeof(unsigned) * n_words));
+    if (!ctx->tasks.p || sizeof(PPTask) * q_cap > ctx->tasks.cap) ctx->q_dirty = true;
     CKR(ensure(ctx, ctx->tasks, sizeof(PPTask) * q_cap));
-    CKR(ensure(ctx, ctx->ready, sizeof(int) * q_cap));
+    CKR(ensure(ctx, ctx->q_order, sizeof(unsigned) * (2 * K3_ORDER_BUCKETS + 1)));
     CKR(ensure(ctx, ctx->block_count, sizeof(unsigned) * n_blocks));
     CKR(ensure(ctx, ctx->block_off, sizeof(unsigned long long) * n_blocks));
     if (cap_segs > ctx->cap_segs) {
@@ -521,14 +525,17 @@
 {
     StageRange nvtx_range("pypore:split");
     const int64_t q_cap = ctx->q_cap;
-    CK(cudaMemsetAsync(ctx->ready.p, 0, sizeof(int) * q_cap, ctx->stream));
+    if (ctx->q_dirty) CK(cudaMemsetAsync(ctx->tasks.p, 0, ctx->tasks.cap, ctx->stream));
+    ctx->q_dirty = false;
+    const int order = ctx->opt_split_order;
+    if (order != K3_ORDER_TRACE)
+        CK(cudaMemsetAsync(ctx->q_order.p, 0, sizeof(unsigned) * (2 * K3_ORDER_BUCKETS + 1), ctx->stream));
     K3Global G;
     G.cc = (const double2 *)ctx->cc.p;
     G.ev_off = (const int64_t *)ctx->ev_off.p;
     G.ev_len = (const int64_t *)ctx->ev_len.p;
     G.bits = (unsigned *)ctx->bits.p;
     G.tasks = (PPTask *)ctx->tasks.p;
-    G.ready = (int *)ctx->ready.p;
     G.q_cap = q_cap;
     G.ctr = ctx->ctr;
     if (W + 1 > ctx->T_len) {
@@ -539,6 +546,7 @@
     }
     G.RN = (const double *)ctx->Ttab.p;
     G.screen = ctx->opt_screen;
+    G.share = ctx->opt_split_share;
 #if K3_CFG_HALFKEY
     CKR(ensure(ctx, ctx->hk, 2 * sizeof(unsigned long long) * (size_t)ctx->flat_cap));
     G.hkL = (unsigned long long *)ctx->hk.p;
@@ -546,14 +554,19 @@
 #endif
     K3Params P;
     P.mw = mw; P.MW = MW; P.W = W; P.min_gain = min_gain;
-    k3_init_queue<<<ctx->sm_count, 256, 0, ctx->stream>>>(G, ctx->opt_spine);
-    LAUNCHED(ctx);
+    const int wave = ctx->sm_count * (ctx->opt_split_kernel ? K3F_CTAS_PER_SM : K3_CTAS_PER_SM);
+    const int k3_grid = ctx->opt_split_ctas > 0 && ctx->opt_split_ctas < wave ? ctx->opt_split_ctas : wave;
+    k3_init_queue<<<ctx->sm_count, 256, 0, ctx->stream>>>(G, ctx->opt_spine, order, (unsigned *)ctx->q_order.p);
+    LAUNCHED(ctx);
+    if (order != K3_ORDER_TRACE) {
+        k3_order_queue<<<ctx->sm_count, 256, 0, ctx->stream>>>(G, ctx->opt_spine, order, (unsigned *)ctx->q_order.p,
+                                                               (unsigned)k3_grid * K3_CFG_TAIL / 4u);
+        LAUNCHED(ctx);
+    }
     if (ctx->opt_spine) {
         k3_spine<<<(ctx->sm_count / K3S_CLUSTER) * K3S_CLUSTER, K3S_THREADS, 0, ctx->stream>>>(G, P);
         LAUNCHED(ctx);
     }
-    const int wave = ctx->sm_count * (ctx->opt_split_kernel ? K3F_CTAS_PER_SM : K3_CTAS_PER_SM);
-    const int k3_grid = ctx->opt_split_ctas > 0 && ctx->opt_split_ctas < wave ? ctx->opt_split_ctas : wave;
     if (ctx->opt_split_kernel)
         k3_flow<<<k3_grid, K3F_THREADS, K3F_SMEM_BYTES, ctx->stream>>>(G, P);
     else
@@ -652,6 +665,7 @@
 int check_overflow(pp_ctx *ctx)
 {
     const unsigned o = ctx->h_ctr->overflow;
+    if (o & PP_OVF_QUEUE) ctx->q_dirty = true;
     if (o & PP_OVF_QUEUE) return fail(ctx, PP_ERR_CAPACITY, "split work queue overflow");
     if (o & PP_OVF_SEGS) return fail(ctx, PP_ERR_CAPACITY, "segment table overflow");
     if (o & PP_OVF_FILTER_SHORT)
@@ -737,7 +751,7 @@
     DevBuf *bufs[] = {&ctx->trace_buf, &ctx->pend[0].buf, &ctx->pend[1].buf, &ctx->trace_spare, &ctx->k1_rec, &ctx->k1_staged, &ctx->k1_blk, &ctx->run_start, &ctx->run_minkey,
                       &ctx->run_maxkey, &ctx->run_len, &ctx->run_min, &ctx->run_max, &ctx->run_below,
                       &ctx->ev_start, &ctx->ev_len, &ctx->ev_off, &ctx->flat64, &ctx->cc, &ctx->bits,
-                      &ctx->tasks, &ctx->ready, &ctx->block_count, &ctx->block_off, &ctx->inexact, &ctx->Ttab, &ctx->ev_tile_off, &ctx->k2_bits, &ctx->k2_tiles,
+                      &ctx->tasks, &ctx->q_order, &ctx->block_count, &ctx->block_off, &ctx->inexact, &ctx->Ttab, &ctx->ev_tile_off, &ctx->k2_bits, &ctx->k2_tiles,
                       &ctx->seg_flat, &ctx->seg_event, &ctx->seg_start, &ctx->seg_end, &ctx->seg_mean,
                       &ctx->seg_std, &ctx->seg_min, &ctx->seg_max, &ctx->evs_mean, &ctx->evs_std,
                       &ctx->evs_min, &ctx->evs_max, &ctx->filt_tmp, &ctx->filt_carry, &ctx->filt_coef, &ctx->hk, &ctx->unpack_flag, &ctx->ctl_buf, &ctx->ctl_peers_dev,
@@ -799,6 +813,14 @@
         if (value < 0 || value > (1 << 20)) return fail(ctx, PP_ERR_ARG, "bad CTA count %lld", (long long)value);
         ctx->opt_split_ctas = (int)value;
         return PP_OK;
+    case PP_OPT_SPLIT_ORDER:
+        if (value < K3_ORDER_LONGEST || value > K3_ORDER_SHORT_LAST) return fail(ctx, PP_ERR_ARG, "bad split order %lld", (long long)value);
+        ctx->opt_split_order = (int)value;
+        return PP_OK;
+    case PP_OPT_SPLIT_SHARE:
+        if (value < 0 || value > 2) return fail(ctx, PP_ERR_ARG, "bad split share policy %lld", (long long)value);
+        ctx->opt_split_share = (int)value;
+        return PP_OK;
     default: return fail(ctx, PP_ERR_ARG, "unknown option %d", option);
     }
 }
@@ -811,6 +833,8 @@
     case PP_OPT_SPINE: *value = ctx->opt_spine; return PP_OK;
     case PP_OPT_SPLIT_KERNEL: *value = ctx->opt_split_kernel; return PP_OK;
     case PP_OPT_SPLIT_CTAS: *value = ctx->opt_split_ctas; return PP_OK;
+    case PP_OPT_SPLIT_ORDER: *value = ctx->opt_split_order; return PP_OK;
+    case PP_OPT_SPLIT_SHARE: *value = ctx->opt_split_share; return PP_OK;
     default: return fail(ctx, PP_ERR_ARG, "unknown option %d", option);
     }
 }
@@ -1448,6 +1472,27 @@
     release(a);
     return PP_OK;
 }
+
+#if K3_CFG_TIMELINE
+int pp_debug_k3_timeline(pp_ctx *ctx, unsigned long long *out, unsigned *counts, int *ctas, int *per_cta)
+{
+    if (!ctx) return PP_ERR_ARG;
+    CKR(set_device(ctx));
+    CK(cudaStreamSynchronize(ctx->stream));
+    if (ctas) *ctas = K3_TL_CTAS;
+    if (per_cta) *per_cta = K3_TL_N;
+    if (!out) {
+        void *p = nullptr;
+        CK(cudaGetSymbolAddress(&p, k3_tl_n));
+        CK(cudaMemset(p, 0, sizeof(unsigned) * K3_TL_CTAS));
+    } else {
+        CK(cudaMemcpyFromSymbol(out, k3_tl, sizeof(unsigned long long) * K3_TL_CTAS * K3_TL_N));
+        CK(cudaMemcpyFromSymbol(counts, k3_tl_n, sizeof(unsigned) * K3_TL_CTAS));
+    }
+    CK(cudaDeviceSynchronize());
+    return PP_OK;
+}
+#endif
 
 int pp_pipeline(pp_ctx *ctx, const pp_pipeline_params *p, int64_t out[4])
 {
@@ -1578,6 +1623,7 @@
     const unsigned o = (unsigned)rec[4];
     if (o & PP_OVF_CTL) return fail(ctx, PP_ERR_STATE, "a peer's control record did not arrive (pp_ctl_exchange timed out)");
     if (rec[0] > ctx->cap_runs) return fail(ctx, PP_ERR_CAPACITY, "run table overflow");
+    if (o & PP_OVF_QUEUE) ctx->q_dirty = true;
     if (o & PP_OVF_QUEUE) return fail(ctx, PP_ERR_CAPACITY, "split work queue overflow");
     if (o & PP_OVF_SEGS) return fail(ctx, PP_ERR_CAPACITY, "segment table overflow");
     return PP_OK;
diff --git a/pypore_b200/csrc/split.cuh b/pypore_b200/csrc/split.cuh
--- a/pypore_b200/csrc/split.cuh
+++ b/pypore_b200/csrc/split.cuh
@@ -54,7 +54,8 @@
 constexpr double K3_HUGE = 1e280;
 constexpr unsigned long long K3_NOKEY = ~0ull;
 
-struct PPTask { int ev, s, e, flags; };
+struct __align__(16) PPTask { int ev, s, e, flags; };
+constexpr int K3_EMPTY_FLAGS = 1;
 struct K3Item { int s, e, ps, pad; };
 struct K3Params { int mw, MW, W; double min_gain; };
 struct K3Best { double g; int x; };
@@ -67,11 +68,11 @@
     const int64_t *ev_len;
     unsigned *bits;
     PPTask *tasks;
-    int *ready;
     int64_t q_cap;
     PPCounters *ctr;
     const double *RN;
     int screen;
+    int share;
 #if K3_CFG_HALFKEY
     unsigned long long *hkL, *hkR;
 #endif
@@ -107,7 +108,7 @@
     unsigned long long red_k[K3_WARPS];
     int red_x[K3_WARPS];
     int share;
-    int few;
+    int share_min;
     int have;
     int ev;
     long long off;
@@ -121,6 +122,29 @@
 };
 
 constexpr size_t K3_SMEM_BYTES = sizeof(K3Shared);
+
+#ifndef K3_CFG_TIMELINE
+#define K3_CFG_TIMELINE 0
+#endif
+#if K3_CFG_TIMELINE
+enum { K3_TL_START = 0, K3_TL_TAKE = 1, K3_TL_DONE = 2, K3_TL_WAIT = 3, K3_TL_EXIT = 4 };
+constexpr int K3_TL_CTAS = 2048, K3_TL_N = 512;
+__device__ unsigned long long k3_tl[K3_TL_CTAS * K3_TL_N];
+__device__ unsigned k3_tl_n[K3_TL_CTAS];
+__device__ __forceinline__ void k3_tl_mark(int kind)
+{
+    unsigned long long t;
+    asm volatile("mov.u64 %0, %%globaltimer;" : "=l"(t));
+    const unsigned b = blockIdx.x, n = k3_tl_n[b < K3_TL_CTAS ? b : 0];
+    if (b < K3_TL_CTAS && n < K3_TL_N) {
+        k3_tl[b * K3_TL_N + n] = (t & ~7ull) | (unsigned long long)kind;
+        k3_tl_n[b] = n + 1;
+    }
+}
+#define K3_TL(kind) k3_tl_mark(kind)
+#else
+#define K3_TL(kind) ((void)0)
+#endif
 
 struct K3GlobalCC {
     const double2 *g;
@@ -557,6 +581,25 @@
     return ((long long)e - s > 2LL * P.mw) || (e - s > P.MW);
 }
 
+__device__ __forceinline__ void k3_slot_put(PPTask *p, const PPTask t)
+{
+    const unsigned long long lo = ((unsigned long long)(unsigned)t.s << 32) | (unsigned)t.ev;
+    const unsigned long long hi = ((unsigned long long)(unsigned)t.flags << 32) | (unsigned)t.e;
+    asm volatile("{\n\t.reg .b128 d, v;\n\tmov.b128 v, {%1, %2};\n\tatom.relaxed.gpu.global.exch.b128 d, [%0], v;\n\t}"
+                 :: "l"(p), "l"(lo), "l"(hi) : "memory");
+}
+
+__device__ __forceinline__ bool k3_slot_take(PPTask *p, PPTask &t)
+{
+    unsigned long long lo, hi;
+    asm volatile("{\n\t.reg .b128 d, v;\n\tmov.b128 v, {%2, %2};\n\tatom.relaxed.gpu.global.exch.b128 d, [%3], v;\n\t"
+                 "mov.b128 {%0, %1}, d;\n\t}"
+                 : "=l"(lo), "=l"(hi) : "l"(0ull), "l"(p) : "memory");
+    t.ev = (int)(unsigned)lo; t.s = (int)(unsigned)(lo >> 32);
+    t.e = (int)(unsigned)hi; t.flags = (int)(unsigned)(hi >> 32);
+    return (lo | hi) != 0ull;
+}
+
 __device__ void k3_push_global(const K3Global &G, int ev, int s, int e, int ps)
 {
     atomicAdd((unsigned long long *)&G.ctr->q_pending, 1ull);
@@ -568,9 +611,7 @@
     }
     PPTask t;
     t.ev = ev; t.s = s; t.e = e; t.flags = ps - s;
-    *reinterpret_cast<int4 *>(&G.tasks[slot]) = *reinterpret_cast<int4 *>(&t);
-    __threadfence();
-    atomicExch(&G.ready[slot], 1);
+    k3_slot_put(&G.tasks[slot], t);
 }
 
 __device__ __forceinline__ int k3_forced(const K3Params &P, int s, int e)
@@ -687,7 +728,7 @@
 #endif
         if (k3_worth(P, x, it.e)) {
             bool away = K3_SHARE > 0 && x - it.s >= K3_SHARE && it.e - x >= K3_SHARE;
-            if (!away && K3_IDLE_SHARE > 0 && S.share > 0 && x - it.s >= K3_IDLE_SHARE && it.e - x >= K3_IDLE_SHARE)
+            if (!away && S.share > 0 && x - it.s >= S.share_min && it.e - x >= S.share_min)
                 away = atomicSub(&S.share, 1) > 0;
             if (away) k3_push_global(G, S.ev, x, it.e, x);
             else { c.s = x; c.e = it.e; c.ps = x; k3_place(&S, &nx, &nc, screen, c); }
@@ -795,9 +836,10 @@
     const int screen = (G.screen && mw >= 1 && W <= K3_MAX_SCREEN_W) ? 1 : 0;
 
     if (tid == 0) {
+        K3_TL(K3_TL_START);
         S.G = G;
         S.P = P;
-        S.few = ((long long)G.ctr->n_events - (long long)G.ctr->ev_begin) < 2LL * gridDim.x ? 1 : 0;
+        S.share_min = G.share == 2 ? (2 * mw > 1 ? 2 * mw : 1) : K3_IDLE_SHARE;
         S.n_sure = 0; S.n_multi = 0; S.n_full = 0; S.n_cont = 0;
     }
     if (tid == 0 && blockIdx.x == 0) G.ctr->n_long = 0ull;
@@ -806,20 +848,19 @@
         if (tid == 0) {
             const unsigned long long h = atomicAdd(&G.ctr->q_head, 1ull);
             bool ok = false;
-            for (;;) {
-                if ((int64_t)h < G.q_cap && *((volatile int *)&G.ready[h]) != 0) { ok = true; break; }
+            PPTask tk;
+            for (int polls = 0;; ++polls) {
+                if ((int64_t)h < G.q_cap && k3_slot_take(&G.tasks[h], tk)) { ok = true; break; }
                 if (*((volatile long long *)&G.ctr->q_pending) <= 0) break;
+                if (polls == 0) K3_TL(K3_TL_WAIT);
                 __nanosleep(256);
             }
             S.have = ok ? 1 : 0;
             if (ok) {
-                __threadfence();
-                const int4 t = __ldcg(reinterpret_cast<const int4 *>(&G.tasks[h]));
-                PPTask tk;
-                tk.ev = t.x; tk.s = t.y; tk.e = t.z; tk.flags = t.w;
+                K3_TL(K3_TL_TAKE);
                 S.task = tk;
-                S.ev = t.x;
-                S.off = (long long)G.ev_off[t.x];
+                S.ev = tk.ev;
+                S.off = (long long)G.ev_off[tk.ev];
                 K3GlobalCC a;
                 a.g = G.cc + S.off;
                 int ebase = 0;
@@ -908,14 +949,16 @@
             acc.g = ccg;
             const int ebase = S.ebase;
             unsigned long long qh = 0ull, qt = 0ull;
-            if (K3_IDLE_SHARE > 0 && tid == 0 && S.few) {
+            if (K3_IDLE_SHARE > 0 && tid == 0 && G.share == 0) {
                 qh = *((volatile unsigned long long *)&G.ctr->q_head);
                 qt = *((volatile unsigned long long *)&G.ctr->q_tail);
             }
             k3_screen_level(G, P, S, cur, nwin, nchunk);
-            if (K3_IDLE_SHARE > 0 && tid == 0 && S.few) {
+            if (K3_IDLE_SHARE > 0 && tid == 0 && G.share == 0) {
                 const long long waiting = (long long)(qh - qt);
                 S.share = waiting > 0 ? (int)(waiting > 64 ? 64 : waiting) : 0;
+            } else if (tid == 0 && G.share == 2) {
+                S.share = 2 * K3_LIST;
             }
             __syncthreads();
             if (tid == 0) {
@@ -1074,11 +1117,12 @@
             atomicAdd(&G.ctr->n_scan, S.scans);
             atomicAdd(&G.ctr->n_exact, S.exact);
             atomicAdd(&G.ctr->n_tasks, 1ull);
-            __threadfence();
             atomicAdd((unsigned long long *)&G.ctr->q_pending, (unsigned long long)(-1LL));
+            K3_TL(K3_TL_DONE);
         }
     }
     if (tid == 0) {
+        K3_TL(K3_TL_EXIT);
         if (S.n_sure) atomicAdd(&G.ctr->n_sure, (unsigned long long)S.n_sure);
         if (S.n_multi) atomicAdd(&G.ctr->n_multi, (unsigned long long)S.n_multi);
         if (S.n_full) atomicAdd(&G.ctr->n_full, (unsigned long long)S.n_full);
@@ -1258,8 +1302,7 @@
         if (next < G.q_cap) {
             PPTask t;
             t.ev = ev; t.s = s; t.e = e; t.flags = ps - s;
-            *reinterpret_cast<int4 *>(&G.tasks[next]) = *reinterpret_cast<int4 *>(&t);
-            G.ready[next] = 1;
+            G.tasks[next] = t;
         } else {
             atomicOr(&G.ctr->overflow, (unsigned)PP_OVF_QUEUE);
             atomicAdd((unsigned long long *)&G.ctr->q_pending, (unsigned long long)(-1LL));
@@ -1268,7 +1311,7 @@
     }
     __device__ __forceinline__ void flush(const K3Global &G, int ev)
     {
-        while (next < end) push(G, ev, 0, 0, 0);
+        while (next < end) push(G, ev, 0, 0, K3_EMPTY_FLAGS);
     }
 };
 
@@ -1438,8 +1481,37 @@
         RN[n] = n > 0 ? __ddiv_rn(1.0, (double)n) : 0.0;
 }
 
+enum { K3_ORDER_LONGEST = 0, K3_ORDER_TRACE = 1, K3_ORDER_SHORTEST = 2, K3_ORDER_SHORT_LAST = 3 };
+constexpr int K3_ORDER_BUCKETS = 1024;
+constexpr int K3_ORDER_SHIFT = 4;
+#ifndef K3_CFG_TAIL
+#define K3_CFG_TAIL 4
+#endif
+
+__device__ __forceinline__ int k3_order_bucket(int64_t len, int order)
+{
+    const int64_t b = len >> K3_ORDER_SHIFT;
+    const int k = (int)(b < K3_ORDER_BUCKETS - 1 ? b : K3_ORDER_BUCKETS - 1);
+    return order == K3_ORDER_LONGEST ? K3_ORDER_BUCKETS - 1 - k : k;
+}
+
+__device__ __forceinline__ void k3_init_task(const K3Global &G, int use_spine, int64_t e, int64_t len, int64_t slot)
+{
+    if (slot < G.q_cap && len < 0x7fffffffLL) {
+        PPTask t;
+        t.ev = (int)e; t.s = 0; t.e = (int)len; t.flags = 0;
+        if (use_spine && len > K3_CAP) {
+            t.e = 0;
+            t.flags = K3_EMPTY_FLAGS;
+        }
+        G.tasks[slot] = t;
+    } else {
+        atomicOr(&G.ctr->overflow, (unsigned)PP_OVF_QUEUE);
+    }
+}
+
 __global__ void __launch_bounds__(256)
-k3_init_queue(K3Global G, int use_spine)
+k3_init_queue(K3Global G, int use_spine, int order, unsigned *hist)
 {
     const int64_t n_events = (int64_t)G.ctr->n_events;
     const int64_t ev_begin = (int64_t)G.ctr->ev_begin;
@@ -1447,20 +1519,10 @@
          e += (int64_t)gridDim.x * blockDim.x) {
         const int64_t off = G.ev_off[e];
         const int64_t len = G.ev_len[e];
-        const int64_t slot = e - ev_begin;
         atomicOr(&G.bits[off >> 5], 1u << (unsigned)(off & 31));
-        if (slot < G.q_cap && len < 0x7fffffffLL) {
-            PPTask t;
-            t.ev = (int)e; t.s = 0; t.e = (int)len; t.flags = 0;
-            if (use_spine && len > K3_CAP) {
-                t.e = 0;
-                atomicAdd(&G.ctr->n_long, 1ull);
-            }
-            G.tasks[slot] = t;
-            G.ready[slot] = 1;
-        } else {
-            atomicOr(&G.ctr->overflow, (unsigned)PP_OVF_QUEUE);
-        }
+        if (use_spine && len > K3_CAP && len < 0x7fffffffLL) atomicAdd(&G.ctr->n_long, 1ull);
+        if (order == K3_ORDER_TRACE) k3_init_task(G, use_spine, e, len, e - ev_begin);
+        else atomicAdd(&hist[k3_order_bucket(len, order)], 1u);
     }
     if (blockIdx.x == 0 && threadIdx.x == 0) {
         const int64_t cnt = n_events - ev_begin;
@@ -1477,6 +1539,55 @@
             G.ctr->n_multi = 0;
             G.ctr->n_full = 0;
         }
+    }
+}
+
+__global__ void __launch_bounds__(256)
+k3_order_queue(K3Global G, int use_spine, int order, unsigned *hist, unsigned tail)
+{
+    constexpr int PER = K3_ORDER_BUCKETS / 256;
+    __shared__ unsigned base[K3_ORDER_BUCKETS + 1];
+    __shared__ unsigned wsum[8];
+    __shared__ unsigned tail_n;
+    const int tid = threadIdx.x, lane = tid & 31, warp = tid >> 5;
+    unsigned c[PER], tot = 0;
+#pragma unroll
+    for (int k = 0; k < PER; ++k) { c[k] = __ldcg(hist + tid * PER + k); tot += c[k]; }
+    unsigned inc = tot;
+#pragma unroll
+    for (int d = 1; d < 32; d <<= 1) {
+        const unsigned t = __shfl_up_sync(PP_FULL, inc, d);
+        if (lane >= d) inc += t;
+    }
+    if (lane == 31) wsum[warp] = inc;
+    if (tid == 0) tail_n = 0;
+    __syncthreads();
+    unsigned run = inc - tot;
+    for (int w = 0; w < warp; ++w) run += wsum[w];
+    unsigned tl = 0;
+#pragma unroll
+    for (int k = 0; k < PER; ++k) {
+        base[tid * PER + k] = run;
+        run += c[k];
+        if (run <= tail) tl = run;
+    }
+    if (tid == 255) base[K3_ORDER_BUCKETS] = run;
+    if (tl) atomicMax(&tail_n, tl);
+    __syncthreads();
+    const int64_t n_events = (int64_t)G.ctr->n_events;
+    const int64_t ev_begin = (int64_t)G.ctr->ev_begin;
+    const unsigned head_n = (unsigned)(n_events - ev_begin) - tail_n;
+    for (int64_t e = ev_begin + blockIdx.x * (int64_t)blockDim.x + threadIdx.x; e < n_events;
+         e += (int64_t)gridDim.x * blockDim.x) {
+        const int64_t len = G.ev_len[e];
+        const int b = k3_order_bucket(len, order);
+        int64_t slot;
+        if (order != K3_ORDER_SHORT_LAST) slot = (int64_t)base[b] + atomicAdd(&hist[K3_ORDER_BUCKETS + b], 1u);
+        else if (base[b + 1] <= tail_n)
+            slot = (int64_t)head_n + (tail_n - base[b + 1]) + atomicAdd(&hist[K3_ORDER_BUCKETS + b], 1u);
+        else
+            slot = atomicAdd(&hist[2 * K3_ORDER_BUCKETS], 1u);
+        k3_init_task(G, use_spine, e, len, slot);
     }
 }
 
diff --git a/pypore_b200/csrc/split_flow.cuh b/pypore_b200/csrc/split_flow.cuh
--- a/pypore_b200/csrc/split_flow.cuh
+++ b/pypore_b200/csrc/split_flow.cuh
@@ -82,22 +82,6 @@
     atomicExch(&S.lock, 0);
 }
 
-__device__ __forceinline__ void f_push_global(const K3Global &G, int ev, int s, int e, int ps)
-{
-    atomicAdd((unsigned long long *)&G.ctr->q_pending, 1ull);
-    const unsigned long long slot = atomicAdd(&G.ctr->q_tail, 1ull);
-    if ((int64_t)slot >= G.q_cap) {
-        atomicOr(&G.ctr->overflow, (unsigned)PP_OVF_QUEUE);
-        atomicAdd((unsigned long long *)&G.ctr->q_pending, (unsigned long long)(-1LL));
-        return;
-    }
-    PPTask t;
-    t.ev = ev; t.s = s; t.e = e; t.flags = ps - s;
-    *reinterpret_cast<int4 *>(&G.tasks[slot]) = *reinterpret_cast<int4 *>(&t);
-    __threadfence();
-    atomicExch(&G.ready[slot], 1);
-}
-
 __device__ __forceinline__ void f_finish_event(K3FShared &S, int es)
 {
     S.evs[es].ev = -1;
@@ -112,7 +96,7 @@
     const int pe = k3_window_end(P, it);
     const int nch = (pe - it.ps - 2 * P.mw + 1 + 31) >> 5;
     if (S.n_free == 0) {
-        f_push_global(S.G, S.evs[es].ev, it.s, it.e, it.ps);
+        k3_push_global(S.G, S.evs[es].ev, it.s, it.e, it.ps);
         return;
     }
     const int w = S.free_list[--S.n_free];
@@ -155,7 +139,7 @@
                     r.s = x; r.e = it.e; r.ps = x; r.pad = 0;
                     const bool wl = k3_worth(P, l.s, l.e), wr = k3_worth(P, r.s, r.e);
                     if (wl && wr) {
-                        if (sp < 4) st[sp++] = r; else f_push_global(G, S.evs[es].ev, r.s, r.e, r.s);
+                        if (sp < 4) st[sp++] = r; else k3_push_global(G, S.evs[es].ev, r.s, r.e, r.s);
                         it = l;
                         continue;
                     }
@@ -294,8 +278,9 @@
     const K3Global &G = S.G;
     const unsigned long long h = atomicAdd(&G.ctr->q_head, 1ull);
     bool ok = false;
+    PPTask tk;
     for (long long spin = 0;; ++spin) {
-        if ((int64_t)h < G.q_cap && *((volatile int *)&G.ready[h]) != 0) { ok = true; break; }
+        if ((int64_t)h < G.q_cap && k3_slot_take(&G.tasks[h], tk)) { ok = true; break; }
         if (*((volatile long long *)&G.ctr->q_pending) <= 0) break;
         if (spin > (K3F_SPIN_LIMIT >> 4)) { atomicOr(&G.ctr->overflow, (unsigned)PP_OVF_QUEUE); S.failed = 1; break; }
         __nanosleep(1000);
@@ -307,8 +292,7 @@
         f_unlock(S);
         return -1;
     }
-    __threadfence();
-    const int4 t = __ldcg(reinterpret_cast<const int4 *>(&G.tasks[h]));
+    const int4 t = make_int4(tk.ev, tk.s, tk.e, tk.flags);
     const long long off = (long long)G.ev_off[t.x];
     int ebase = K3_NO_EBASE;
     if (t.z > t.y) {
@@ -577,7 +561,7 @@
                     away = __shfl_sync(PP_FULL, waiting, 0) != 0;
                 }
                 if (away) {
-                    if (lane == 0) f_push_global(G, S.evs[es].ev, x, it.e, x);
+                    if (lane == 0) k3_push_global(G, S.evs[es].ev, x, it.e, x);
                 } else {
                     c.s = x; c.e = it.e; c.ps = x;
                     child(c);
```

New measurement: 41600 (median of 6 runs). 1.9% higher.
